# LIU-YUXI/SA-GNN

Hardware: AMD Instinct MI355X
Metric: spmm_edges_per_sec (higher is better)
Workload: dtype f32

## Files before the change

### include/sagnn.h

```cpp
#ifndef SAGNN_H
#define SAGNN_H

#include <stddef.h>
#include <stdint.h>

#ifdef __cplusplus
extern "C" {
#endif

#define SAGNN_VERSION 10302

enum {
  SAGNN_OK = 0,
  SAGNN_ERR_NULL = -1,
  SAGNN_ERR_DIM = -2,
  SAGNN_ERR_ALIGN = -3,
  SAGNN_ERR_CSR = -4,
  SAGNN_ERR_ARG = -5,
  SAGNN_ERR_WORKSPACE = -6,
  SAGNN_ERR_NOMEM = -7
};

int sagnn_version(void);

enum { SAGNN_ENGINE_F16X2 = 0, SAGNN_ENGINE_F32 = 1, SAGNN_ENGINE_VALU = 2 };
int sagnn_set_engine(int engine);
int sagnn_get_engine(void);
int sagnn_range_redo_count(int64_t* count, int reset);

size_t sagnn_last_error(char* buf, size_t cap);

int sagnn_profile_enable(int capacity);
int sagnn_profile_read(float* ms, int32_t* kind, int64_t* units_a, int64_t* units_b, int cap,
                       int* n_out);

int sagnn_csr_check_host(const int32_t* h_rowptr, const int32_t* h_colidx,
                         int64_t n_rows, int64_t n_src, int64_t nnz);

typedef struct sagnn_spmm_plan sagnn_spmm_plan;

typedef struct sagnn_spmm_tuning {
  int32_t short_thresh;
  int32_t long_thresh;
  int32_t chunk_edges;
  int32_t reserved;
} sagnn_spmm_tuning;

typedef struct sagnn_spmm_plan_info {
  int64_t n_rows, n_src, nnz;
  int64_t n_long_rows;
  int64_t n_chunks;
  int32_t short_thresh, long_thresh, chunk_edges;
  int32_t max_degree;
  int32_t on_device;
  int32_t reserved;
} sagnn_spmm_plan_info;

int sagnn_spmm_plan_create(const int32_t* h_rowptr, const int32_t* d_rowptr,
                           const int32_t* d_colidx, int64_t n_rows, int64_t n_src,
                           int64_t nnz, const sagnn_spmm_tuning* tuning ,
                           sagnn_spmm_plan** plan_out);
int sagnn_spmm_plan_destroy(sagnn_spmm_plan* plan);
int sagnn_spmm_plan_get_info(const sagnn_spmm_plan* plan, sagnn_spmm_plan_info* info);
int sagnn_spmm_plan_copy_chunks(const sagnn_spmm_plan* plan, int32_t* rows, int32_t* e_begin,
                                int32_t* e_end, int64_t cap);
size_t sagnn_spmm_workspace_bytes(const sagnn_spmm_plan* plan, int d);

int sagnn_spmm_f32(const sagnn_spmm_plan* plan, const float* X, int64_t ldx, int d,
                   const float* residual, int64_t ldr, float leaky, float* out, int64_t ldo,
                   const float* acc_in, int64_t ld_acc_in, float* acc_out, int64_t ld_acc_out,
                   void* workspace, size_t workspace_bytes, void* stream);

typedef struct sagnn_spmm_epilogue {
  float leaky;
  const float* residual; int64_t ldr;
  float* out; int64_t ldo;
  const float* acc_in; int64_t ld_acc_in;
  float* acc_out; int64_t ld_acc_out;
  uint8_t* mask_out;
  const uint8_t* mask_in;
  float* out2; int64_t ldo2; float slope2;
  const float* acc_in2; int64_t ld_acc_in2;
} sagnn_spmm_epilogue;

int sagnn_spmm_ex_f32(const sagnn_spmm_plan* plan, const float* X, int64_t ldx, int d,
                      const sagnn_spmm_epilogue* epilogue, void* workspace, size_t workspace_bytes,
                      void* stream);
int sagnn_mask_scale_f32(const float* g, int64_t ldg, const uint8_t* mask, float slope, float* out, int64_t ldo,
                         int64_t n_rows, int d, void* stream);

int sagnn_gnn_interval_f32(const sagnn_spmm_plan* plan_user, const sagnn_spmm_plan* plan_item,
                           const float* u0, int64_t ld_u0, const float* i0, int64_t ld_i0,
                           int d, int n_layers, float leaky, float* scratch_u, float* scratch_i,
                           float* user_out, int64_t ld_uo, float* item_out, int64_t ld_io,
                           void* workspace, size_t workspace_bytes, void* stream);

int sagnn_gnn_interval_ex_f32(const sagnn_spmm_plan* plan_user, const sagnn_spmm_plan* plan_item,
                              const float* u0, int64_t ld_u0, const float* i0, int64_t ld_i0, int d,
                              int n_layers, float leaky, float* scratch_u, float* scratch_i,
                              float* user_out, int64_t ld_uo, float* item_out, int64_t ld_io,
                              uint8_t* mask_u, uint8_t* mask_i, void* workspace,
                              size_t workspace_bytes, void* stream);

int sagnn_gnn_interval_bwd_f32(const sagnn_spmm_plan* plan_user, const sagnn_spmm_plan* plan_item,
                               const float* G_u, int64_t ld_gu, const float* G_i, int64_t ld_gi, int d,
                               int n_layers, float leaky, const uint8_t* mask_u, const uint8_t* mask_i,
                               float* scratch_u, float* scratch_i, float* grad_u0, int64_t ld_du,
                               float* grad_i0, int64_t ld_di, void* workspace, size_t workspace_bytes,
                               void* stream);

typedef struct sagnn_spmm_batch sagnn_spmm_batch;
int sagnn_spmm_batch_create(const sagnn_spmm_plan* const* plans_user, const sagnn_spmm_plan* const* plans_item,
                            int n_intervals, sagnn_spmm_batch** batch_out);
int sagnn_spmm_batch_destroy(sagnn_spmm_batch* batch);
size_t sagnn_spmm_batch_workspace_bytes(const sagnn_spmm_batch* batch, int d);
int sagnn_gnn_stack_f32(const sagnn_spmm_batch* batch, const float* u0, int64_t ld_u0, int64_t slab_u0,
                        const float* i0, int64_t ld_i0, int64_t slab_i0, int d, int n_layers, float leaky,
                        float* scratch_u, float* scratch_i, float* user_out, int64_t ld_uo, int64_t slab_uo,
                        float* item_out, int64_t ld_io, int64_t slab_io, uint8_t* mask_u, uint8_t* mask_i,
                        void* workspace, size_t workspace_bytes, void* stream);
int sagnn_gnn_stack_bwd_f32(const sagnn_spmm_batch* batch, const float* G_u, int64_t ld_gu, int64_t slab_gu,
                            const float* G_i, int64_t ld_gi, int64_t slab_gi, int d, int n_layers, float leaky,
                            const uint8_t* mask_u, const uint8_t* mask_i, float* scratch_u, float* scratch_i,
                            float* grad_u0, int64_t ld_du, int64_t slab_du, float* grad_i0, int64_t ld_di,
                            int64_t slab_di, void* workspace, size_t workspace_bytes, void* stream);

int sagnn_lstm_fwd_f32(const float* x, int64_t ld_n, int64_t ld_t, int64_t n, int t, int d, const float* W,
                       const float* b, float forget_bias, const float* drop_scale, float* h,
                       int64_t ld_h, void* stream);
int sagnn_lstm_fwd_state_f32(const float* x, int64_t ld_n, int64_t ld_t, int64_t n, int t, int d,
                             const float* W, const float* b, float forget_bias, const float* drop_scale,
                             const float* h_init, int64_t ld_hi, const float* c_init, float* h, int64_t ld_h,
                             float* c_final, void* stream);
int sagnn_layernorm_td_f32(const float* x, int64_t ld_n, int64_t ld_t, int64_t n, int t, int d,
                           const float* gamma, const float* beta, float eps, float* y,
                           int64_t ld_y, void* stream);
int sagnn_mhsa_mean_f32(const float* x, int64_t ld_n, int64_t ld_t, int64_t n, int t, int d, int heads,
                        const float* Wq, const float* bq, const float* Wk, const float* bk,
                        const float* Wv, const float* bv, float* out, int64_t ld_out,
                        void* stream);
size_t sagnn_mhsa_wide_workspace_bytes(int64_t n, int t, int d);
int sagnn_mhsa_mean_wide_f32(const float* x, int64_t ld_n, int64_t ld_t, int64_t n, int t, int d, int heads,
                             const float* Wq, const float* bq, const float* Wk, const float* bk, const float* Wv,
                             const float* bv, float* out, int64_t ld_out, void* workspace, size_t workspace_bytes,
                             void* stream);
size_t sagnn_ln_mhsa_mean_workspace_bytes(int64_t n, int t, int d, int heads);
int sagnn_ln_mhsa_mean_f32(const float* x, int64_t ld_n, int64_t ld_t, int64_t n, int t, int d, int heads,
                           const float* ln_gamma, const float* ln_beta, float ln_eps, const float* Wq,
                           const float* bq, const float* Wk, const float* bk, const float* Wv, const float* bv,
                           float* out, int64_t ld_out, void* workspace, size_t workspace_bytes, void* stream);
int sagnn_interval_fusion_f32(const float* x, int64_t ld_n, int64_t ld_t, int64_t n, int t, int d, int heads,
                              const float* lstm_W, const float* lstm_b, float forget_bias,
                              const float* ln_gamma, const float* ln_beta, float ln_eps,
                              const float* Wq, const float* bq, const float* Wk, const float* bk,
                              const float* Wv, const float* bv, float* out, int64_t ld_out,
                              void* workspace, size_t workspace_bytes, void* stream);
size_t sagnn_interval_fusion_workspace_bytes(int64_t n, int t, int d);

int sagnn_lstm_fwd_train_f32(const float* x, int64_t ld_n, int64_t ld_t, int64_t n, int t, int d,
                             const float* W, const float* b, float forget_bias, const float* drop_scale,
                             float* h, int64_t ld_h, float* gates, float* cell, void* stream);
int sagnn_attn_bwd_f32(float* qkv, const float* g_out, int64_t ld_g, int64_t n, int t, int d, int heads,
                       void* stream);
int sagnn_layernorm_td_bwd_f32(const float* h, int64_t ld_h, const float* dy, int64_t ld_dy, int64_t n, int t,
                               int d, const float* gamma, float eps, float* dh, int64_t ld_dh, float* dgamma,
                               float* dbeta, void* stream);
int sagnn_lstm_bwd_step_f32(const float* gates, const float* cell, const float* dh_ext, int64_t ld_dhe,
                            const float* drop_scale, const float* dh_rec, int64_t ld_dhr, const float* dc_in,
                            float* dgates, float* dc_out, int64_t n, int t, int d, int ts, void* stream);
int sagnn_attn_bwd_front_supported(int d, int t, int heads);
int sagnn_attn_bwd_front_f32(const float* x, int64_t ld_n, int64_t ld_t, int64_t n, int t, int d, int heads,
                             const float* ln_gamma, const float* ln_beta, float ln_eps, int apply_ln,
                             const float* Wq, const float* bq, const float* Wk, const float* bk, const float* Wv,
                             const float* bv, const float* g_out, int64_t ld_g, float* dqkv, float* y_out,
                             void* stream);
int sagnn_attn_bwd_tail_supported(int d);
int sagnn_attn_bwd_tail_f32(float* y, const float* dqkv, int64_t rows, int d, const float* Wqkv, float* dWqkv,
                            float* dbqkv, void* stream);
int sagnn_lstm_bwd_supported(int d);
int sagnn_lstm_bwd_f32(const float* x, int64_t ld_n, int64_t ld_t, const float* h, const float* gates,
                       const float* cell, const float* dh_ext, int64_t ld_dhe, const float* drop_scale,
                       const float* W, float* dx, float* dW, float* db, int64_t n, int t, int d, void* stream);
size_t sagnn_lstm_bwd_workspace_bytes(int64_t n, int t, int d);
int sagnn_lstm_bwd_ws_f32(const float* x, int64_t ld_n, int64_t ld_t, const float* h, const float* gates,
                          const float* cell, const float* dh_ext, int64_t ld_dhe, const float* drop_scale,
                          const float* W, float* dx, float* dW, float* db, int64_t n, int t, int d, void* workspace,
                          size_t workspace_bytes, void* stream);

int sagnn_leaky_add_f32(const float* a, const float* b, float* out, float leaky, int64_t count, void* stream);
int sagnn_pair_score_f32(const float* U, int64_t ldu, const float* I, int64_t ldi, const float* S, int64_t lds,
                         const float* A, int64_t lda, const int32_t* uids, const int32_t* iids,
                         const int32_t* locs, float leaky, float* out, int64_t n_pairs, int d, void* stream);

int sagnn_pair_score_bwd_f32(const float* U, int64_t ldu, const float* I, int64_t ldi, const float* S, int64_t lds,
                             const float* A, int64_t lda, const int32_t* uids, const int32_t* iids,
                             const int32_t* locs, float leaky, const float* g, float* dU, float* dI, float* dS,
                             float* dA, int64_t n_pairs, int d, void* stream);
int sagnn_prod_leaky_sum_f32(const float* X, int64_t ldx, const float* Y, int64_t ldy, const int32_t* uids,
                             const int32_t* iids, float leaky, float* out, int64_t n_pairs, int d, void* stream);
int sagnn_prod_leaky_sum_bwd_f32(const float* X, int64_t ldx, const float* Y, int64_t ldy, const int32_t* uids,
                                 const int32_t* iids, float leaky, const float* g, float* dX, float* dY,
                                 int64_t n_pairs, int d, void* stream);
int sagnn_meta_features_f32(const float* F, int64_t ldf, const float* V, int64_t ldv, const int32_t* uids,
                            float* out, int64_t n, int d, void* stream);
int sagnn_meta_features_bwd_f32(const float* F, int64_t ldf, const float* V, int64_t ldv, const int32_t* uids,
                                const float* dm, float* dF, float* dV, int64_t n, int d, void* stream);
int sagnn_leaky_f32(const float* a, const float* g, float* out, float leaky, int64_t count, int backward,
                    void* stream);
int sagnn_rowdot_sigmoid_f32(const float* A, int64_t lda, const float* w3, const float* b3, float* out, int64_t n,
                             int k, void* stream);
int sagnn_rowdot_sigmoid_bwd_f32(const float* A, int64_t lda, const float* w3, const float* w, const float* dw,
                                 float* dA, int64_t ldda, float* dw3, float* db3, int64_t n, int k, void* stream);
int sagnn_hinge_f32(const float* pos, const float* neg, const float* wp, const float* wn, const float* sp,
                    const float* sn, float scale, float* loss, float* dpos, float* dneg, float* dwp, float* dwn,
                    int64_t n, void* stream);

int sagnn_mul_f32(const float* a, const float* b, float* out, int64_t count, void* stream);

int sagnn_adam_step_f32(float* param, const float* grad, float* m, float* v, int64_t count, float lr,
                        float beta1, float beta2, float eps, float l2, int64_t step, void* stream);

int sagnn_adam_multi_f32(int n_tensors, float* const* params, const float* const* grads, float* const* m,
                         float* const* v, const int64_t* counts, const float* l2, float lr, float beta1,
                         float beta2, float eps, int64_t step, void* stream);

int sagnn_dense_nn_f32(const float* X, int64_t ldx, int64_t n, int din, int dout, const float* W,
                       const float* bias, float* Y, int64_t ldy, int accumulate, void* stream);
int sagnn_dense_tn_f32(const float* X, int64_t ldx, const float* G, int64_t ldg, int64_t n, int din,
                       int dout, float* dW, float* db, void* stream);
int sagnn_dense_tn_seg_f32(const float* X, int64_t ldx, int64_t x_seg, const float* G, int64_t ldg, int64_t g_seg,
                           int64_t seg_rows, int n_seg, int din, int dout, float* dW, float* db, void* stream);

size_t sagnn_score_topk_workspace_bytes(int64_t n_queries, int64_t n_items, int d, int k);
int sagnn_score_topk_f32(const float* Q, int64_t ldq, const float* I, int64_t ldi, int64_t n_queries, int64_t n_items,
                         int d, int k, const int32_t* excl_rowptr, const int32_t* excl_items, const int32_t* target,
                         int32_t* topk_items, float* topk_scores, int64_t* target_rank, void* workspace,
                         size_t workspace_bytes, void* stream);

int sagnn_candidate_rank_f32(const float* U, int64_t ldu, const float* I, int64_t ldi, const float* S, int64_t lds,
                             const float* A, int64_t lda, const int32_t* uids, const int32_t* cand, int64_t ldc,
                             const int32_t* target, float leaky, int64_t n_rows, int C, int d, int64_t* rank,
                             float* scores, int64_t ld_scores, void* stream);

int sagnn_sample_train_i32(const int32_t* bat_ids, int64_t n_batch, int64_t n_slots, const int64_t* seq_ptr,
                           const int32_t* seq_items, const int64_t* ban_ptr, const int32_t* ban_items, int64_t n_users,
                           int64_t n_items, int train_sample_num, int pred_num, int pos_length, const int64_t* pair_off,
                           int64_t n_pairs, uint64_t seed, int64_t step, int32_t* uids, int32_t* iids,
                           int32_t* uLocs_seq, int64_t* seg_begin, int32_t* seg_len, void* stream);
int sagnn_sample_ssl_i32(const int32_t* bat_ids, int64_t n_batch, int n_intervals, const int64_t* sub_ptr,
                         const int32_t* sub_items, int64_t n_users, int ssl_num, const int64_t* ssl_off, int64_t n_out,
                         uint64_t seed, int64_t step, int32_t* uids, int32_t* iids, int32_t* uLocs_seq, void* stream);
int sagnn_seq_sum_f32(const float* fi, int64_t ldf, int64_t n_items, const float* pos_embed, int64_t ldp,
                      int pos_length, const int32_t* seq_items, int64_t n_flat, const int64_t* seg_begin,
                      const int32_t* seg_len, int64_t n_slots, int d, float* seq_tok, float* pos_tok, int64_t ldo,
                      void* stream);
int sagnn_seq_sum_bwd_f32(const float* g_seq, const float* g_pos, int64_t ldg, const int32_t* seq_items, int64_t n_flat,
                          const int64_t* seg_begin, const int32_t* seg_len, int64_t n_slots, int pos_length, int d,
                          float* d_fi, int64_t ld_dfi, int64_t n_items, float* d_pos, int64_t ld_dpos, void* stream);

int sagnn_rows_mark_i32(const int32_t* ids, int64_t n_ids, int64_t n_rows, uint8_t* flags, void* stream);
int sagnn_rows_mark_seg_i32(const int32_t* seq_items, int64_t n_flat, const int64_t* seg_begin, const int32_t* seg_len,
                            int64_t n_slots, int max_len, int64_t n_rows, uint8_t* flags, void* stream);
size_t sagnn_rows_compact_workspace_bytes(int64_t n_rows);
int sagnn_rows_compact_i32(uint8_t* flags, int64_t n_rows, int32_t* rows, int64_t cap, int32_t* count, void* workspace,
                           size_t workspace_bytes, void* stream);
int sagnn_rows_gather_f32(const float* x, int64_t ld_n, int64_t ld_t, int64_t n_rows, int t, int d, const int32_t* rows,
                          int64_t cap, const int32_t* count, float* out, void* stream);
int sagnn_rows_scatter_f32(const float* src, const int32_t* rows, int64_t cap, const int32_t* count, int t, int d,
                           float* dst, int64_t ld_n, int64_t ld_t, int64_t n_rows, void* stream);

#ifdef __cplusplus
}
#endif
#endif
```

### sa-gnn_amd/_lib.py

```python
from __future__ import annotations

import ctypes
import os
from ctypes import POINTER, c_char_p, c_float, c_int, c_int32, c_int64, c_size_t, c_uint64, c_void_p

_HERE = os.path.dirname(os.path.abspath(__file__))
LIB_PATH = os.environ.get("SAGNN_LIB") or os.path.join(_HERE, "lib", "libsagnn.so")


class SagnnError(RuntimeError):
    def __init__(self, code: int, msg: str):
        super().__init__(f"libsagnn error {code}: {msg}")
        self.code = code


class Tuning(ctypes.Structure):
    _fields_ = [("short_thresh", c_int32), ("long_thresh", c_int32), ("chunk_edges", c_int32),
                ("reserved", c_int32)]


class SpmmEpilogue(ctypes.Structure):
    _fields_ = [("leaky", c_float), ("residual", c_void_p), ("ldr", c_int64), ("out", c_void_p),
                ("ldo", c_int64), ("acc_in", c_void_p), ("ld_acc_in", c_int64), ("acc_out", c_void_p),
                ("ld_acc_out", c_int64), ("mask_out", c_void_p), ("mask_in", c_void_p),
                ("out2", c_void_p), ("ldo2", c_int64), ("slope2", c_float), ("acc_in2", c_void_p),
                ("ld_acc_in2", c_int64)]


class PlanInfo(ctypes.Structure):
    _fields_ = [("n_rows", c_int64), ("n_src", c_int64), ("nnz", c_int64),
                ("n_long_rows", c_int64), ("n_chunks", c_int64), ("short_thresh", c_int32),
                ("long_thresh", c_int32), ("chunk_edges", c_int32), ("max_degree", c_int32),
                ("on_device", c_int32), ("reserved", c_int32)]


SIGNATURES = {
    "sagnn_version": (c_int, []),
    "sagnn_set_engine": (c_int, [c_int]),
    "sagnn_get_engine": (c_int, []),
    "sagnn_range_redo_count": (c_int, [POINTER(c_int64), c_int]),
    "sagnn_last_error": (c_size_t, [c_char_p, c_size_t]),
    "sagnn_profile_enable": (c_int, [c_int]),
    "sagnn_profile_read": (c_int, [c_void_p, c_void_p, c_void_p, c_void_p, c_int, POINTER(c_int)]),
    "sagnn_csr_check_host": (c_int, [c_void_p, c_void_p, c_int64, c_int64, c_int64]),
    "sagnn_spmm_plan_create": (c_int, [c_void_p, c_void_p, c_void_p, c_int64, c_int64, c_int64,
                                       POINTER(Tuning), POINTER(c_void_p)]),
    "sagnn_spmm_plan_destroy": (c_int, [c_void_p]),
    "sagnn_spmm_plan_get_info": (c_int, [c_void_p, POINTER(PlanInfo)]),
    "sagnn_spmm_plan_copy_chunks": (c_int, [c_void_p, c_void_p, c_void_p, c_void_p, c_int64]),
    "sagnn_spmm_workspace_bytes": (c_size_t, [c_void_p, c_int]),
    "sagnn_spmm_f32": (c_int, [c_void_p, c_void_p, c_int64, c_int, c_void_p, c_int64, c_float,
                               c_void_p, c_int64, c_void_p, c_int64, c_void_p, c_int64, c_void_p,
                               c_size_t, c_void_p]),
    "sagnn_spmm_ex_f32": (c_int, [c_void_p, c_void_p, c_int64, c_int, POINTER(SpmmEpilogue), c_void_p, c_size_t,
                                  c_void_p]),
    "sagnn_mask_scale_f32": (c_int, [c_void_p, c_int64, c_void_p, c_float, c_void_p, c_int64, c_int64, c_int, c_void_p]),
    "sagnn_gnn_interval_ex_f32": (c_int, [c_void_p, c_void_p, c_void_p, c_int64, c_void_p, c_int64, c_int, c_int,
                                          c_float, c_void_p, c_void_p, c_void_p, c_int64, c_void_p, c_int64,
                                          c_void_p, c_void_p, c_void_p, c_size_t, c_void_p]),
    "sagnn_gnn_interval_bwd_f32": (c_int, [c_void_p, c_void_p, c_void_p, c_int64, c_void_p, c_int64, c_int, c_int,
                                           c_float, c_void_p, c_void_p, c_void_p, c_void_p, c_void_p, c_int64,
                                           c_void_p, c_int64, c_void_p, c_size_t, c_void_p]),
    "sagnn_spmm_batch_create": (c_int, [c_void_p, c_void_p, c_int, POINTER(c_void_p)]),
    "sagnn_spmm_batch_destroy": (c_int, [c_void_p]),
    "sagnn_spmm_batch_workspace_bytes": (c_size_t, [c_void_p, c_int]),
    "sagnn_gnn_stack_f32": (c_int, [c_void_p, c_void_p, c_int64, c_int64, c_void_p, c_int64, c_int64, c_int, c_int, c_float,
                                    c_void_p, c_void_p, c_void_p, c_int64, c_int64, c_void_p, c_int64, c_int64, c_void_p,
                                    c_void_p, c_void_p, c_size_t, c_void_p]),
    "sagnn_gnn_stack_bwd_f32": (c_int, [c_void_p, c_void_p, c_int64, c_int64, c_void_p, c_int64, c_int64, c_int, c_int,
                                        c_float, c_void_p, c_void_p, c_void_p, c_void_p, c_void_p, c_int64, c_int64,
                                        c_void_p, c_int64, c_int64, c_void_p, c_size_t, c_void_p]),
    "sagnn_gnn_interval_f32": (c_int, [c_void_p, c_void_p, c_void_p, c_int64, c_void_p, c_int64,
                                       c_int, c_int, c_float, c_void_p, c_void_p, c_void_p, c_int64,
                                       c_void_p, c_int64, c_void_p, c_size_t, c_void_p]),
    "sagnn_lstm_fwd_train_f32": (c_int, [c_void_p, c_int64, c_int64, c_int64, c_int, c_int, c_void_p, c_void_p, c_float,
                                         c_void_p, c_void_p, c_int64, c_void_p, c_void_p, c_void_p]),
    "sagnn_mhsa_wide_workspace_bytes": (c_size_t, [c_int64, c_int, c_int]),
    "sagnn_ln_mhsa_mean_workspace_bytes": (c_size_t, [c_int64, c_int, c_int, c_int]),
    "sagnn_ln_mhsa_mean_f32": (c_int, [c_void_p, c_int64, c_int64, c_int64, c_int, c_int, c_int, c_void_p, c_void_p,
                                       c_float, c_void_p, c_void_p, c_void_p, c_void_p, c_void_p, c_void_p, c_void_p,
                                       c_int64, c_void_p, c_size_t, c_void_p]),
    "sagnn_mhsa_mean_wide_f32": (c_int, [c_void_p, c_int64, c_int64, c_int64, c_int, c_int, c_int, c_void_p, c_void_p,
                                         c_void_p, c_void_p, c_void_p, c_void_p, c_void_p, c_int64, c_void_p, c_size_t,
                                         c_void_p]),
    "sagnn_attn_bwd_f32": (c_int, [c_void_p, c_void_p, c_int64, c_int64, c_int, c_int, c_int, c_void_p]),
    "sagnn_layernorm_td_bwd_f32": (c_int, [c_void_p, c_int64, c_void_p, c_int64, c_int64, c_int, c_int, c_void_p,
                                           c_float, c_void_p, c_int64, c_void_p, c_void_p, c_void_p]),
    "sagnn_lstm_bwd_step_f32": (c_int, [c_void_p, c_void_p, c_void_p, c_int64, c_void_p, c_void_p, c_int64, c_void_p,
                                        c_void_p, c_void_p, c_int64, c_int, c_int, c_int, c_void_p]),
    "sagnn_attn_bwd_front_supported": (c_int, [c_int, c_int, c_int]),
    "sagnn_attn_bwd_front_f32": (c_int, [c_void_p, c_int64, c_int64, c_int64, c_int, c_int, c_int, c_void_p, c_void_p,
                                         c_float, c_int, c_void_p, c_void_p, c_void_p, c_void_p, c_void_p, c_void_p,
                                         c_void_p, c_int64, c_void_p, c_void_p, c_void_p]),
    "sagnn_attn_bwd_tail_supported": (c_int, [c_int]),
    "sagnn_attn_bwd_tail_f32": (c_int, [c_void_p, c_void_p, c_int64, c_int, c_void_p, c_void_p, c_void_p, c_void_p]),
    "sagnn_lstm_bwd_supported": (c_int, [c_int]),
    "sagnn_lstm_bwd_f32": (c_int, [c_void_p, c_int64, c_int64, c_void_p, c_void_p, c_void_p, c_void_p, c_int64, c_void_p,
                                   c_void_p, c_void_p, c_void_p, c_void_p, c_int64, c_int, c_int, c_void_p]),
    "sagnn_lstm_bwd_workspace_bytes": (c_size_t, [c_int64, c_int, c_int]),
    "sagnn_lstm_bwd_ws_f32": (c_int, [c_void_p, c_int64, c_int64, c_void_p, c_void_p, c_void_p, c_void_p, c_int64, c_void_p,
                                      c_void_p, c_void_p, c_void_p, c_void_p, c_int64, c_int, c_int, c_void_p, c_size_t, c_void_p]),
    "sagnn_leaky_add_f32": (c_int, [c_void_p, c_void_p, c_void_p, c_float, c_int64, c_void_p]),
    "sagnn_pair_score_f32": (c_int, [c_void_p, c_int64, c_void_p, c_int64, c_void_p, c_int64, c_void_p, c_int64,
                                     c_void_p, c_void_p, c_void_p, c_float, c_void_p, c_int64, c_int, c_void_p]),
    "sagnn_pair_score_bwd_f32": (c_int, [c_void_p, c_int64, c_void_p, c_int64, c_void_p, c_int64, c_void_p, c_int64,
                                         c_void_p, c_void_p, c_void_p, c_float, c_void_p, c_void_p, c_void_p, c_void_p,
                                         c_void_p, c_int64, c_int, c_void_p]),
    "sagnn_prod_leaky_sum_f32": (c_int, [c_void_p, c_int64, c_void_p, c_int64, c_void_p, c_void_p, c_float, c_void_p,
                                         c_int64, c_int, c_void_p]),
    "sagnn_prod_leaky_sum_bwd_f32": (c_int, [c_void_p, c_int64, c_void_p, c_int64, c_void_p, c_void_p, c_float,
                                             c_void_p, c_void_p, c_void_p, c_int64, c_int, c_void_p]),
    "sagnn_meta_features_f32": (c_int, [c_void_p, c_int64, c_void_p, c_int64, c_void_p, c_void_p, c_int64, c_int,
                                        c_void_p]),
    "sagnn_meta_features_bwd_f32": (c_int, [c_void_p, c_int64, c_void_p, c_int64, c_void_p, c_void_p, c_void_p,
                                            c_void_p, c_int64, c_int, c_void_p]),
    "sagnn_leaky_f32": (c_int, [c_void_p, c_void_p, c_void_p, c_float, c_int64, c_int, c_void_p]),
    "sagnn_rowdot_sigmoid_f32": (c_int, [c_void_p, c_int64, c_void_p, c_void_p, c_void_p, c_int64, c_int, c_void_p]),
    "sagnn_rowdot_sigmoid_bwd_f32": (c_int, [c_void_p, c_int64, c_void_p, c_void_p, c_void_p, c_void_p, c_int64,
                                             c_void_p, c_void_p, c_int64, c_int, c_void_p]),
    "sagnn_hinge_f32": (c_int, [c_void_p, c_void_p, c_void_p, c_void_p, c_void_p, c_void_p, c_float, c_void_p,
                                c_void_p, c_void_p, c_void_p, c_void_p, c_int64, c_void_p]),
    "sagnn_mul_f32": (c_int, [c_void_p, c_void_p, c_void_p, c_int64, c_void_p]),
    "sagnn_adam_step_f32": (c_int, [c_void_p, c_void_p, c_void_p, c_void_p, c_int64, c_float, c_float, c_float,
                                    c_float, c_float, c_int64, c_void_p]),
    "sagnn_adam_multi_f32": (c_int, [c_int, c_void_p, c_void_p, c_void_p, c_void_p, c_void_p, c_void_p, c_float, c_float,
                                     c_float, c_float, c_int64, c_void_p]),
    "sagnn_dense_nn_f32": (c_int, [c_void_p, c_int64, c_int64, c_int, c_int, c_void_p, c_void_p, c_void_p, c_int64,
                                   c_int, c_void_p]),
    "sagnn_dense_tn_f32": (c_int, [c_void_p, c_int64, c_void_p, c_int64, c_int64, c_int, c_int, c_void_p, c_void_p,
                                   c_void_p]),
    "sagnn_dense_tn_seg_f32": (c_int, [c_void_p, c_int64, c_int64, c_void_p, c_int64, c_int64, c_int64, c_int, c_int, c_int,
                                       c_void_p, c_void_p, c_void_p]),
    "sagnn_lstm_fwd_f32": (c_int, [c_void_p, c_int64, c_int64, c_int64, c_int, c_int, c_void_p, c_void_p,
                                   c_float, c_void_p, c_void_p, c_int64, c_void_p]),
    "sagnn_lstm_fwd_state_f32": (c_int, [c_void_p, c_int64, c_int64, c_int64, c_int, c_int, c_void_p, c_void_p, c_float,
                                         c_void_p, c_void_p, c_int64, c_void_p, c_void_p, c_int64, c_void_p, c_void_p]),
    "sagnn_layernorm_td_f32": (c_int, [c_void_p, c_int64, c_int64, c_int64, c_int, c_int, c_void_p, c_void_p,
                                       c_float, c_void_p, c_int64, c_void_p]),
    "sagnn_mhsa_mean_f32": (c_int, [c_void_p, c_int64, c_int64, c_int64, c_int, c_int, c_int, c_void_p,
                                    c_void_p, c_void_p, c_void_p, c_void_p, c_void_p, c_void_p,
                                    c_int64, c_void_p]),
    "sagnn_interval_fusion_f32": (c_int, [c_void_p, c_int64, c_int64, c_int64, c_int, c_int, c_int, c_void_p,
                                          c_void_p, c_float, c_void_p, c_void_p, c_float, c_void_p,
                                          c_void_p, c_void_p, c_void_p, c_void_p, c_void_p, c_void_p,
                                          c_int64, c_void_p, c_size_t, c_void_p]),
    "sagnn_interval_fusion_workspace_bytes": (c_size_t, [c_int64, c_int, c_int]),
    "sagnn_score_topk_workspace_bytes": (c_size_t, [c_int64, c_int64, c_int, c_int]),
    "sagnn_score_topk_f32": (c_int, [c_void_p, c_int64, c_void_p, c_int64, c_int64, c_int64, c_int, c_int, c_void_p,
                                     c_void_p, c_void_p, c_void_p, c_void_p, c_void_p, c_void_p, c_size_t, c_void_p]),
    "sagnn_candidate_rank_f32": (c_int, [c_void_p, c_int64, c_void_p, c_int64, c_void_p, c_int64, c_void_p, c_int64,
                                         c_void_p, c_void_p, c_int64, c_void_p, c_float, c_int64, c_int, c_int, c_void_p,
                                         c_void_p, c_int64, c_void_p]),
    "sagnn_sample_train_i32": (c_int, [c_void_p, c_int64, c_int64, c_void_p, c_void_p, c_void_p, c_void_p, c_int64, c_int64,
                                       c_int, c_int, c_int, c_void_p, c_int64, c_uint64, c_int64, c_void_p, c_void_p,
                                       c_void_p, c_void_p, c_void_p, c_void_p]),
    "sagnn_sample_ssl_i32": (c_int, [c_void_p, c_int64, c_int, c_void_p, c_void_p, c_int64, c_int, c_void_p, c_int64,
                                     c_uint64, c_int64, c_void_p, c_void_p, c_void_p, c_void_p]),
    "sagnn_seq_sum_f32": (c_int, [c_void_p, c_int64, c_int64, c_void_p, c_int64, c_int, c_void_p, c_int64, c_void_p,
                                  c_void_p, c_int64, c_int, c_void_p, c_void_p, c_int64, c_void_p]),
    "sagnn_seq_sum_bwd_f32": (c_int, [c_void_p, c_void_p, c_int64, c_void_p, c_int64, c_void_p, c_void_p, c_int64, c_int,
                                      c_int, c_void_p, c_int64, c_int64, c_void_p, c_int64, c_void_p]),
    "sagnn_rows_mark_i32": (c_int, [c_void_p, c_int64, c_int64, c_void_p, c_void_p]),
    "sagnn_rows_mark_seg_i32": (c_int, [c_void_p, c_int64, c_void_p, c_void_p, c_int64, c_int, c_int64, c_void_p, c_void_p]),
    "sagnn_rows_compact_workspace_bytes": (c_size_t, [c_int64]),
    "sagnn_rows_compact_i32": (c_int, [c_void_p, c_int64, c_void_p, c_int64, c_void_p, c_void_p, c_size_t, c_void_p]),
    "sagnn_rows_gather_f32": (c_int, [c_void_p, c_int64, c_int64, c_int64, c_int, c_int, c_void_p, c_int64, c_void_p,
                                      c_void_p, c_void_p]),
    "sagnn_rows_scatter_f32": (c_int, [c_void_p, c_void_p, c_int64, c_void_p, c_int, c_int, c_void_p, c_int64, c_int64,
                                       c_int64, c_void_p]),
}

_lib = None


def load() -> ctypes.CDLL:
    global _lib
    if _lib is not None:
        return _lib
    if not os.path.exists(LIB_PATH):
        raise ImportError(
            f"{LIB_PATH} not found: build it with `python -c 'import __graft_entry__ as g; "
            "g.build()'` (or `make -C sa-gnn_amd/csrc`). There is no fallback path.")
    lib = ctypes.CDLL(LIB_PATH)
    for name, (res, args) in SIGNATURES.items():
        fn = getattr(lib, name)
        fn.restype = res
        fn.argtypes = args
    _lib = lib
    return lib


def last_error() -> str:
    buf = ctypes.create_string_buffer(1024)
    load().sagnn_last_error(buf, 1024)
    return buf.value.decode("utf-8", "replace")


def check(rc: int) -> None:
    if rc != 0:
        raise SagnnError(rc, last_error())
```

### sa-gnn_amd/csrc/attn_split.hip

```cpp
#include "common.h"
#include "f16_split.h"

namespace {

typedef float f32x4 __attribute__((ext_vector_type(4)));
typedef int i32x4 __attribute__((ext_vector_type(4)));
typedef int i32x2 __attribute__((ext_vector_type(2)));

constexpr int kRows = 64;
constexpr int kBT = 4;
constexpr int kRec = 48;

template <int D>
__device__ __forceinline__ int swz(int row) {
  if (D == 128) return row & 15;
  if (D == 64) return (row >> 1) & 7;
  const int g = (row >> 2) & 3;
  return (0x78 >> (2 * g)) & 3;
}
__device__ __forceinline__ void lds_barrier() { asm volatile("s_waitcnt lgkmcnt(0)\n\ts_barrier" ::: "memory"); }

__host__ __device__ constexpr int pad_node(int t) { return t == 6 ? 16 : 0; }
__host__ __device__ constexpr int pad_group(int t) { return (t == 1 || t == 3 || t == 5) ? 64 : t == 6 ? 32 : 16; }
__host__ __device__ constexpr int lanes_per_pair(int t, int d) {
  if (d == 128) return (t % 4 == 0) ? 4 : (t % 2 == 0) ? 2 : 1;
  return t == 16 ? 4 : (t == 8 || t == 12) ? 2 : 1;
}

template <int DK>
struct HeadVec {
  typedef float type __attribute__((ext_vector_type(DK)));
  static __device__ __forceinline__ type load(const char* p, int gs) { return *reinterpret_cast<const type*>(p); }
  static __device__ __forceinline__ void store(char* p, int gs, type v) { *reinterpret_cast<type*>(p) = v; }
};
template <>
struct HeadVec<8> {
  typedef float type __attribute__((ext_vector_type(8)));
  typedef float f4 __attribute__((ext_vector_type(4)));
  static __device__ __forceinline__ type load(const char* p, int gs) {
    const f4 a = *reinterpret_cast<const f4*>(p), b = *reinterpret_cast<const f4*>(p + gs);
    return type{a[0], a[1], a[2], a[3], b[0], b[1], b[2], b[3]};
  }
  static __device__ __forceinline__ void store(char* p, int gs, type v) {
    *reinterpret_cast<f4*>(p) = f4{v[0], v[1], v[2], v[3]};
    *reinterpret_cast<f4*>(p + gs) = f4{v[4], v[5], v[6], v[7]};
  }
};

template <int CTRL>
__device__ __forceinline__ float dpp_add(float v) {
  return v + __builtin_bit_cast(float, __builtin_amdgcn_update_dpp(0, __builtin_bit_cast(int, v), CTRL, 0xf, 0xf, true));
}
template <int LPR>
__device__ __forceinline__ float row_sum(float v) {
  v = dpp_add<0xB1>(v);
  v = dpp_add<0x4E>(v);
  v = dpp_add<0x141>(v);
  if constexpr (LPR >= 16) v = dpp_add<0x140>(v);
  if constexpr (LPR == 32) v += __shfl_xor(v, 16);
  return v;
}

template <int D, int T, int LP, bool BWD>
__global__ __launch_bounds__(64 * (D >= 64 ? 4 : D / 16), (D == 128 || (BWD && T >= 8)) ? 1 : 2) void ln_mhsa_split_kernel(
    const float* __restrict__ x, int64_t ld_n, int64_t ld_t, int64_t n, const float* __restrict__ gamma,
    const float* __restrict__ beta, float eps, int apply_ln, const float* __restrict__ Wq,
    const float* __restrict__ bq, const float* __restrict__ Wk, const float* __restrict__ bk,
    const float* __restrict__ Wv, const float* __restrict__ bv, float* out, int64_t ld_out,
    int64_t n_tiles, float* __restrict__ dqkv_out, float* __restrict__ y_out, unsigned int* __restrict__ redo_ctr) {
  static_assert(!BWD || D <= 64 || LP == 1, "d = 128: the backward front keeps a pair in one lane");
  constexpr int NW = D >= 64 ? 4 : D / 16, NT = 64 * NW, KS = D / 32;
  constexpr int DK = D / 16;
  constexpr int HPW = 16 / DK;
  constexpr int NB = kRows / T;
  constexpr int ROWS = NB * T;
  constexpr int PLANE = kRows * D * 2;
  constexpr int LPR = D / 4, RPP = NT / LPR, NFILL = kRows / RPP;
  constexpr int PN = pad_node(T), PG = pad_group(T);
  constexpr int GS = kRows * kRec + NB * PN + PG;
  constexpr int QKVW = 4 * GS;
  typedef typename HeadVec<DK>::type vec;

  extern __shared__ __attribute__((aligned(16))) char lds[];
  char* const Yp = lds;
  char* const QKV = lds + 2 * PLANE;
  float2* const rstat = reinterpret_cast<float2*>(QKV + NW * QKVW);
  float2* const nstat = rstat + kRows;
  int* const flags = reinterpret_cast<int*>(nstat + NB);
  const int tid = threadIdx.x, lane = tid & 63;
  const int wave = __builtin_amdgcn_readfirstlane(tid >> 6);
  const int m = lane & 15, q = lane >> 4;
  const int cbase = 64 * (int)blockIdx.y + 16 * wave;
  const int col0 = cbase + 4 * q;
  const int fr = tid / LPR, fc4 = (tid % LPR) * 4;
  char* const tab = QKV + wave * QKVW;
  constexpr bool WL = D == 64 && (T & (T - 1)) == 0;
  constexpr int PP = T >= 4 ? T / 4 : 1;
  constexpr int GP = T >= 4 ? 4 : T;
  auto fill_row = [&](int p, int fr_now) { return WL ? 16 * wave + 4 * p + (lane >> 4) : p * RPP + fr_now; };

  float k4096 = 4096.f;
  asm volatile("" : "+v"(k4096));
  if (tid < 3) flags[tid] = 0;
  __syncthreads();
  const float qscale = 1.44269504088896340736f * (DK == 4 ? 0.5f : DK == 2 ? 0.70710678118654752440f : 0.35355339059327376220f);

  i32x4 wf[3][KS][2];
  {
    const float* const Ws[3] = {Wq, Wk, Wv};
    RangeTrack wr = range_init();
#pragma unroll
    for (int mat = 0; mat < 3; ++mat)
#pragma unroll
      for (int ks = 0; ks < KS; ++ks) {
        float wv[8];
#pragma unroll
        for (int j = 0; j < 8; ++j) wv[j] = Ws[mat][(size_t)(32 * ks + 8 * q + j) * D + cbase + m] * (mat == 0 ? qscale : 1.f);
        range_seg4(wr, wv[0], wv[1], wv[2], wv[3]);
        range_seg4(wr, wv[4], wv[5], wv[6], wv[7]);
#pragma unroll
        for (int e = 0; e < 4; ++e) {
          const int hd = head2(wv[2 * e], wv[2 * e + 1]);
          wf[mat][ks][0][e] = hd;
          wf[mat][ks][1][e] = tail2(hd, wv[2 * e], wv[2 * e + 1], k4096);
        }
      }
    if (range_bad(wr)) flags[2] = 1;
  }
  f32x4 bias3[3];
#pragma unroll
  for (int r = 0; r < 4; ++r) {
    bias3[0][r] = bq[col0 + r] * qscale;
    bias3[1][r] = bk[col0 + r];
    bias3[2][r] = bv[col0 + r];
  }
  float4 g4 = make_float4(1.f, 1.f, 1.f, 1.f), b4 = make_float4(0.f, 0.f, 0.f, 0.f);
  if (apply_ln) {
    g4 = *reinterpret_cast<const float4*>(gamma + fc4);
    b4 = *reinterpret_cast<const float4*>(beta + fc4);
  }
  const float inv_t = 1.f / (float)T;

  float4 xr[NFILL];
  auto fetch_tile = [&](int64_t tile) {
    const int64_t node0 = tile * NB;
#pragma unroll
    for (int p = 0; p < NFILL; ++p) {
      const int r = fill_row(p, fr);
      const int nb = r / T, ts = r - nb * T;
      xr[p] = make_float4(0.f, 0.f, 0.f, 0.f);
      if (tile < n_tiles && r < ROWS && node0 + nb < n)
        xr[p] = *reinterpret_cast<const float4*>(x + (node0 + nb) * ld_n + (int64_t)ts * ld_t + fc4);
    }
  };
  fetch_tile(blockIdx.x);

  int par = 0;
  for (int64_t tile = blockIdx.x; tile < n_tiles; tile += gridDim.x, par ^= 1) {
    const int64_t node0 = tile * NB;
    if (tid == 0) flags[par] = 0;
    int fr_ = fr, fc4_ = fc4, m_ = m, q_ = q;
    asm volatile("" : "+v"(fr_), "+v"(fc4_), "+v"(m_), "+v"(q_));

    float2 wst[NFILL];
    if constexpr (WL) {
      if (apply_ln) {
        float mr[NFILL], m2[NFILL];
#pragma unroll
        for (int p = 0; p < NFILL; ++p) {
          mr[p] = row_sum<LPR>((xr[p].x + xr[p].y) + (xr[p].z + xr[p].w)) * (1.f / (float)D);
          const float dx = xr[p].x - mr[p], dy = xr[p].y - mr[p], dz = xr[p].z - mr[p], dw = xr[p].w - mr[p];
          m2[p] = row_sum<LPR>((dx * dx + dy * dy) + (dz * dz + dw * dw));
        }
#pragma unroll
        for (int j = 0; j < NFILL / PP; ++j) {
          float sm = 0.f;
#pragma unroll
          for (int i = 0; i < PP; ++i) sm += mr[j * PP + i];
          if constexpr (GP >= 2) sm += __shfl_xor(sm, 16);
          if constexpr (GP == 4) sm += __shfl_xor(sm, 32);
          const float mean = sm * inv_t;
          float q2 = 0.f;
#pragma unroll
          for (int i = 0; i < PP; ++i) {
            const float dm = mr[j * PP + i] - mean;
            q2 += m2[j * PP + i] + (float)D * dm * dm;
          }
          if constexpr (GP >= 2) q2 += __shfl_xor(q2, 16);
          if constexpr (GP == 4) q2 += __shfl_xor(q2, 32);
          const float2 st = make_float2(mean, rsqrtf(q2 * (1.f / (float)(T * D)) + eps));
#pragma unroll
          for (int i = 0; i < PP; ++i) wst[j * PP + i] = st;
          const int r0 = fill_row(j * PP, fr_);
          if (fc4_ == 0 && r0 % T == 0) nstat[r0 / T] = st;
        }
      }
    } else if (apply_ln) {
#pragma unroll
      for (int p = 0; p < NFILL; ++p) {
        const float mr = row_sum<LPR>((xr[p].x + xr[p].y) + (xr[p].z + xr[p].w)) * (1.f / (float)D);
        const float dx = xr[p].x - mr, dy = xr[p].y - mr, dz = xr[p].z - mr, dw = xr[p].w - mr;
        const float m2 = row_sum<LPR>((dx * dx + dy * dy) + (dz * dz + dw * dw));
        if (fc4_ == 0) rstat[p * RPP + fr_] = make_float2(mr, m2);
      }
      lds_barrier();
      if (tid < NB) {
        float ms = 0.f;
#pragma unroll
        for (int ts = 0; ts < T; ++ts) ms += rstat[tid * T + ts].x;
        const float mean = ms * inv_t;
        float m2 = 0.f;
#pragma unroll
        for (int ts = 0; ts < T; ++ts) {
          const float2 st = rstat[tid * T + ts];
          const float dm = st.x - mean;
          m2 += st.y + (float)D * dm * dm;
        }
        nstat[tid] = make_float2(mean, rsqrtf(m2 * (1.f / (float)(T * D)) + eps));
      }
      lds_barrier();
    }
    RangeTrack yr = range_init();
#pragma unroll
    for (int p = 0; p < NFILL; ++p) {
      const int r = fill_row(p, fr_);
      float4 y = xr[p];
      if (apply_ln) {
        const float2 st = WL ? wst[p] : nstat[r < ROWS ? r / T : 0];
        const float ix = st.y * g4.x, iy = st.y * g4.y, iz = st.y * g4.z, iw = st.y * g4.w;
        y.x = xr[p].x * ix + (b4.x - st.x * ix);
        y.y = xr[p].y * iy + (b4.y - st.x * iy);
        y.z = xr[p].z * iz + (b4.z - st.x * iz);
        y.w = xr[p].w * iw + (b4.w - st.x * iw);
      }
      range_seg4(yr, y.x, y.y, y.z, y.w);
      if constexpr (BWD) {
        if (y_out && blockIdx.y == 0 && r < ROWS && node0 + r / T < n)
          *reinterpret_cast<float4*>(y_out + (node0 * T + r) * D + fc4_) = y;
      }
      const int p0 = head2(y.x, y.y), p1 = head2(y.z, y.w);
      const int off = r * (D * 2) + (((fc4_ >> 3) ^ swz<D>(r)) << 4) + ((fc4_ >> 2) & 1) * 8;
      *reinterpret_cast<i32x2*>(Yp + off) = i32x2{p0, p1};
      *reinterpret_cast<i32x2*>(Yp + PLANE + off) = i32x2{tail2(p0, y.x, y.y, k4096), tail2(p1, y.z, y.w, k4096)};
    }
    fetch_tile(tile + gridDim.x);
    lds_barrier();
    if (range_bad(yr)) flags[par] = 1;

#pragma unroll
    for (int bt = 0; bt < kBT; ++bt) {
      const int row = bt * 16 + m_;
      const int sw = swz<D>(row);
      f32x4 hi[3] = {bias3[0], bias3[1], bias3[2]};
      f32x4 lo[3];
#pragma unroll
      for (int ks = 0; ks < KS; ++ks) {
        const int off = row * (D * 2) + (((ks * 4 + q_) ^ sw) << 4);
        const f16x8 b1 = __builtin_bit_cast(f16x8, *reinterpret_cast<const i32x4*>(Yp + off));
        const f16x8 b2 = __builtin_bit_cast(f16x8, *reinterpret_cast<const i32x4*>(Yp + PLANE + off));
#pragma unroll
        for (int mat = 0; mat < 3; ++mat) {
          const f16x8 a1 = __builtin_bit_cast(f16x8, wf[mat][ks][0]);
          const f16x8 a2 = __builtin_bit_cast(f16x8, wf[mat][ks][1]);
          lo[mat] = __builtin_amdgcn_mfma_f32_16x16x32_f16(a2, b1, ks == 0 ? f32x4{0.f, 0.f, 0.f, 0.f} : lo[mat], 0, 0, 0);
          lo[mat] = __builtin_amdgcn_mfma_f32_16x16x32_f16(a1, b2, lo[mat], 0, 0, 0);
          hi[mat] = __builtin_amdgcn_mfma_f32_16x16x32_f16(a1, b1, hi[mat], 0, 0, 0);
        }
      }
      f32x4 acc[3];
#pragma unroll
      for (int mat = 0; mat < 3; ++mat)
#pragma unroll
        for (int r = 0; r < 4; ++r) acc[mat][r] = fmaf(lo[mat][r], kLoInv, hi[mat][r]);
      char* rec = tab + q_ * GS + row * kRec + (row / T) * PN;
      *reinterpret_cast<f32x4*>(rec) = acc[0];
      *reinterpret_cast<f32x4*>(rec + 16) = acc[1];
      *reinterpret_cast<f32x4*>(rec + 32) = acc[2];
    }
    lds_barrier();
    if (flags[par] | flags[2]) {
      if (tid == 0 && redo_ctr) atomicAdd(redo_ctr, 1u);
      constexpr int NCOL = 16 * NW;
      const float* const Ws[3] = {Wq, Wk, Wv};
      const float* const bs[3] = {bq, bk, bv};
      for (int idx = tid; idx < ROWS * 3 * NCOL; idx += NT) {
        const int r = idx / (3 * NCOL), rem = idx - r * (3 * NCOL), mat = rem / NCOL, cl = rem - mat * NCOL;
        const int nb = r / T, ts = r - nb * T;
        if (node0 + nb >= n) continue;
        const int col = 64 * (int)blockIdx.y + cl;
        const float sc = mat == 0 ? qscale : 1.f;
        const float2 st = apply_ln ? nstat[nb] : make_float2(0.f, 1.f);
        const float* const xrow = x + (node0 + nb) * ld_n + (int64_t)ts * ld_t;
        float acc = bs[mat][col] * sc;
        for (int k = 0; k < D; ++k) {
          float yv = xrow[k];
          if (apply_ln) {
            const float ik = st.y * gamma[k];
            yv = yv * ik + (beta[k] - st.x * ik);
          }
          acc = fmaf(yv, Ws[mat][(size_t)k * D + col] * sc, acc);
        }
        *reinterpret_cast<float*>(QKV + (cl >> 4) * QKVW + ((cl >> 2) & 3) * GS + r * kRec + nb * PN + mat * 16 + (cl & 3) * 4) = acc;
      }
      __syncthreads();
    }

    constexpr int PAIRS = NB * HPW;
    constexpr int LSTEP = 64 / LP;
    constexpr int TQ = T / LP;
    constexpr int KC = T <= 8 ? T : T / 2;
    static_assert(T % LP == 0 && T % KC == 0 && LP <= T, "query / key split");
    const int part = lane % LP;
    if constexpr (BWD) {
      const float scale = qscale * 0.69314718055994530942f;
      auto quad_sum = [&](float v) {
        if constexpr (LP > 1) v += __builtin_bit_cast(float, __builtin_amdgcn_update_dpp(0, __builtin_bit_cast(int, v), 0xB1, 0xf, 0xf, true));
        if constexpr (LP > 2) v += __builtin_bit_cast(float, __builtin_amdgcn_update_dpp(0, __builtin_bit_cast(int, v), 0x4E, 0xf, 0xf, true));
        return v;
      };
#pragma unroll 1
      for (int p = lane / LP; p < PAIRS; p += LSTEP) {
        const int hl = p % HPW, nb = p / HPW;
        const char* base = tab + ((hl * DK) >> 2) * GS + nb * (T * kRec + PN) + ((hl * DK) & 3) * 4;
        const int64_t node = node0 + nb;
        vec g = (vec)(0.f);
        if (node < n) g = *reinterpret_cast<const vec*>(out + node * ld_out + cbase + hl * DK);
        g *= inv_t;
        vec kv[T], vv[T], dk[T];
        float ps[T], asum[T];
#pragma unroll
        for (int ts = 0; ts < T; ++ts) {
          kv[ts] = HeadVec<DK>::load(base + ts * kRec + 16, GS);
          vv[ts] = HeadVec<DK>::load(base + ts * kRec + 32, GS);
          dk[ts] = (vec)(0.f);
          asum[ts] = 0.f;
          float pd = g[0] * vv[ts][0];
#pragma unroll
          for (int c = 1; c < DK; ++c) pd = fmaf(g[c], vv[ts][c], pd);
          ps[ts] = pd;
        }
        float* const drow = dqkv_out + (node * T) * (3 * D) + cbase + hl * DK;
#pragma unroll
        for (int i = 0; i < TQ; ++i) {
          const int tq = part * TQ + i;
          const vec qv = HeadVec<DK>::load(base + tq * kRec, GS);
          float a[T];
          float rs = 0.f;
#pragma unroll
          for (int s_ = 0; s_ < T; ++s_) {
            float z = qv[0] * kv[s_][0];
#pragma unroll
            for (int c = 1; c < DK; ++c) z = fmaf(qv[c], kv[s_][c], z);
            a[s_] = __builtin_amdgcn_exp2f(z);
            rs += a[s_];
          }
          const float inv = __builtin_amdgcn_rcpf(rs + 1e-8f);
          float dot = 0.f;
#pragma unroll
          for (int s_ = 0; s_ < T; ++s_) {
            a[s_] *= inv;
            dot = fmaf(a[s_], ps[s_], dot);
          }
          vec dq = (vec)(0.f);
#pragma unroll
          for (int s_ = 0; s_ < T; ++s_) {
            const float dz = a[s_] * (ps[s_] - dot);
            dq += dz * kv[s_];
            dk[s_] += dz * qv;
            asum[s_] += a[s_];
          }
          if (node < n) *reinterpret_cast<vec*>(drow + tq * (3 * D)) = dq * scale;
        }
        if constexpr (LP > 1) {
#pragma unroll
          for (int ts = 0; ts < T; ++ts) {
#pragma unroll
            for (int c = 0; c < DK; ++c) {
              float v = dk[ts][c];
              v = quad_sum(v);
              dk[ts][c] = v;
            }
            asum[ts] = quad_sum(asum[ts]);
          }
        }
        if (node < n) {
#pragma unroll
          for (int ts = 0; ts < T; ++ts) {
            if (LP > 1 && ts / TQ != part) continue;
            *reinterpret_cast<vec*>(drow + ts * (3 * D) + D) = dk[ts] * 0.69314718055994530942f;
            *reinterpret_cast<vec*>(drow + ts * (3 * D) + 2 * D) = g * asum[ts];
          }
        }
      }
      continue;
    }
#pragma unroll 1
    for (int p = lane / LP; p < PAIRS; p += LSTEP) {
      const int hl = p % HPW, nb = p / HPW;
      char* base = tab + ((hl * DK) >> 2) * GS + nb * (T * kRec + PN) + ((hl * DK) & 3) * 4;
      vec qv[TQ];
      float e[TQ][T], rs[TQ];
#pragma unroll
      for (int i = 0; i < TQ; ++i) qv[i] = HeadVec<DK>::load(base + (part * TQ + i) * kRec, GS);
#pragma unroll
      for (int ch = 0; ch < T / KC; ++ch) {
        vec k[KC];
#pragma unroll
        for (int s = 0; s < KC; ++s) k[s] = HeadVec<DK>::load(base + (ch * KC + s) * kRec + 16, GS);
#pragma unroll
        for (int i = 0; i < TQ; ++i)
#pragma unroll
          for (int s = 0; s < KC; ++s) {
            float pd = qv[i][0] * k[s][0];
#pragma unroll
            for (int c = 1; c < DK; ++c) pd = fmaf(qv[i][c], k[s][c], pd);
            const float ev = __builtin_amdgcn_exp2f(pd);
            e[i][ch * KC + s] = ev;
            rs[i] = (ch == 0 && s == 0) ? ev : rs[i] + ev;
          }
      }
      float w[T];
#pragma unroll
      for (int i = 0; i < TQ; ++i) {
        const float inv = __builtin_amdgcn_rcpf(rs[i] + 1e-8f);
#pragma unroll
        for (int s = 0; s < T; ++s) w[s] = i == 0 ? e[0][s] * inv : fmaf(e[i][s], inv, w[s]);
      }
      vec o = (vec)(0.f);
#pragma unroll
      for (int ch = 0; ch < T / KC; ++ch) {
        vec v[KC];
#pragma unroll
        for (int s = 0; s < KC; ++s) v[s] = HeadVec<DK>::load(base + (ch * KC + s) * kRec + 32, GS);
#pragma unroll
        for (int s = 0; s < KC; ++s) o += w[ch * KC + s] * v[s];
      }
      if (LP > 1) {
#pragma unroll
        for (int c = 0; c < DK; ++c) {
          float oc = o[c];
          oc += __builtin_bit_cast(float, __builtin_amdgcn_update_dpp(0, __builtin_bit_cast(int, oc), 0xB1, 0xf, 0xf, true));
          if (LP > 2) oc += __builtin_bit_cast(float, __builtin_amdgcn_update_dpp(0, __builtin_bit_cast(int, oc), 0x4E, 0xf, 0xf, true));
          o[c] = oc;
        }
      }
      const int64_t node = node0 + nb;
      if (part == 0 && node < n) {
        const vec ov = o * inv_t;
        float* dst = out + node * ld_out + cbase + hl * DK;
        if constexpr (DK == 8) {
          *reinterpret_cast<float4*>(dst) = make_float4(ov[0], ov[1], ov[2], ov[3]);
          *reinterpret_cast<float4*>(dst + 4) = make_float4(ov[4], ov[5], ov[6], ov[7]);
        } else {
          *reinterpret_cast<vec*>(dst) = ov;
        }
      }
    }
  }
}

}

namespace sagnn {

template <int D, int T, bool BWD = false>
static int launch_split(const float* x, int64_t ld_n, int64_t ld_t, int64_t n, const float* gamma, const float* beta,
                        float eps, int apply_ln, const float* Wq, const float* bq, const float* Wk, const float* bk,
                        const float* Wv, const float* bv, float* out, int64_t ld_out, hipStream_t s,
                        float* dqkv = nullptr, float* y = nullptr) {
  constexpr int NW = D >= 64 ? 4 : D / 16, NB = kRows / T;
  constexpr int LP = (BWD && D == 128) ? 1 : lanes_per_pair(T, D);
  constexpr int GS = kRows * kRec + NB * pad_node(T) + pad_group(T);
  const size_t lds = (size_t)2 * kRows * D * 2 + (size_t)NW * 4 * GS + (size_t)(kRows + NB) * sizeof(float2) + 16;
  if (int rc = ensure_dynamic_lds(reinterpret_cast<const void*>(&ln_mhsa_split_kernel<D, T, LP, BWD>), lds)) return rc;
  const int per_cu = (D == 128 || (BWD && T >= 8)) ? 1 : D == 64 ? 2 : 4;
  constexpr int CB = D == 128 ? 2 : 1;
  const int64_t n_tiles = (n + NB - 1) / NB;
  const int64_t want = (int64_t)cu_count_current() * per_cu / CB;
  const int64_t blocks = n_tiles < want ? n_tiles : (want > 0 ? want : 1);
  ProfileScope prof(kProfMhsa, s, n, T);
  hipLaunchKernelGGL((ln_mhsa_split_kernel<D, T, LP, BWD>), dim3((unsigned)blocks, CB), dim3(64 * NW), lds, s, x, ld_n, ld_t, n,
                     gamma, beta, eps, apply_ln, Wq, bq, Wk, bk, Wv, bv, out, ld_out, n_tiles, dqkv, y, redo_counter());
  SAGNN_HIP_TRY(hipGetLastError());
  return SAGNN_OK;
}

template <int D>
static int dispatch_t(const float* x, int64_t ld_n, int64_t ld_t, int64_t n, int t, const float* gamma,
                      const float* beta, float eps, int apply_ln, const float* Wq, const float* bq, const float* Wk,
                      const float* bk, const float* Wv, const float* bv, float* out, int64_t ld_out, hipStream_t s) {
#define SAGNN_T_CASE(TT) \
  case TT: return launch_split<D, TT>(x, ld_n, ld_t, n, gamma, beta, eps, apply_ln, Wq, bq, Wk, bk, Wv, bv, out, ld_out, s);
  switch (t) {
    SAGNN_T_CASE(1) SAGNN_T_CASE(2) SAGNN_T_CASE(3) SAGNN_T_CASE(4) SAGNN_T_CASE(5) SAGNN_T_CASE(6)
    SAGNN_T_CASE(8) SAGNN_T_CASE(12) SAGNN_T_CASE(16)
    default: return fail(SAGNN_ERR_DIM, "split attention: t = %d has no specialised kernel", t);
  }
#undef SAGNN_T_CASE
}

int ln_mhsa_mean_split(const float* x, int64_t ld_n, int64_t ld_t, int64_t n, int t, int d, int heads,
                       const float* gamma, const float* beta, float eps, int apply_ln, const float* Wq,
                       const float* bq, const float* Wk, const float* bk, const float* Wv, const float* bv,
                       float* out, int64_t ld_out, hipStream_t s) {
  if (!mhsa_split_supported(d, t, heads)) return fail(SAGNN_ERR_DIM, "split attention: unsupported d/t/heads");
  if (d == 128) return dispatch_t<128>(x, ld_n, ld_t, n, t, gamma, beta, eps, apply_ln, Wq, bq, Wk, bk, Wv, bv, out, ld_out, s);
  if (d == 64) return dispatch_t<64>(x, ld_n, ld_t, n, t, gamma, beta, eps, apply_ln, Wq, bq, Wk, bk, Wv, bv, out, ld_out, s);
  return dispatch_t<32>(x, ld_n, ld_t, n, t, gamma, beta, eps, apply_ln, Wq, bq, Wk, bk, Wv, bv, out, ld_out, s);
}

template <int D>
static int dispatch_bwd_t(const float* x, int64_t ld_n, int64_t ld_t, int64_t n, int t, const float* gamma, const float* beta,
                          float eps, int apply_ln, const float* Wq, const float* bq, const float* Wk, const float* bk,
                          const float* Wv, const float* bv, const float* g_out, int64_t ld_g, float* dqkv, float* y,
                          hipStream_t s) {
#define SAGNN_T_CASE(TT)                                                                                              \
  case TT:                                                                                                            \
    return launch_split<D, TT, true>(x, ld_n, ld_t, n, gamma, beta, eps, apply_ln, Wq, bq, Wk, bk, Wv, bv,            \
                                     const_cast<float*>(g_out), ld_g, s, dqkv, y);
  switch (t) {
    SAGNN_T_CASE(1) SAGNN_T_CASE(2) SAGNN_T_CASE(3) SAGNN_T_CASE(4) SAGNN_T_CASE(5) SAGNN_T_CASE(6)
    case 8: case 12: case 16:
      if constexpr (D <= 64) {
        if (t == 8) return launch_split<D, 8, true>(x, ld_n, ld_t, n, gamma, beta, eps, apply_ln, Wq, bq, Wk, bk, Wv, bv, const_cast<float*>(g_out), ld_g, s, dqkv, y);
        if (t == 12) return launch_split<D, 12, true>(x, ld_n, ld_t, n, gamma, beta, eps, apply_ln, Wq, bq, Wk, bk, Wv, bv, const_cast<float*>(g_out), ld_g, s, dqkv, y);
        return launch_split<D, 16, true>(x, ld_n, ld_t, n, gamma, beta, eps, apply_ln, Wq, bq, Wk, bk, Wv, bv, const_cast<float*>(g_out), ld_g, s, dqkv, y);
      }
      [[fallthrough]];
    default: return fail(SAGNN_ERR_DIM, "split attention backward front: t = %d has no specialised kernel", t);
  }
#undef SAGNN_T_CASE
}

int attn_bwd_front_split(const float* x, int64_t ld_n, int64_t ld_t, int64_t n, int t, int d, int heads, const float* gamma,
                         const float* beta, float eps, int apply_ln, const float* Wq, const float* bq, const float* Wk,
                         const float* bk, const float* Wv, const float* bv, const float* g_out, int64_t ld_g, float* dqkv,
                         float* y, hipStream_t s) {
  if (!attn_bwd_front_split_supported(d, t, heads)) return fail(SAGNN_ERR_DIM, "split attention backward front: unsupported d/t/heads");
  if (d == 128)
    return dispatch_bwd_t<128>(x, ld_n, ld_t, n, t, gamma, beta, eps, apply_ln, Wq, bq, Wk, bk, Wv, bv, g_out, ld_g, dqkv, y, s);
  if (d == 64)
    return dispatch_bwd_t<64>(x, ld_n, ld_t, n, t, gamma, beta, eps, apply_ln, Wq, bq, Wk, bk, Wv, bv, g_out, ld_g, dqkv, y, s);
  return dispatch_bwd_t<32>(x, ld_n, ld_t, n, t, gamma, beta, eps, apply_ln, Wq, bq, Wk, bk, Wv, bv, g_out, ld_g, dqkv, y, s);
}

}
```

### sa-gnn_amd/csrc/common.h

```cpp
#pragma once
#include <hip/hip_runtime.h>
#include <stdint.h>
#include <stdio.h>
#include <string>

#include "engine.h"
#include "sagnn.h"

namespace sagnn {

std::string& last_error_slot();
int fail(int code, const char* fmt, ...) __attribute__((format(printf, 2, 3)));
int hip_fail(hipError_t e, const char* what);

inline bool aligned16(const void* p) { return (reinterpret_cast<uintptr_t>(p) & 15u) == 0; }

#define SAGNN_HIP_TRY(expr)                                   \
  do {                                                        \
    hipError_t _e = (expr);                                   \
    if (_e != hipSuccess) return ::sagnn::hip_fail(_e, #expr); \
  } while (0)

inline int lanes_per_row(int d) {
  int need = (d + 3) / 4;
  int lpr = 8;
  while (lpr < need) lpr <<= 1;
  return lpr;
}

int ensure_dynamic_lds(const void* kernel, size_t bytes);
int cu_count_current();
unsigned int* redo_counter();

int lstm_fwd_mfma(const float* x, int64_t ld_n, int64_t ld_t, int64_t n, int t, int d, const float* W,
                  const float* b, float forget_bias, const float* drop, float* h, int64_t ld_h,
                  float* gates_out, float* c_out, const float* h_init, int64_t ld_hi, const float* c_init,
                  float* c_final, hipStream_t s);
int ln_mhsa_mean_mfma(const float* x, int64_t ld_n, int64_t ld_t, int64_t n, int t, int d, int heads,
                      const float* gamma, const float* beta, float eps, int apply_ln, const float* Wq,
                      const float* bq, const float* Wk, const float* bk, const float* Wv,
                      const float* bv, float* out, int64_t ld_out, hipStream_t s);
int attn_bwd_front_mfma(const float* x, int64_t ld_n, int64_t ld_t, int64_t n, int t, int d, int heads,
                        const float* gamma, const float* beta, float eps, int apply_ln, const float* Wq,
                        const float* bq, const float* Wk, const float* bk, const float* Wv, const float* bv,
                        const float* g_out, int64_t ld_g, float* dqkv, float* y, hipStream_t s);
int lstm_fwd_f16(const float* x, int64_t ld_n, int64_t ld_t, int64_t n, int t, int d, const float* W, const float* b,
                 float forget_bias, const float* drop, float* h, int64_t ld_h, float* gates_out, float* c_out,
                 const float* h_init, int64_t ld_hi, const float* c_init, float* c_final, hipStream_t s);
int ln_mhsa_mean_split(const float* x, int64_t ld_n, int64_t ld_t, int64_t n, int t, int d, int heads,
                       const float* gamma, const float* beta, float eps, int apply_ln, const float* Wq,
                       const float* bq, const float* Wk, const float* bk, const float* Wv, const float* bv,
                       float* out, int64_t ld_out, hipStream_t s);
int lstm_fwd_split128(const float* x, int64_t ld_n, int64_t ld_t, int64_t n, int t, const float* W, const float* b,
                      float forget_bias, const float* drop, float* h, int64_t ld_h, float* gates_out, float* c_out,
                      const float* h_init, int64_t ld_hi, const float* c_init, float* c_final, hipStream_t s);
int attn_bwd_tail_f16(float* y, const float* dqkv, int64_t rows, int d, const float* Wqkv, float* dWqkv, float* dbqkv,
                      hipStream_t s);
int lstm_dw_f16(const float* x, int64_t ld_n, int64_t ld_t, const float* h, const float* dg, int64_t n, int t, int d, float* dW,
                hipStream_t s);
int attn_bwd_front_split(const float* x, int64_t ld_n, int64_t ld_t, int64_t n, int t, int d, int heads, const float* gamma,
                         const float* beta, float eps, int apply_ln, const float* Wq, const float* bq, const float* Wk,
                         const float* bk, const float* Wv, const float* bv, const float* g_out, int64_t ld_g, float* dqkv,
                         float* y, hipStream_t s);
int dense_nn_any(const float* X, int64_t ldx, int64_t n, int din, int dout, const float* W, int64_t ldw,
                 const float* bias, float* Y, int64_t ldy, int accumulate, hipStream_t s);
int dense_tn_any(const float* X, int64_t ldx, const float* G, int64_t ldg, int64_t n, int din, int dout, float* dW,
                 int64_t lddw, float* db, hipStream_t s);
int gemm_nn(const float* X, int64_t ldx, int64_t n, int din, int dout, const float* W, int64_t ldw, const float* bias, float* Y,
            int64_t ldy, int accumulate, hipStream_t s);
int gemm_tn(const float* X, int64_t ldx, int64_t xseg, const float* G, int64_t ldg, int64_t gseg, int64_t seg_rows, int64_t n_seg,
            int din, int dout, float* dW, int64_t lddw, float* db, hipStream_t s);

enum ProfileKind { kProfSpmmRows = 0, kProfSpmmFixup = 1, kProfLstm = 2, kProfLayerNorm = 3, kProfMhsa = 4 };

class ProfileScope {
 public:
  ProfileScope(int kind, hipStream_t stream, int64_t units_a, int64_t units_b);
  ~ProfileScope();
  ProfileScope(const ProfileScope&) = delete;
  ProfileScope& operator=(const ProfileScope&) = delete;

 private:
  int slot_;
  hipStream_t stream_;
};

}
```

### sa-gnn_amd/csrc/engine.cpp

```cpp
#include "engine.h"

#include "common.h"

namespace sagnn {

static thread_local Engine tl_engine = Engine::F16x2;
Engine calling_engine() { return tl_engine; }

static bool d32_or_64(int d) { return d == 32 || d == 64; }

LstmFwd select_lstm_fwd(Engine e, int d, int t, bool vec, int64_t ld_h, bool h_vec, bool train, bool drop, bool drop_vec) {
  if (e == Engine::Valu || !vec) return LstmFwd::Valu;
  if (d32_or_64(d)) {
    if (e == Engine::F16x2 && !(train && drop) && ld_h < (1 << 22) && (int64_t)t * d < (1 << 18)) return LstmFwd::F16x2;
    return LstmFwd::F32Mfma;
  }
  if (d == 128 && e == Engine::F16x2 && h_vec && (train ? drop_vec : !drop)) return LstmFwd::Split128;
  return LstmFwd::Valu;
}

AttnFwd select_attn_fwd(Engine e, int d, int t, int heads, bool vec) {
  if (e == Engine::Valu) return AttnFwd::Valu;
  if (vec && e == Engine::F16x2 && mhsa_split_supported(d, t, heads)) return AttnFwd::Split;
  if (vec && mhsa_mfma_supported(d, t, heads)) return AttnFwd::F32Mfma;
  if (!d32_or_64(d) && wide_supported(d)) return AttnFwd::Wide;
  return AttnFwd::Valu;
}

AttnBwdFront select_attn_bwd_front(Engine e, int d, int t, int heads) {
  if (e != Engine::F32 && attn_bwd_front_split_supported(d, t, heads)) return AttnBwdFront::Split;
  if (mhsa_mfma_supported(d, t, heads) && (d / heads == 2 || d / heads == 4) && (t <= 6 || t == 8))
    return AttnBwdFront::F32Mfma;
  return AttnBwdFront::None;
}

AttnBwdTail select_attn_bwd_tail(Engine e, int d) {
  return !d32_or_64(d) ? AttnBwdTail::None : e == Engine::F32 ? AttnBwdTail::F32Mfma : AttnBwdTail::F16x2;
}

LstmBwd select_lstm_bwd(Engine e, int d, bool workspace) {
  return !d32_or_64(d) ? LstmBwd::None : e == Engine::F16x2 && workspace ? LstmBwd::SplitDw : LstmBwd::OneLaunch;
}

bool mhsa_split_supported(int d, int t, int heads) {
  if (heads != 16 || !(d == 32 || d == 64 || d == 128)) return false;
  return (t >= 1 && t <= 6) || t == 8 || t == 12 || t == 16;
}

bool attn_bwd_front_split_supported(int d, int t, int heads) {
  if (heads != 16) return false;
  if (d == 128) return t >= 1 && t <= 6;
  return d32_or_64(d) && ((t >= 1 && t <= 6) || t == 8 || t == 12 || t == 16);
}

bool mhsa_mfma_supported(int d, int t, int heads) {
  if (!d32_or_64(d) || t < 1 || t > 32 || heads < 1 || d % heads) return false;
  const int dk = d / heads;
  return (dk & (dk - 1)) == 0;
}

bool wide_supported(int d) { return d % 32 == 0 && d >= 32 && d <= 256; }

}

extern "C" int sagnn_set_engine(int engine) {
  if (engine != SAGNN_ENGINE_F16X2 && engine != SAGNN_ENGINE_F32 && engine != SAGNN_ENGINE_VALU)
    return sagnn::fail(SAGNN_ERR_ARG, "sagnn_set_engine: unknown engine %d", engine);
  sagnn::tl_engine = static_cast<sagnn::Engine>(engine);
  return SAGNN_OK;
}
extern "C" int sagnn_get_engine(void) { return static_cast<int>(sagnn::calling_engine()); }
```

### sa-gnn_amd/csrc/engine.h

```cpp
#pragma once
#include <stdint.h>

#include "sagnn.h"

namespace sagnn {

enum class Engine { F16x2 = SAGNN_ENGINE_F16X2, F32 = SAGNN_ENGINE_F32, Valu = SAGNN_ENGINE_VALU };
Engine calling_engine();

enum class LstmFwd { F16x2, F32Mfma, Split128, Valu };
enum class AttnFwd { Split, F32Mfma, Wide, Valu };
enum class AttnBwdFront { Split, F32Mfma, None };
enum class AttnBwdTail { F16x2, F32Mfma, None };
enum class LstmBwd { OneLaunch, SplitDw, None };

LstmFwd select_lstm_fwd(Engine e, int d, int t, bool vec, int64_t ld_h, bool h_vec, bool train, bool drop, bool drop_vec);
AttnFwd select_attn_fwd(Engine e, int d, int t, int heads, bool vec);
AttnBwdFront select_attn_bwd_front(Engine e, int d, int t, int heads);
AttnBwdTail select_attn_bwd_tail(Engine e, int d);
LstmBwd select_lstm_bwd(Engine e, int d, bool workspace);

bool mhsa_split_supported(int d, int t, int heads);
bool attn_bwd_front_split_supported(int d, int t, int heads);
bool mhsa_mfma_supported(int d, int t, int heads);
bool wide_supported(int d);

}
```

### sa-gnn_amd/csrc/fusion.hip

```cpp
#include "common.h"

namespace {

constexpr int kBlock = 256;
constexpr int kLstmRowsPerThread = 4;

__device__ __forceinline__ float sigmoidf_(float x) { return 1.f / (1.f + expf(-x)); }

__global__ void lstm_fwd_valu_kernel(const float* __restrict__ x, int64_t ld_n, int64_t ld_t,
                                     int64_t n, int t, int d, const float* __restrict__ W,
                                     const float* __restrict__ b, float forget_bias,
                                     const float* __restrict__ drop, float* __restrict__ h_out,
                                     int64_t ld_h, float* __restrict__ gates_out,
                                     float* __restrict__ c_out, const float* __restrict__ h_init, int64_t ld_hi,
                                     const float* __restrict__ c_init, float* __restrict__ c_final) {
  extern __shared__ float sm[];
  constexpr int RPT = kLstmRowsPerThread;
  const int j = threadIdx.x % d;
  const int rs = threadIdx.x / d;
  const int slots = blockDim.x / d;
  const int rows_pb = slots * RPT;
  const int64_t row_base = (int64_t)blockIdx.x * rows_pb;
  const int d2 = 2 * d, d4 = 4 * d;

  float c[RPT];
#pragma unroll
  for (int r = 0; r < RPT; ++r) {
    const int64_t row = row_base + rs * RPT + r;
    c[r] = (c_init && row < n) ? c_init[row * d + j] : 0.f;
  }
  for (int i = threadIdx.x; i < rows_pb * d; i += blockDim.x) {
    const int64_t row = row_base + i / d;
    sm[(i / d) * d2 + d + (i % d)] = (h_init && row < n) ? h_init[row * ld_hi + (i % d)] : 0.f;
  }

  const float b_i = b[j], b_j = b[d + j], b_f = b[2 * d + j], b_o = b[3 * d + j];
  for (int ts = 0; ts < t; ++ts) {
    for (int i = threadIdx.x; i < rows_pb * d; i += blockDim.x) {
      const int r = i / d, k = i % d;
      const int64_t row = row_base + r;
      sm[r * d2 + k] = row < n ? x[row * ld_n + (int64_t)ts * ld_t + k] : 0.f;
    }
    __syncthreads();
    float gi[RPT], gj[RPT], gf[RPT], go[RPT];
#pragma unroll
    for (int r = 0; r < RPT; ++r) {
      gi[r] = 0.f;
      gj[r] = 0.f;
      gf[r] = 0.f;
      go[r] = 0.f;
    }
    for (int k = 0; k < d2; ++k) {
      const float* wr = W + (int64_t)k * d4 + j;
      const float wi = wr[0], wj = wr[d], wf = wr[2 * d], wo = wr[3 * d];
#pragma unroll
      for (int r = 0; r < RPT; ++r) {
        const float a = sm[(rs * RPT + r) * d2 + k];
        gi[r] = fmaf(a, wi, gi[r]);
        gj[r] = fmaf(a, wj, gj[r]);
        gf[r] = fmaf(a, wf, gf[r]);
        go[r] = fmaf(a, wo, go[r]);
      }
    }
    __syncthreads();
#pragma unroll
    for (int r = 0; r < RPT; ++r) {
      const int lr = rs * RPT + r;
      const int64_t row = row_base + lr;
      const float si = sigmoidf_(gi[r] + b_i), tj = tanhf(gj[r] + b_j);
      const float sf = sigmoidf_(gf[r] + b_f + forget_bias), so = sigmoidf_(go[r] + b_o);
      const float cn = c[r] * sf + si * tj;
      const float hn = tanhf(cn) * so;
      c[r] = cn;
      sm[lr * d2 + d + j] = hn;
      if (gates_out && row < n) {
        float* gp = gates_out + (row * t + ts) * (int64_t)d4 + j;
        gp[0] = si;
        gp[d] = tj;
        gp[2 * d] = sf;
        gp[3 * d] = so;
        c_out[(row * t + ts) * (int64_t)d + j] = cn;
      }
      if (row < n) {
        const int64_t o = row * ld_h + (int64_t)ts * d + j;
        h_out[o] = drop ? hn * drop[row * (int64_t)t * d + (int64_t)ts * d + j] : hn;
      }
    }
  }
  if (c_final) {
#pragma unroll
    for (int r = 0; r < RPT; ++r) {
      const int64_t row = row_base + rs * RPT + r;
      if (row < n) c_final[row * d + j] = c[r];
    }
  }
}

__global__ void layernorm_td_kernel(const float* x, int64_t ld_n, int64_t ld_t, int64_t n, int t, int d,
                                    const float* __restrict__ gamma,
                                    const float* __restrict__ beta, float eps, float* y,
                                    int64_t ld_y) {
  const int lane = threadIdx.x & 63;
  const int64_t node = (int64_t)blockIdx.x * (blockDim.x >> 6) + (threadIdx.x >> 6);
  if (node >= n) return;
  const int td = t * d;
  const float* xr = x + node * ld_n;
  float s = 0.f;
  for (int i = lane; i < td; i += 64) s += xr[(int64_t)(i / d) * ld_t + (i % d)];
#pragma unroll
  for (int off = 32; off > 0; off >>= 1) s += __shfl_xor(s, off);
  const float mean = s / (float)td;
  float v = 0.f;
  for (int i = lane; i < td; i += 64) {
    const float dlt = xr[(int64_t)(i / d) * ld_t + (i % d)] - mean;
    v = fmaf(dlt, dlt, v);
  }
#pragma unroll
  for (int off = 32; off > 0; off >>= 1) v += __shfl_xor(v, off);
  const float rstd = rsqrtf(v / (float)td + eps);
  float* yr = y + node * ld_y;
  for (int i = lane; i < td; i += 64) {
    const int k = i % d;
    const float inv = rstd * gamma[k];
    yr[i] = xr[(int64_t)(i / d) * ld_t + k] * inv + (beta[k] - mean * inv);
  }
}

__global__ void mhsa_mean_valu_kernel(const float* __restrict__ x, int64_t ld_n, int64_t ld_t,
                                      int64_t n, int t, int d, int heads,
                                      const float* __restrict__ Wq,
                                      const float* __restrict__ bq, const float* __restrict__ Wk,
                                      const float* __restrict__ bk, const float* __restrict__ Wv,
                                      const float* __restrict__ bv, float* __restrict__ out,
                                      int64_t ld_out) {
  extern __shared__ float sm[];
  const int j = threadIdx.x % d;
  const int slot = threadIdx.x / d;
  const int slots = blockDim.x / d;
  const int td = t * d;
  float* ys = sm + (size_t)slot * 4 * td;
  float* qs = ys + td;
  float* ks = qs + td;
  float* vs = ks + td;
  const int dk = d / heads;
  const int hoff = (j / dk) * dk;
  const float scale = 1.f / sqrtf((float)dk);

  for (int64_t node0 = (int64_t)blockIdx.x * slots; node0 < n; node0 += (int64_t)gridDim.x * slots) {
    const int64_t node = node0 + slot;
    const bool valid = node < n;
    for (int ts = 0; ts < t; ++ts) ys[ts * d + j] = valid ? x[node * ld_n + (int64_t)ts * ld_t + j] : 0.f;
    __syncthreads();
    for (int ts = 0; ts < t; ++ts) {
      float q = 0.f, k = 0.f, v = 0.f;
      for (int kk = 0; kk < d; ++kk) {
        const float a = ys[ts * d + kk];
        q = fmaf(a, Wq[kk * d + j], q);
        k = fmaf(a, Wk[kk * d + j], k);
        v = fmaf(a, Wv[kk * d + j], v);
      }
      qs[ts * d + j] = q + bq[j];
      ks[ts * d + j] = k + bk[j];
      vs[ts * d + j] = v + bv[j];
    }
    __syncthreads();
    float o = 0.f;
    for (int tq = 0; tq < t; ++tq) {
      float rowsum = 0.f, ctx = 0.f;
      for (int s = 0; s < t; ++s) {
        float dot = 0.f;
        for (int c = 0; c < dk; ++c) dot = fmaf(qs[tq * d + hoff + c], ks[s * d + hoff + c], dot);
        const float e = expf(dot * scale);
        rowsum += e;
        ctx = fmaf(e, vs[s * d + j], ctx);
      }
      o += ctx / (rowsum + 1e-8f);
    }
    if (valid) out[node * ld_out + j] = o / (float)t;
    __syncthreads();
  }
}



__global__ void attn_mean_from_qkv_kernel(const float* __restrict__ qkv, int64_t n, int t, int d, int heads,
                                          float* __restrict__ out, int64_t ld_out) {
  extern __shared__ float sm[];
  const int j = threadIdx.x % d;
  const int slot = threadIdx.x / d;
  const int slots = blockDim.x / d;
  const int td = t * d;
  float* qs = sm + (size_t)slot * 3 * td;
  float* ks = qs + td;
  float* vs = ks + td;
  const int dk = d / heads;
  const int hoff = (j / dk) * dk;
  const float scale = 1.f / sqrtf((float)dk);
  for (int64_t node0 = (int64_t)blockIdx.x * slots; node0 < n; node0 += (int64_t)gridDim.x * slots) {
    const int64_t node = node0 + slot;
    const bool valid = node < n;
    const float* row = qkv + (valid ? node : 0) * (int64_t)(3 * td);
    for (int ts = 0; ts < t; ++ts) {
      qs[ts * d + j] = row[ts * 3 * d + j];
      ks[ts * d + j] = row[ts * 3 * d + d + j];
      vs[ts * d + j] = row[ts * 3 * d + 2 * d + j];
    }
    __syncthreads();
    float o = 0.f;
    for (int tq = 0; tq < t; ++tq) {
      float rowsum = 0.f, ctx = 0.f;
      for (int s2 = 0; s2 < t; ++s2) {
        float dot = 0.f;
        for (int c = 0; c < dk; ++c) dot = fmaf(qs[tq * d + hoff + c], ks[s2 * d + hoff + c], dot);
        const float e = expf(dot * scale);
        rowsum += e;
        ctx = fmaf(e, vs[s2 * d + j], ctx);
      }
      o += ctx / (rowsum + 1e-8f);
    }
    if (valid) out[node * ld_out + j] = o / (float)t;
    __syncthreads();
  }
}

int check_dims(int64_t n, int t, int d) {
  if (n < 0) return sagnn::fail(SAGNN_ERR_ARG, "n = %lld < 0", (long long)n);
  if (t < 1 || t > 64) return sagnn::fail(SAGNN_ERR_DIM, "t = %d: need 1..64", t);
  if (d < 4 || d > 256 || (d & 3)) return sagnn::fail(SAGNN_ERR_DIM, "d = %d: need a multiple of 4 in [4, 256]", d);
  return SAGNN_OK;
}

int check_strides(int64_t ld_n, int64_t ld_t, int64_t n, int t, int d) {
  if (ld_n < d || ld_t < d) return sagnn::fail(SAGNN_ERR_ARG, "ld_n / ld_t smaller than d");
  const bool node_major = ld_n >= (int64_t)(t - 1) * ld_t + d;
  const bool time_major = ld_t >= (n - 1) * ld_n + d;
  if (!node_major && !time_major && n > 1 && t > 1)
    return sagnn::fail(SAGNN_ERR_ARG, "ld_n = %lld, ld_t = %lld overlap for n = %lld, t = %d",
                       (long long)ld_n, (long long)ld_t, (long long)n, t);
  return SAGNN_OK;
}

}

namespace sagnn {

int lstm_fwd_valu(const float* x, int64_t ld_n, int64_t ld_t, int64_t n, int t, int d, const float* W,
                  const float* b, float forget_bias, const float* drop, float* h, int64_t ld_h,
                  float* gates_out, float* c_out, const float* h_init, int64_t ld_hi, const float* c_init,
                  float* c_final, hipStream_t s) {
  const int slots = kBlock / d > 0 ? kBlock / d : 1;
  const int threads = slots * d;
  const int rows_pb = slots * kLstmRowsPerThread;
  const int64_t blocks = (n + rows_pb - 1) / rows_pb;
  if (blocks > INT32_MAX) return fail(SAGNN_ERR_ARG, "grid too large");
  const size_t lds = (size_t)rows_pb * 2 * d * sizeof(float);
  ProfileScope prof(kProfLstm, s, n, t);
  hipLaunchKernelGGL(lstm_fwd_valu_kernel, dim3((unsigned)blocks), dim3(threads), lds, s, x, ld_n, ld_t,
                     n, t, d, W, b, forget_bias, drop, h, ld_h, gates_out, c_out, h_init, ld_hi, c_init, c_final);
  SAGNN_HIP_TRY(hipGetLastError());
  return SAGNN_OK;
}

int mhsa_mean_valu(const float* x, int64_t ld_n, int64_t ld_t, int64_t n, int t, int d, int heads,
                   const float* Wq, const float* bq, const float* Wk, const float* bk,
                   const float* Wv, const float* bv, float* out, int64_t ld_out, hipStream_t s) {
  int slots = kBlock / d > 0 ? kBlock / d : 1;
  while (slots > 1 && (size_t)slots * 4 * t * d * sizeof(float) > 64 * 1024) slots >>= 1;
  const size_t lds = (size_t)slots * 4 * t * d * sizeof(float);
  if (lds > 160 * 1024) return fail(SAGNN_ERR_DIM, "t*d = %d too large for LDS", t * d);
  int64_t blocks = (n + slots - 1) / slots;
  if (blocks > 8192) blocks = 8192;
  ProfileScope prof(kProfMhsa, s, n, t);
  hipLaunchKernelGGL(mhsa_mean_valu_kernel, dim3((unsigned)blocks), dim3(slots * d), lds, s, x, ld_n,
                     ld_t, n, t, d, heads, Wq, bq, Wk, bk, Wv, bv, out, ld_out);
  SAGNN_HIP_TRY(hipGetLastError());
  return SAGNN_OK;
}

}


namespace sagnn {

int mhsa_mean_wide(const float* x, int64_t ld_n, int64_t ld_t, int64_t n, int t, int d, int heads, const float* Wq,
                   const float* bq, const float* Wk, const float* bk, const float* Wv, const float* bv, float* out,
                   int64_t ld_out, float* ws, hipStream_t s) {
  ProfileScope prof(kProfMhsa, s, n, t);
  const int64_t ldq = (int64_t)t * 3 * d;
  for (int ts = 0; ts < t; ++ts) {
    const float* xt = x + (int64_t)ts * ld_t;
    float* qt = ws + (int64_t)ts * 3 * d;
    if (int rc = dense_nn_any(xt, ld_n, n, d, d, Wq, d, bq, qt, ldq, 0, s)) return rc;
    if (int rc = dense_nn_any(xt, ld_n, n, d, d, Wk, d, bk, qt + d, ldq, 0, s)) return rc;
    if (int rc = dense_nn_any(xt, ld_n, n, d, d, Wv, d, bv, qt + 2 * d, ldq, 0, s)) return rc;
  }
  int slots = kBlock / d > 0 ? kBlock / d : 1;
  while (slots > 1 && (size_t)slots * 3 * t * d * sizeof(float) > 64 * 1024) slots >>= 1;
  const size_t lds = (size_t)slots * 3 * t * d * sizeof(float);
  if (lds > 160 * 1024) return fail(SAGNN_ERR_DIM, "t*d = %d too large for LDS", t * d);
  if (int rc = sagnn::ensure_dynamic_lds(reinterpret_cast<const void*>(&attn_mean_from_qkv_kernel), lds)) return rc;
  int64_t blocks = (n + slots - 1) / slots;
  if (blocks > 16384) blocks = 16384;
  hipLaunchKernelGGL(attn_mean_from_qkv_kernel, dim3((unsigned)blocks), dim3(slots * d), lds, s, ws, n, t, d, heads,
                     out, ld_out);
  SAGNN_HIP_TRY(hipGetLastError());
  return SAGNN_OK;
}

}

extern "C" size_t sagnn_mhsa_wide_workspace_bytes(int64_t n, int t, int d) {
  return (n <= 0 || d <= 0 || t <= 0) ? 0 : (size_t)n * (size_t)t * 3 * (size_t)d * sizeof(float);
}

extern "C" int sagnn_mhsa_mean_wide_f32(const float* x, int64_t ld_n, int64_t ld_t, int64_t n, int t, int d,
                                        int heads, const float* Wq, const float* bq, const float* Wk,
                                        const float* bk, const float* Wv, const float* bv, float* out,
                                        int64_t ld_out, void* workspace, size_t workspace_bytes, void* stream) {
  if (int rc = check_dims(n, t, d)) return rc;
  if (!sagnn::wide_supported(d)) return sagnn::fail(SAGNN_ERR_DIM, "d = %d: the wide path needs a multiple of 32", d);
  if (heads < 1 || d % heads) return sagnn::fail(SAGNN_ERR_DIM, "heads = %d does not divide d = %d", heads, d);
  if (!x || !Wq || !bq || !Wk || !bk || !Wv || !bv || !out) return sagnn::fail(SAGNN_ERR_NULL, "null tensor pointer");
  if (int rc = check_strides(ld_n, ld_t, n, t, d)) return rc;
  if ((ld_n & 3) || (ld_t & 3) || !sagnn::aligned16(x)) return sagnn::fail(SAGNN_ERR_ALIGN, "x rows must be 16-byte aligned");
  if (n == 0) return SAGNN_OK;
  if (!workspace || workspace_bytes < sagnn_mhsa_wide_workspace_bytes(n, t, d))
    return sagnn::fail(SAGNN_ERR_WORKSPACE, "mhsa wide workspace needs %zu bytes", sagnn_mhsa_wide_workspace_bytes(n, t, d));
  return sagnn::mhsa_mean_wide(x, ld_n, ld_t, n, t, d, heads, Wq, bq, Wk, bk, Wv, bv, out, ld_out,
                               static_cast<float*>(workspace), static_cast<hipStream_t>(stream));
}

static int lstm_fwd(const float* x, int64_t ld_n, int64_t ld_t, int64_t n, int t, int d, const float* W, const float* b,
                    float forget_bias, const float* drop, float* h, int64_t ld_h, bool train, float* gates, float* cell,
                    const float* h_init, int64_t ld_hi, const float* c_init, float* c_final, void* stream) {
  if (int rc = check_dims(n, t, d)) return rc;
  if (!x || !W || !b || !h || (train && (!gates || !cell))) return sagnn::fail(SAGNN_ERR_NULL, "null tensor pointer");
  if ((h_init == nullptr) != (c_init == nullptr)) return sagnn::fail(SAGNN_ERR_NULL, "give both h_init and c_init or neither");
  if (int rc = check_strides(ld_n, ld_t, n, t, d)) return rc;
  if (ld_h < (int64_t)t * d) return sagnn::fail(SAGNN_ERR_ARG, "ld_h smaller than t*d");
  if (h_init && ld_hi < d) return sagnn::fail(SAGNN_ERR_ARG, "ld_hi smaller than d");
  if (n == 0) return SAGNN_OK;
  const bool vec = sagnn::aligned16(x) && (ld_n & 3) == 0 && (ld_t & 3) == 0 &&
                   (!h_init || (sagnn::aligned16(h_init) && (ld_hi & 3) == 0));
  const bool h_vec = (ld_h & 3) == 0 && sagnn::aligned16(h);
  hipStream_t s = static_cast<hipStream_t>(stream);
  switch (sagnn::select_lstm_fwd(sagnn::calling_engine(), d, t, vec, ld_h, h_vec, train, drop != nullptr,
                                 !drop || sagnn::aligned16(drop))) {
    case sagnn::LstmFwd::F16x2:
      return sagnn::lstm_fwd_f16(x, ld_n, ld_t, n, t, d, W, b, forget_bias, drop, h, ld_h, gates, cell, h_init, ld_hi, c_init,
                                 c_final, s);
    case sagnn::LstmFwd::F32Mfma:
      return sagnn::lstm_fwd_mfma(x, ld_n, ld_t, n, t, d, W, b, forget_bias, drop, h, ld_h, gates, cell, h_init, ld_hi, c_init,
                                  c_final, s);
    case sagnn::LstmFwd::Split128:
      return sagnn::lstm_fwd_split128(x, ld_n, ld_t, n, t, W, b, forget_bias, drop, h, ld_h, gates, cell, h_init, ld_hi, c_init,
                                      c_final, s);
    default:
      return sagnn::lstm_fwd_valu(x, ld_n, ld_t, n, t, d, W, b, forget_bias, drop, h, ld_h, gates, cell, h_init, ld_hi, c_init,
                                  c_final, s);
  }
}

extern "C" int sagnn_lstm_fwd_state_f32(const float* x, int64_t ld_n, int64_t ld_t, int64_t n, int t, int d,
                                        const float* W, const float* b, float forget_bias,
                                        const float* drop_scale, const float* h_init, int64_t ld_hi,
                                        const float* c_init, float* h, int64_t ld_h, float* c_final, void* stream) {
  return lstm_fwd(x, ld_n, ld_t, n, t, d, W, b, forget_bias, drop_scale, h, ld_h, false, nullptr, nullptr, h_init, ld_hi,
                  c_init, c_final, stream);
}

extern "C" int sagnn_lstm_fwd_f32(const float* x, int64_t ld_n, int64_t ld_t, int64_t n, int t, int d,
                                  const float* W, const float* b, float forget_bias,
                                  const float* drop_scale, float* h, int64_t ld_h, void* stream) {
  return lstm_fwd(x, ld_n, ld_t, n, t, d, W, b, forget_bias, drop_scale, h, ld_h, false, nullptr, nullptr, nullptr, 0, nullptr,
                  nullptr, stream);
}

extern "C" int sagnn_lstm_fwd_train_f32(const float* x, int64_t ld_n, int64_t ld_t, int64_t n, int t, int d,
                                        const float* W, const float* b, float forget_bias,
                                        const float* drop_scale, float* h, int64_t ld_h, float* gates,
                                        float* cell, void* stream) {
  return lstm_fwd(x, ld_n, ld_t, n, t, d, W, b, forget_bias, drop_scale, h, ld_h, true, gates, cell, nullptr, 0, nullptr,
                  nullptr, stream);
}

extern "C" int sagnn_layernorm_td_f32(const float* x, int64_t ld_n, int64_t ld_t, int64_t n, int t, int d,
                                      const float* gamma, const float* beta, float eps, float* y,
                                      int64_t ld_y, void* stream) {
  if (int rc = check_dims(n, t, d)) return rc;
  if (!x || !gamma || !beta || !y) return sagnn::fail(SAGNN_ERR_NULL, "null tensor pointer");
  if (int rc = check_strides(ld_n, ld_t, n, t, d)) return rc;
  if (ld_y < (int64_t)t * d) return sagnn::fail(SAGNN_ERR_ARG, "ld_y smaller than t*d");
  if (n == 0) return SAGNN_OK;
  const int64_t blocks = (n + 3) / 4;
  if (blocks > INT32_MAX) return sagnn::fail(SAGNN_ERR_ARG, "grid too large");
  sagnn::ProfileScope prof(sagnn::kProfLayerNorm, static_cast<hipStream_t>(stream), n, t);
  hipLaunchKernelGGL(layernorm_td_kernel, dim3((unsigned)blocks), dim3(kBlock), 0,
                     static_cast<hipStream_t>(stream), x, ld_n, ld_t, n, t, d, gamma, beta, eps, y, ld_y);
  SAGNN_HIP_TRY(hipGetLastError());
  return SAGNN_OK;
}

static bool fused(sagnn::AttnFwd k) { return k == sagnn::AttnFwd::Split || k == sagnn::AttnFwd::F32Mfma; }

static int fused_attention(sagnn::AttnFwd k, const float* x, int64_t ld_n, int64_t ld_t, int64_t n, int t, int d, int heads,
                           const float* gamma, const float* beta, float eps, int apply_ln, const float* Wq, const float* bq,
                           const float* Wk, const float* bk, const float* Wv, const float* bv, float* out, int64_t ld_out,
                           void* stream) {
  const auto launch = k == sagnn::AttnFwd::Split ? sagnn::ln_mhsa_mean_split : sagnn::ln_mhsa_mean_mfma;
  return launch(x, ld_n, ld_t, n, t, d, heads, gamma, beta, eps, apply_ln, Wq, bq, Wk, bk, Wv, bv, out, ld_out,
                static_cast<hipStream_t>(stream));
}

extern "C" int sagnn_mhsa_mean_f32(const float* x, int64_t ld_n, int64_t ld_t, int64_t n, int t, int d, int heads,
                                   const float* Wq, const float* bq, const float* Wk,
                                   const float* bk, const float* Wv, const float* bv, float* out,
                                   int64_t ld_out, void* stream) {
  if (int rc = check_dims(n, t, d)) return rc;
  if (heads < 1 || d % heads) return sagnn::fail(SAGNN_ERR_DIM, "heads = %d does not divide d = %d", heads, d);
  if (!x || !Wq || !bq || !Wk || !bk || !Wv || !bv || !out)
    return sagnn::fail(SAGNN_ERR_NULL, "null tensor pointer");
  if (int rc = check_strides(ld_n, ld_t, n, t, d)) return rc;
  if (ld_out < d) return sagnn::fail(SAGNN_ERR_ARG, "ld_out smaller than d");
  if (n == 0) return SAGNN_OK;
  const bool vec = sagnn::aligned16(x) && (ld_n & 3) == 0 && (ld_t & 3) == 0;
  const sagnn::AttnFwd k = sagnn::select_attn_fwd(sagnn::calling_engine(), d, t, heads, vec);
  if (fused(k))
    return fused_attention(k, x, ld_n, ld_t, n, t, d, heads, nullptr, nullptr, 0.f, 0, Wq, bq, Wk, bk, Wv, bv, out, ld_out,
                           stream);
  return sagnn::mhsa_mean_valu(x, ld_n, ld_t, n, t, d, heads, Wq, bq, Wk, bk, Wv, bv, out, ld_out,
                               static_cast<hipStream_t>(stream));
}

extern "C" size_t sagnn_interval_fusion_workspace_bytes(int64_t n, int t, int d) {
  if (n <= 0 || t <= 0 || d <= 0) return 0;
  size_t bytes = (size_t)n * (size_t)t * (size_t)d * sizeof(float);
  if (sagnn::select_attn_fwd(sagnn::calling_engine(), d, t, 1, false) == sagnn::AttnFwd::Wide)
    bytes += sagnn_mhsa_wide_workspace_bytes(n, t, d);
  return bytes;
}

extern "C" int sagnn_interval_fusion_f32(const float* x, int64_t ld_n, int64_t ld_t, int64_t n, int t,
                                         int d, int heads, const float* lstm_W, const float* lstm_b,
                                         float forget_bias, const float* ln_gamma,
                                         const float* ln_beta, float ln_eps, const float* Wq,
                                         const float* bq, const float* Wk, const float* bk,
                                         const float* Wv, const float* bv, float* out,
                                         int64_t ld_out, void* workspace, size_t workspace_bytes,
                                         void* stream) {
  if (int rc = check_dims(n, t, d)) return rc;
  const size_t need = sagnn_interval_fusion_workspace_bytes(n, t, d);
  if (n > 0 && (!workspace || workspace_bytes < need))
    return sagnn::fail(SAGNN_ERR_WORKSPACE, "fusion workspace needs %zu bytes", need);
  float* h = static_cast<float*>(workspace);
  const int64_t ldw = (int64_t)t * d;
  if (heads < 1 || d % heads) return sagnn::fail(SAGNN_ERR_DIM, "heads = %d does not divide d = %d", heads, d);
  if (!ln_gamma || !ln_beta || !Wq || !bq || !Wk || !bk || !Wv || !bv || !out)
    return sagnn::fail(SAGNN_ERR_NULL, "null tensor pointer");
  if (n == 0) return SAGNN_OK;
  const sagnn::AttnFwd k = sagnn::select_attn_fwd(sagnn::calling_engine(), d, t, heads, true);
  if (int rc = sagnn_lstm_fwd_f32(x, ld_n, ld_t, n, t, d, lstm_W, lstm_b, forget_bias, nullptr, h, ldw, stream)) return rc;
  if (fused(k))
    return fused_attention(k, h, ldw, d, n, t, d, heads, ln_gamma, ln_beta, ln_eps, 1, Wq, bq, Wk, bk, Wv, bv, out, ld_out,
                           stream);
  if (int rc = sagnn_layernorm_td_f32(h, ldw, d, n, t, d, ln_gamma, ln_beta, ln_eps, h, ldw, stream)) return rc;
  if (k == sagnn::AttnFwd::Wide)
    return sagnn_mhsa_mean_wide_f32(h, ldw, d, n, t, d, heads, Wq, bq, Wk, bk, Wv, bv, out, ld_out, h + n * ldw,
                                    workspace_bytes - (size_t)n * ldw * sizeof(float), stream);
  return sagnn_mhsa_mean_f32(h, ldw, d, n, t, d, heads, Wq, bq, Wk, bk, Wv, bv, out, ld_out, stream);
}


extern "C" size_t sagnn_ln_mhsa_mean_workspace_bytes(int64_t n, int t, int d, int heads) {
  if (n <= 0 || t <= 0 || d <= 0) return 0;
  const sagnn::AttnFwd k = sagnn::select_attn_fwd(sagnn::calling_engine(), d, t, heads, true);
  if (fused(k)) return 0;
  size_t bytes = (size_t)n * (size_t)t * (size_t)d * sizeof(float);
  if (k == sagnn::AttnFwd::Wide) bytes += sagnn_mhsa_wide_workspace_bytes(n, t, d);
  return bytes;
}

extern "C" int sagnn_ln_mhsa_mean_f32(const float* x, int64_t ld_n, int64_t ld_t, int64_t n, int t, int d, int heads,
                                      const float* ln_gamma, const float* ln_beta, float ln_eps, const float* Wq,
                                      const float* bq, const float* Wk, const float* bk, const float* Wv,
                                      const float* bv, float* out, int64_t ld_out, void* workspace,
                                      size_t workspace_bytes, void* stream) {
  if (int rc = check_dims(n, t, d)) return rc;
  if (heads < 1 || d % heads) return sagnn::fail(SAGNN_ERR_DIM, "heads = %d does not divide d = %d", heads, d);
  if (!x || !ln_gamma || !ln_beta || !Wq || !bq || !Wk || !bk || !Wv || !bv || !out)
    return sagnn::fail(SAGNN_ERR_NULL, "null tensor pointer");
  if (int rc = check_strides(ld_n, ld_t, n, t, d)) return rc;
  if (ld_out < d) return sagnn::fail(SAGNN_ERR_ARG, "ld_out smaller than d");
  if (n == 0) return SAGNN_OK;
  const bool vec = sagnn::aligned16(x) && (ld_n & 3) == 0 && (ld_t & 3) == 0;
  const sagnn::AttnFwd k = sagnn::select_attn_fwd(sagnn::calling_engine(), d, t, heads, vec);
  if (fused(k))
    return fused_attention(k, x, ld_n, ld_t, n, t, d, heads, ln_gamma, ln_beta, ln_eps, 1, Wq, bq, Wk, bk, Wv, bv, out, ld_out,
                           stream);
  const size_t ybytes = (size_t)n * t * d * sizeof(float);
  size_t need = ybytes + (k == sagnn::AttnFwd::Wide ? sagnn_mhsa_wide_workspace_bytes(n, t, d) : 0);
  if (!workspace || workspace_bytes < need)
    return sagnn::fail(SAGNN_ERR_WORKSPACE, "ln_mhsa_mean workspace needs %zu bytes", need);
  float* y = static_cast<float*>(workspace);
  const int64_t ldw = (int64_t)t * d;
  if (int rc = sagnn_layernorm_td_f32(x, ld_n, ld_t, n, t, d, ln_gamma, ln_beta, ln_eps, y, ldw, stream)) return rc;
  if (k == sagnn::AttnFwd::Wide)
    return sagnn_mhsa_mean_wide_f32(y, ldw, d, n, t, d, heads, Wq, bq, Wk, bk, Wv, bv, out, ld_out, y + n * ldw,
                                    workspace_bytes - ybytes, stream);
  return sagnn_mhsa_mean_f32(y, ldw, d, n, t, d, heads, Wq, bq, Wk, bk, Wv, bv, out, ld_out, stream);
}

extern "C" int sagnn_attn_bwd_front_supported(int d, int t, int heads) {
  const sagnn::Engine e = sagnn::calling_engine();
  return e != sagnn::Engine::Valu && sagnn::select_attn_bwd_front(e, d, t, heads) != sagnn::AttnBwdFront::None;
}

extern "C" int sagnn_attn_bwd_front_f32(const float* x, int64_t ld_n, int64_t ld_t, int64_t n, int t, int d, int heads,
                                        const float* ln_gamma, const float* ln_beta, float ln_eps, int apply_ln,
                                        const float* Wq, const float* bq, const float* Wk, const float* bk,
                                        const float* Wv, const float* bv, const float* g_out, int64_t ld_g,
                                        float* dqkv, float* y_out, void* stream) {
  if (int rc = check_dims(n, t, d)) return rc;
  const sagnn::AttnBwdFront k = sagnn::select_attn_bwd_front(sagnn::calling_engine(), d, t, heads);
  if (k == sagnn::AttnBwdFront::None)
    return sagnn::fail(SAGNN_ERR_DIM, "attn_bwd_front: unsupported d = %d, t = %d, heads = %d", d, t, heads);
  if (!x || !Wq || !bq || !Wk || !bk || !Wv || !bv || !g_out || !dqkv || (apply_ln && (!ln_gamma || !ln_beta)))
    return sagnn::fail(SAGNN_ERR_NULL, "null tensor pointer");
  if (int rc = check_strides(ld_n, ld_t, n, t, d)) return rc;
  if (ld_g < d) return sagnn::fail(SAGNN_ERR_ARG, "ld_g smaller than d");
  if (!sagnn::aligned16(x) || (ld_n & 3) || (ld_t & 3) || !sagnn::aligned16(g_out) || (ld_g & 3) ||
      !sagnn::aligned16(dqkv) || (y_out && !sagnn::aligned16(y_out)))
    return sagnn::fail(SAGNN_ERR_ALIGN, "attn_bwd_front: need 16-byte aligned rows");
  if (n == 0) return SAGNN_OK;
  const auto launch = k == sagnn::AttnBwdFront::Split ? sagnn::attn_bwd_front_split : sagnn::attn_bwd_front_mfma;
  return launch(x, ld_n, ld_t, n, t, d, heads, ln_gamma, ln_beta, ln_eps, apply_ln, Wq, bq, Wk, bk, Wv, bv, g_out, ld_g, dqkv,
                y_out, static_cast<hipStream_t>(stream));
}
```

### sa-gnn_amd/csrc/lstm_f16.hip

```cpp
#include "lstm_f16_kernel.h"

namespace sagnn {

int lstm_fwd_f16(const float* x, int64_t ld_n, int64_t ld_t, int64_t n, int t, int d, const float* W, const float* b,
                 float forget_bias, const float* drop, float* h, int64_t ld_h, float* gates_out, float* c_out,
                 const float* h_init, int64_t ld_hi, const float* c_init, float* c_final, hipStream_t s) {
  const bool save = gates_out != nullptr;
  if (ld_h >= (1 << 22) || (int64_t)t * d >= (1 << 18))
    return fail(SAGNN_ERR_ARG, "f16 LSTM: output row stride must stay below 2^22 floats and t*d below 2^18");
  if (ld_h < (int64_t)t * d) return fail(SAGNN_ERR_ARG, "f16 LSTM: ld_h = %lld < t*d", (long long)ld_h);
  if (save && drop) return fail(SAGNN_ERR_ARG, "f16 LSTM: the training forward takes no dropout mask");
  if (d == 64) return save ? lstm_f16_d64_save(SAGNN_LSTM_F16_PASS) : lstm_f16_d64(SAGNN_LSTM_F16_PASS);
  if (d == 32) return save ? lstm_f16_d32_save(SAGNN_LSTM_F16_PASS) : lstm_f16_d32(SAGNN_LSTM_F16_PASS);
  return fail(SAGNN_ERR_DIM, "f16 LSTM supports d = 32 or 64, got %d", d);
}

}
```

### sa-gnn_amd/csrc/lstm_f16_kernel.h

```cpp
#include <type_traits>
#include <utility>

#pragma once
#include "common.h"
#include "f16_split.h"

namespace {

typedef float f32x4 __attribute__((ext_vector_type(4)));
typedef int i32x4 __attribute__((ext_vector_type(4)));
typedef int i32x2 __attribute__((ext_vector_type(2)));

#ifndef SAGNN_LSTM_F16_BT
#define SAGNN_LSTM_F16_BT 6
#endif
constexpr int kBT = SAGNN_LSTM_F16_BT;
static_assert(kBT % 2 == 0 && kBT >= 4, "x passes ride two per tile on the last kBT / 2 tiles");
constexpr int kRows = 16 * kBT;

template <int D>
__device__ __forceinline__ int swz(int row) {
  if (D == 64) return (row >> 1) & 7;
  const int g = (row >> 2) & 3;
  return (0x78 >> (2 * g)) & 3;
}

template <int LO, class F, int... I>
__device__ __forceinline__ void static_for_impl(F&& f, std::integer_sequence<int, I...>) {
  (f(std::integral_constant<int, LO + I>{}), ...);
}
template <int LO, int HI, class F>
__device__ __forceinline__ void static_for(F&& f) {
  if constexpr (HI > LO) static_for_impl<LO>(static_cast<F&&>(f), std::make_integer_sequence<int, HI - LO>{});
}

constexpr int kGateOps = 118, kXOps = 16;
#include "lstm_f16_schedule.inc"
template <int NM, bool XO>
__host__ __device__ constexpr int sched_start(int i) {
  if (NM == 48) return XO ? kStart48X[i] : kStart48[i];
  if (NM == 24) return XO ? kStart24X[i] : kStart24[i];
  return XO ? kStart12X[i] : kStart12[i];
}
template <int NM, bool XO>
__host__ __device__ constexpr int sched_op(int pos) {
  if (NM == 48) return XO ? kOrder48X[pos] : kOrder48[pos];
  if (NM == 24) return XO ? kOrder24X[pos] : kOrder24[pos];
  return XO ? kOrder12X[pos] : kOrder12[pos];
}

__device__ __forceinline__ void lds_barrier() {
  asm volatile("s_waitcnt lgkmcnt(0)\n\ts_barrier" ::: "memory");
}

__device__ __forceinline__ float sigmoid_e2(float z) {
  return __builtin_amdgcn_rcpf(1.f + __builtin_amdgcn_exp2f(-1.44269504088896340736f * z));
}

template <int D, bool SAVE, bool DROP>
__global__ __launch_bounds__(64 * (D / 16), 1) void lstm_fwd_f16_kernel(
    const float* __restrict__ x, int64_t ld_n, int64_t ld_t, int64_t n, int t, const float* __restrict__ W,
    const float* __restrict__ bias, float forget_bias, const float* __restrict__ drop, float* __restrict__ h_out,
    int64_t ld_h, float* __restrict__ gates_out, float* __restrict__ c_out, int64_t n_tiles,
    const float* __restrict__ h_init, int64_t ld_hi, const float* __restrict__ c_init, float* __restrict__ c_final,
    unsigned int* __restrict__ redo_ctr) {
  constexpr int NW = D / 16;
  constexpr int NT = 64 * NW;
  constexpr int KSH = D / 32;
  constexpr int KS = 2 * KSH;
  constexpr int NC = 4 * D;
  constexpr int PLANE = kRows * D * 2;
  constexpr int LPR = D / 4;
  constexpr int RPP = NT / LPR;
  constexpr int NFILL = kRows / RPP;
  constexpr float kL2E = 1.44269504088896340736f;

  extern __shared__ __attribute__((aligned(16))) char lds[];
  char* const Xp = lds;
  char* const Hp = lds + 4 * PLANE;
  int* const flags = reinterpret_cast<int*>(lds + 8 * PLANE);
  const int tid = threadIdx.x;
  const int lane = tid & 63;
  const int wave = __builtin_amdgcn_readfirstlane(tid >> 6);
  const int m = lane & 15, q = lane >> 4;
  const int hid0 = 16 * wave + 4 * q;
  const int fr = tid / LPR, fc4 = (tid % LPR) * 4;
  float k4096 = 4096.f;
  asm volatile("" : "+v"(k4096));

  if (tid < 3) flags[tid] = 0;
  __syncthreads();

  i32x4 wf[4][KS][2];
  {
    RangeTrack wr = range_init();
#pragma unroll
    for (int g = 0; g < 4; ++g)
#pragma unroll
      for (int ks = 0; ks < KS; ++ks) {
        float wv[8];
#pragma unroll
        for (int j = 0; j < 8; ++j)
          wv[j] = W[(size_t)(32 * ks + 8 * q + j) * NC + g * D + 16 * wave + m] * (g == 1 ? 2.f * kL2E : -kL2E);
        range_seg4(wr, wv[0], wv[1], wv[2], wv[3]);
        range_seg4(wr, wv[4], wv[5], wv[6], wv[7]);
#pragma unroll
        for (int e = 0; e < 4; ++e) {
          const int hd = head2(wv[2 * e], wv[2 * e + 1]);
          wf[g][ks][0][e] = hd;
          wf[g][ks][1][e] = tail_hi(tail_lo(resid<0>(hd, wv[2 * e]), k4096), resid<1>(hd, wv[2 * e + 1]), k4096);
        }
      }
    if (range_bad(wr)) flags[2] = 1;
  }
  f32x4 bc[4];
#pragma unroll
  for (int g = 0; g < 4; ++g)
#pragma unroll
    for (int r = 0; r < 4; ++r) {
      const float b = bias[g * D + hid0 + r] + (g == 2 ? forget_bias : 0.f);
      bc[g][r] = (g == 1 ? 2.f * kL2E : -kL2E) * b;
    }

  auto write_pieces = [&](char* img, int row, int col4, float4 v) {
    const int p0 = head2(v.x, v.y), p1 = head2(v.z, v.w);
    const int s0 = tail_hi(tail_lo(resid<0>(p0, v.x), k4096), resid<1>(p0, v.y), k4096);
    const int s1 = tail_hi(tail_lo(resid<0>(p1, v.z), k4096), resid<1>(p1, v.w), k4096);
    const int off = row * (D * 2) + ((((col4 >> 3)) ^ swz<D>(row)) << 4) + ((col4 >> 2) & 1) * 8;
    *reinterpret_cast<i32x2*>(img + off) = i32x2{p0, p1};
    *reinterpret_cast<i32x2*>(img + PLANE + off) = i32x2{s0, s1};
  };

  int par = 0;
  for (int64_t tile = blockIdx.x; tile < n_tiles; tile += gridDim.x, par ^= 1) {
    const int64_t row0 = tile * kRows;
    const int rows_valid = (int)(n - row0 < kRows ? n - row0 : kRows);
    if (tid == 0) flags[par] = 0;
    RangeTrack xrng = range_init();
    float4 xr[NFILL];
    auto fetch_x = [&](int ts) {
#pragma unroll
      for (int p = 0; p < NFILL; ++p) {
        const int r = p * RPP + fr;
        xr[p] = make_float4(0.f, 0.f, 0.f, 0.f);
        if (r < rows_valid) xr[p] = *reinterpret_cast<const float4*>(x + (row0 + r) * ld_n + (int64_t)ts * ld_t + fc4);
      }
    };
    fetch_x(0);

    const auto rs_h = __builtin_amdgcn_make_buffer_rsrc(h_out + row0 * ld_h, 0, rows_valid * (int)ld_h * 4, 0x00020000);
    const auto rs_g = __builtin_amdgcn_make_buffer_rsrc(SAVE ? gates_out + row0 * t * NC : h_out, 0,
                                                        SAVE ? rows_valid * t * NC * 4 : 0, 0x00020000);
    const auto rs_c = __builtin_amdgcn_make_buffer_rsrc(SAVE ? c_out + row0 * t * D : h_out, 0,
                                                        SAVE ? rows_valid * t * D * 4 : 0, 0x00020000);
    const auto rs_d = __builtin_amdgcn_make_buffer_rsrc(const_cast<float*>(drop ? drop + row0 * t * D : x), 0,
                                                        drop ? rows_valid * t * D * 4 : 0, 0x00020000);
    const auto rs_ci = __builtin_amdgcn_make_buffer_rsrc(const_cast<float*>(c_init ? c_init + row0 * D : x), 0,
                                                         c_init ? rows_valid * D * 4 : 0, 0x00020000);
    const auto rs_cf = __builtin_amdgcn_make_buffer_rsrc(c_final ? c_final + row0 * D : h_out, 0,
                                                         c_final ? rows_valid * D * 4 : 0, 0x00020000);

    f32x4 c[kBT];
#pragma unroll
    for (int bt = 0; bt < kBT; ++bt) {
      c[bt] = f32x4{0.f, 0.f, 0.f, 0.f};
      if (h_init) c[bt] = __builtin_bit_cast(f32x4, __builtin_amdgcn_raw_buffer_load_b128(rs_ci, ((bt * 16 + m) * D + hid0) * 4, 0, 0));
    }
    if (h_init) {
#pragma unroll
      for (int p = 0; p < NFILL; ++p) {
        const int r = p * RPP + fr;
        float4 v = make_float4(0.f, 0.f, 0.f, 0.f);
        if (r < rows_valid) v = *reinterpret_cast<const float4*>(h_init + (row0 + r) * ld_hi + fc4);
        range_seg4_hi(xrng, v.x, v.y, v.z, v.w);
        write_pieces(Hp, r, fc4, v);
      }
    }
#pragma unroll
    for (int p = 0; p < NFILL; ++p) {
      range_seg4(xrng, xr[p].x, xr[p].y, xr[p].z, xr[p].w);
      write_pieces(Xp, p * RPP + fr, fc4, xr[p]);
    }
    lds_barrier();

    auto step = [&](auto recur_c, int ts) {
      constexpr bool RECUR = decltype(recur_c)::value;
      constexpr int KSN = RECUR ? KS : KSH;
      constexpr int NM = 12 * KSN;
      const char* const Xcur = Xp + (ts & 1) * 2 * PLANE;
      const char* const Hcur = Hp + (ts & 1) * 2 * PLANE;
      char* const Hnxt = Hp + ((ts & 1) ^ 1) * 2 * PLANE;
      char* const Xnxt = Xp + ((ts & 1) ^ 1) * 2 * PLANE;
      int m_ = m, q_ = q, fr_ = fr, fc4_ = fc4;
      asm volatile("" : "+v"(m_), "+v"(q_), "+v"(fr_), "+v"(fc4_));
      const int hid = 16 * wave + 4 * q_;

      f32x4 ahi[4], alo[4];
      int xw0[2][2], xw1[2][2], xoff[2];
      float xq[2][4], xs[2];
      uint32_t xsb[2];
      f32x4 ga[4], gl[4];
      f32x4 dv;
      float tt[4][4], pr[4], cn[4], u[4], hn[4], hv[4], r1[4];
      int w0[2], w1[2], hoff;
      i32x4 bf[2][2];

      auto read_b = [&](int bt, int ks, i32x4 (&dst)[2]) {
        const int row = bt * 16 + m_;
        const char* img = ks < KSH ? Xcur : Hcur;
        const int off = row * (D * 2) + ((((ks % KSH) * 4 + q_) ^ swz<D>(row)) << 4);
        dst[0] = *reinterpret_cast<const i32x4*>(img + off);
        dst[1] = *reinterpret_cast<const i32x4*>(img + PLANE + off);
      };
      auto gate_op = [&](auto pb_c, auto k_c) {
        constexpr int PB = decltype(pb_c)::value, K = decltype(k_c)::value;
        const int row = PB * 16 + m_;
        if constexpr (K == 0) {
          const int e_td = (row * t + ts) * D + hid;
          if constexpr (DROP) dv = __builtin_bit_cast(f32x4, __builtin_amdgcn_raw_buffer_load_b128(rs_d, e_td * 4, 0, 0));
        } else if constexpr (K < 17) {
          constexpr int k = K - 1, g = k >> 2, r = k & 3;
          ga[g][r] = fmaf(gl[g][r], kLoInv, ga[g][r]);
        } else if constexpr (K < 33) {
          constexpr int k = K - 17, g = k >> 2, r = k & 3;
          tt[g][r] = __builtin_amdgcn_exp2f(ga[g][r]);
        } else if constexpr (K < 49) {
          constexpr int k = K - 33, g = k >> 2, r = k & 3;
          tt[g][r] = 1.f + tt[g][r];
        } else if constexpr (K < 65) {
          constexpr int k = K - 49, g = k >> 2, r = k & 3;
          tt[g][r] = __builtin_amdgcn_rcpf(tt[g][r]);
        } else if constexpr (K < 69) {
          tt[1][K - 65] = fmaf(-2.f, tt[1][K - 65], 1.f);
        } else if constexpr (K < 73) {
          pr[K - 69] = tt[0][K - 69] * tt[1][K - 69];
        } else if constexpr (K < 77) {
          cn[K - 73] = fmaf(c[PB][K - 73], tt[2][K - 73], pr[K - 73]);
        } else if constexpr (K < 81) {
          u[K - 77] = cn[K - 77] * (2.f * kL2E);
        } else if constexpr (K < 85) {
          u[K - 81] = __builtin_amdgcn_exp2f(u[K - 81]);
        } else if constexpr (K < 89) {
          u[K - 85] = 1.f + u[K - 85];
        } else if constexpr (K < 93) {
          u[K - 89] = __builtin_amdgcn_rcpf(u[K - 89]);
        } else if constexpr (K < 97) {
          u[K - 93] = fmaf(-2.f, u[K - 93], 1.f);
        } else if constexpr (K < 101) {
          hn[K - 97] = u[K - 97] * tt[3][K - 97];
        } else if constexpr (K < 105) {
          if constexpr (DROP) hv[K - 101] = hn[K - 101] * dv[K - 101];
          else hv[K - 101] = hn[K - 101];
        } else if constexpr (K == 105) {
          w0[0] = head2(hn[0], hn[1]);
        } else if constexpr (K == 106) {
          w0[1] = head2(hn[2], hn[3]);
        } else if constexpr (K < 111) {
          constexpr int i = K - 107;
          r1[i] = resid<(i & 1)>(w0[i >> 1], hn[i]);
        } else if constexpr (K == 111) {
          w1[0] = tail_lo(r1[0], k4096);
        } else if constexpr (K == 112) {
          w1[0] = tail_hi(w1[0], r1[1], k4096);
        } else if constexpr (K == 113) {
          w1[1] = tail_lo(r1[2], k4096);
        } else if constexpr (K == 114) {
          w1[1] = tail_hi(w1[1], r1[3], k4096);
          hoff = row * (D * 2) + (((hid >> 3) ^ swz<D>(row)) << 4) + ((hid >> 2) & 1) * 8;
        } else if constexpr (K == 115) {
          *reinterpret_cast<i32x2*>(Hnxt + hoff) = i32x2{w0[0], w0[1]};
          *reinterpret_cast<i32x2*>(Hnxt + PLANE + hoff) = i32x2{w1[0], w1[1]};
        } else if constexpr (K == 116) {
          const i32x4 hvv = {__builtin_bit_cast(int, hv[0]), __builtin_bit_cast(int, hv[1]), __builtin_bit_cast(int, hv[2]),
                             __builtin_bit_cast(int, hv[3])};
          __builtin_amdgcn_raw_buffer_store_b128(hvv, rs_h, (row * (int)ld_h + ts * D + hid) * 4, 0, 0);
          c[PB] = f32x4{cn[0], cn[1], cn[2], cn[3]};
        } else if constexpr (K == 117) {
          if constexpr (SAVE) {
            const int e_td = (row * t + ts) * D + hid;
            const int go_ = (row * t + ts) * NC + hid;
#pragma unroll
            for (int g = 0; g < 4; ++g) {
              const i32x4 gv = {__builtin_bit_cast(int, tt[g][0]), __builtin_bit_cast(int, tt[g][1]),
                                __builtin_bit_cast(int, tt[g][2]), __builtin_bit_cast(int, tt[g][3])};
              __builtin_amdgcn_raw_buffer_store_b128(gv, rs_g, (go_ + g * D) * 4, 0, 0);
            }
            const i32x4 cv = {__builtin_bit_cast(int, cn[0]), __builtin_bit_cast(int, cn[1]), __builtin_bit_cast(int, cn[2]),
                              __builtin_bit_cast(int, cn[3])};
            __builtin_amdgcn_raw_buffer_store_b128(cv, rs_c, e_td * 4, 0, 0);
          }
        } else {
          constexpr int PS = (K - kGateOps) / kXOps;
          constexpr int XP = 2 * (PB - (kBT - 1 - kBT / 2)) + PS;
          constexpr int X = (K - kGateOps) % kXOps;
          const float xv[4] = {xr[XP].x, xr[XP].y, xr[XP].z, xr[XP].w};
          const int xrow = XP * RPP + fr_;
          if constexpr (X == 0) {
            xw0[PS][0] = head2(xv[0], xv[1]);
          } else if constexpr (X == 1) {
            xw0[PS][1] = head2(xv[2], xv[3]);
          } else if constexpr (X < 6) {
            constexpr int i = X - 2;
            xq[PS][i] = resid<(i & 1)>(xw0[PS][i >> 1], xv[i]);
          } else if constexpr (X == 6) {
            xw1[PS][0] = tail_lo(xq[PS][0], k4096);
          } else if constexpr (X == 7) {
            xw1[PS][0] = tail_hi(xw1[PS][0], xq[PS][1], k4096);
          } else if constexpr (X == 8) {
            xw1[PS][1] = tail_lo(xq[PS][2], k4096);
          } else if constexpr (X == 9) {
            xw1[PS][1] = tail_hi(xw1[PS][1], xq[PS][3], k4096);
          } else if constexpr (X == 10) {
            xs[PS] = maxabs3(xv[0], xv[1], xv[2]);
          } else if constexpr (X == 11) {
            xs[PS] = maxabs_acc(xs[PS], xv[3]);
            xoff[PS] = xrow * (D * 2) + (((fc4_ >> 3) ^ swz<D>(xrow)) << 4) + ((fc4_ >> 2) & 1) * 8;
          } else if constexpr (X == 12) {
            xrng.hi = maxabs_acc(xrng.hi, xs[PS]);
          } else if constexpr (X == 13) {
            xsb[PS] = __builtin_bit_cast(uint32_t, xs[PS]) - 1u;
          } else if constexpr (X == 14) {
            xrng.lo = xsb[PS] < xrng.lo ? xsb[PS] : xrng.lo;
          } else {
            *reinterpret_cast<i32x2*>(Xnxt + xoff[PS]) = i32x2{xw0[PS][0], xw0[PS][1]};
            *reinterpret_cast<i32x2*>(Xnxt + PLANE + xoff[PS]) = i32x2{xw1[PS][0], xw1[PS][1]};
          }
        }
      };
      auto slot = [&](auto bt_c, auto i_c) {
        constexpr int BT = decltype(bt_c)::value, I = decltype(i_c)::value;
        constexpr int ks = I / 12, term = (I % 12) / 4, g = I % 4;
        constexpr int cur = (BT * KSN + ks) & 1;
        if constexpr (I % 12 == 0) {
          if constexpr (ks + 1 < KSN) read_b(BT, ks + 1, bf[cur ^ 1]);
          else if constexpr (BT + 1 < kBT) read_b(BT + 1, 0, bf[cur ^ 1]);
        }
        if constexpr (term == 0) {
          const f32x4 cin = ks == 0 ? f32x4{0.f, 0.f, 0.f, 0.f} : alo[g];
          alo[g] = __builtin_amdgcn_mfma_f32_16x16x32_f16(__builtin_bit_cast(f16x8, wf[g][ks][1]),
                                                          __builtin_bit_cast(f16x8, bf[cur][0]), cin, 0, 0, 0);
        } else if constexpr (term == 1) {
          alo[g] = __builtin_amdgcn_mfma_f32_16x16x32_f16(__builtin_bit_cast(f16x8, wf[g][ks][0]),
                                                          __builtin_bit_cast(f16x8, bf[cur][1]), alo[g], 0, 0, 0);
        } else {
          const f32x4 cin = ks == 0 ? bc[g] : ahi[g];
          ahi[g] = __builtin_amdgcn_mfma_f32_16x16x32_f16(__builtin_bit_cast(f16x8, wf[g][ks][0]),
                                                          __builtin_bit_cast(f16x8, bf[cur][0]), cin, 0, 0, 0);
        }
        if constexpr (BT > 0) {
          constexpr bool XO = BT >= kBT - kBT / 2;
          constexpr int lo = sched_start<NM, XO>(I), hi = sched_start<NM, XO>(I + 1);
          static_for<lo, hi>([&](auto pos_c) {
            gate_op(std::integral_constant<int, BT - 1>{}, std::integral_constant<int, sched_op<NM, XO>(decltype(pos_c)::value)>{});
          });
        }
        __builtin_amdgcn_sched_barrier(0);
      };
      auto tile_fn = [&](auto bt_c) {
        static_for<0, NM>([&](auto i_c) { slot(bt_c, i_c); });
#pragma unroll
        for (int g = 0; g < 4; ++g) ga[g] = ahi[g], gl[g] = alo[g];
      };
      read_b(0, 0, bf[0]);
      static_for<0, kBT>(tile_fn);
      static_for<0, kGateOps>([&](auto pos_c) {
        gate_op(std::integral_constant<int, kBT - 1>{}, std::integral_constant<int, kOrder48[decltype(pos_c)::value]>{});
      });
    };

    for (int ts = 0; ts < t; ++ts) {
      if (ts + 1 < t) fetch_x(ts + 1);
      if (ts > 0 || h_init != nullptr) step(std::true_type{}, ts);
      else step(std::false_type{}, ts);
      if (ts + 1 < t) lds_barrier();
    }
    if (range_bad(xrng)) flags[par] = 1;
    lds_barrier();
    const bool redo = (flags[par] | flags[2]) != 0;
    if (c_final && !redo) {
#pragma unroll
      for (int bt = 0; bt < kBT; ++bt)
        __builtin_amdgcn_raw_buffer_store_b128(__builtin_bit_cast(i32x4, c[bt]), rs_cf, ((bt * 16 + m) * D + hid0) * 4, 0, 0);
    }
    if (redo) {
      if (tid == 0 && redo_ctr) atomicAdd(redo_ctr, 1u);
      __syncthreads();
      float* const hs = reinterpret_cast<float*>(lds);
      float* const cs = hs + 2 * kRows * D;
      float* const xs = cs + kRows * D;
      for (int idx = tid; idx < kRows * D; idx += NT) {
        const int r = idx / D, uu = idx - r * D;
        const bool live = r < rows_valid;
        hs[idx] = (h_init && live) ? h_init[(row0 + r) * ld_hi + uu] : 0.f;
        cs[idx] = (c_init && live) ? c_init[(row0 + r) * D + uu] : 0.f;
      }
      constexpr int RSTEP = NT / D, RPT = kRows / RSTEP;
      static_assert(NT % D == 0 && kRows % RSTEP == 0, "one hidden unit per thread");
      const int uu = tid % D, r0 = tid / D;
      for (int ts = 0; ts < t; ++ts) {
        const float* const hc = hs + (ts & 1) * kRows * D;
        float* const hnx = hs + ((ts & 1) ^ 1) * kRows * D;
        __syncthreads();
        for (int idx = tid; idx < kRows * D; idx += NT) {
          const int r = idx / D, c_ = idx - r * D;
          xs[idx] = r < rows_valid ? x[(row0 + r) * ld_n + (int64_t)ts * ld_t + c_] : 0.f;
        }
        __syncthreads();
        float a[RPT][4];
#pragma unroll
        for (int j = 0; j < RPT; ++j)
#pragma unroll
          for (int g = 0; g < 4; ++g) a[j][g] = bias[g * D + uu] + (g == 2 ? forget_bias : 0.f);
        for (int half = 0; half < 2; ++half) {
          const float* const src = half ? hc : xs;
          for (int k = 0; k < D; k += 4) {
            float w[4][4];
#pragma unroll
            for (int kk = 0; kk < 4; ++kk)
#pragma unroll
              for (int g = 0; g < 4; ++g) w[kk][g] = W[(size_t)(half * D + k + kk) * NC + g * D + uu];
#pragma unroll
            for (int j = 0; j < RPT; ++j) {
              const float4 v = *reinterpret_cast<const float4*>(src + (r0 + j * RSTEP) * D + k);
              const float vv[4] = {v.x, v.y, v.z, v.w};
#pragma unroll
              for (int kk = 0; kk < 4; ++kk)
#pragma unroll
                for (int g = 0; g < 4; ++g) a[j][g] = fmaf(vv[kk], w[kk][g], a[j][g]);
            }
          }
        }
#pragma unroll
        for (int j = 0; j < RPT; ++j) {
          const int r = r0 + j * RSTEP, idx = r * D + uu;
          const float gi = sigmoid_e2(a[j][0]), gj = tanhf(a[j][1]), gf = sigmoid_e2(a[j][2]), go = sigmoid_e2(a[j][3]);
          const float cnew = fmaf(cs[idx], gf, gi * gj);
          const float hnew = tanhf(cnew) * go;
          cs[idx] = cnew;
          hnx[idx] = hnew;
          if (r < rows_valid) {
            const int64_t e_td = ((row0 + r) * t + ts) * D + uu;
            h_out[(row0 + r) * ld_h + (int64_t)ts * D + uu] = DROP ? hnew * drop[e_td] : hnew;
            if constexpr (SAVE) {
              float* const gp = gates_out + ((row0 + r) * t + ts) * NC + uu;
              gp[0] = gi, gp[D] = gj, gp[2 * D] = gf, gp[3 * D] = go;
              c_out[e_td] = cnew;
            }
          }
        }
      }
      __syncthreads();
      if (c_final)
        for (int idx = tid; idx < rows_valid * D; idx += NT) c_final[row0 * D + idx] = cs[idx];
      __syncthreads();
    }
  }
}

}

namespace sagnn {

template <int D, bool SAVE, bool DROP>
int launch_lstm_f16(const float* x, int64_t ld_n, int64_t ld_t, int64_t n, int t, const float* W, const float* b,
                    float forget_bias, const float* drop, float* h, int64_t ld_h, float* gates_out, float* c_out,
                    const float* h_init, int64_t ld_hi, const float* c_init, float* c_final, hipStream_t s) {
  const size_t lds = (size_t)8 * kRows * D * 2 + 16;
  if (int rc = ensure_dynamic_lds(reinterpret_cast<const void*>(&lstm_fwd_f16_kernel<D, SAVE, DROP>), lds)) return rc;
  const int per_cu = D == 64 ? 1 : 2;
  const int64_t n_tiles = (n + kRows - 1) / kRows;
  const int64_t want = (int64_t)cu_count_current() * per_cu;
  const int64_t blocks = n_tiles < want ? n_tiles : want;
  ProfileScope prof(kProfLstm, s, n, t);
  hipLaunchKernelGGL((lstm_fwd_f16_kernel<D, SAVE, DROP>), dim3((unsigned)blocks), dim3(64 * (D / 16)), lds, s, x, ld_n, ld_t,
                     n, t, W, b, forget_bias, drop, h, ld_h, gates_out, c_out, n_tiles, h_init, ld_hi, c_init, c_final, redo_counter());
  SAGNN_HIP_TRY(hipGetLastError());
  return SAGNN_OK;
}

#define SAGNN_LSTM_F16_ARGS                                                                                       \
  const float *x, int64_t ld_n, int64_t ld_t, int64_t n, int t, const float *W, const float *b, float forget_bias, \
      const float *drop, float *h, int64_t ld_h, float *gates_out, float *c_out, const float *h_init, int64_t ld_hi, \
      const float *c_init, float *c_final, hipStream_t s
#define SAGNN_LSTM_F16_PASS x, ld_n, ld_t, n, t, W, b, forget_bias, drop, h, ld_h, gates_out, c_out, h_init, ld_hi, c_init, c_final, s
int lstm_f16_d64(SAGNN_LSTM_F16_ARGS);
int lstm_f16_d64_save(SAGNN_LSTM_F16_ARGS);
int lstm_f16_d32(SAGNN_LSTM_F16_ARGS);
int lstm_f16_d32_save(SAGNN_LSTM_F16_ARGS);

}
```

### sa-gnn_amd/ops.py

```python
from __future__ import annotations

import ctypes

import numpy as np
import torch

from . import _lib
from ._lib import PlanInfo, Tuning, check

SUPPORTED_D = tuple(range(4, 257, 4))

ENGINES = {"f16x2": 0, "f32": 1, "valu": 2}


def set_engine(name: str) -> None:
    check(_lib.load().sagnn_set_engine(ENGINES[name]))


def get_engine() -> str:
    code = _lib.load().sagnn_get_engine()
    return next(k for k, v in ENGINES.items() if v == code)


def range_redo_count(reset: bool = False) -> int:
    n = ctypes.c_int64(0)
    check(_lib.load().sagnn_range_redo_count(ctypes.byref(n), 1 if reset else 0))
    return int(n.value)


class engine:

    def __init__(self, name: str):
        self.name = name

    def __enter__(self):
        self.prev = get_engine()
        set_engine(self.name)
        return self

    def __exit__(self, *exc):
        set_engine(self.prev)
        return False


def _stream() -> int:
    return torch._C._cuda_getCurrentRawStream(torch.cuda.current_device())


def _ptr(t: torch.Tensor | None) -> int | None:
    return None if t is None else t.data_ptr()


def _f32_rows(name: str, t: torch.Tensor | None, d: int, rows: int | None = None):
    if t is None:
        return 0
    if t.dtype != torch.float32 or not t.is_cuda:
        raise TypeError(f"{name}: expected a float32 device tensor, got {t.dtype} on {t.device}")
    if t.dim() != 2 or t.shape[1] != d or t.stride(1) != 1:
        raise ValueError(f"{name}: expected shape [rows, {d}] with unit inner stride, got "
                         f"{tuple(t.shape)} strides {t.stride()}")
    if rows is not None and t.shape[0] != rows:
        raise ValueError(f"{name}: expected {rows} rows, got {t.shape[0]}")
    return t.stride(0) if t.shape[0] > 1 else max(t.stride(0), d)


class SpmmPlan:

    def __init__(self, rowptr, colidx, n_rows: int, n_src: int, device=None,
                 tuning: tuple[int, int, int] | None = None, validate: bool = True):
        lib = _lib.load()
        self._lib = lib
        self._h = ctypes.c_void_p()
        self.n_rows, self.n_src = int(n_rows), int(n_src)
        rp_t = torch.as_tensor(rowptr)
        ci_t = torch.as_tensor(colidx)
        if rp_t.dtype != torch.int32 or ci_t.dtype != torch.int32:
            raise TypeError("rowptr/colidx must be int32")
        if rp_t.numel() != self.n_rows + 1:
            raise ValueError(f"rowptr has {rp_t.numel()} entries, expected n_rows+1 = {self.n_rows + 1}")
        self.nnz = int(ci_t.numel())
        rp_h = rp_t.cpu().contiguous()
        self._rowptr_host = rp_h.numpy()
        if validate:
            ci_h = ci_t.cpu().contiguous()
            check(lib.sagnn_csr_check_host(rp_h.data_ptr(), ci_h.data_ptr(), self.n_rows, self.n_src,
                                           self.nnz))
        tun = None
        if tuning is not None:
            tun = Tuning(int(tuning[0]), int(tuning[1]), int(tuning[2]), 0)
        if device is None:
            self.rowptr = self.colidx = None
            d_rp = d_ci = None
        else:
            self.rowptr = rp_t.to(device).contiguous()
            self.colidx = ci_t.to(device).contiguous()
            if self.colidx.numel() == 0:
                self.colidx = torch.zeros(1, dtype=torch.int32, device=device)
            d_rp, d_ci = self.rowptr.data_ptr(), self.colidx.data_ptr()
        check(lib.sagnn_spmm_plan_create(rp_h.data_ptr(), d_rp, d_ci, self.n_rows, self.n_src,
                                         self.nnz, ctypes.byref(tun) if tun else None,
                                         ctypes.byref(self._h)))
        info = PlanInfo()
        check(lib.sagnn_spmm_plan_get_info(self._h, ctypes.byref(info)))
        self.info = info
        self.device = device
        self._ws: dict[int, torch.Tensor] = {}
        self.partner_adjoint: SpmmPlan | None = None

    def __del__(self):
        h = getattr(self, "_h", None)
        if h is not None and h.value:
            self._lib.sagnn_spmm_plan_destroy(h)
            self._h = None

    @property
    def handle(self):
        return self._h

    def chunks(self):
        n = int(self.info.n_chunks)
        rows = np.empty(n, np.int32)
        e0 = np.empty(n, np.int32)
        e1 = np.empty(n, np.int32)
        check(self._lib.sagnn_spmm_plan_copy_chunks(self._h, rows.ctypes.data, e0.ctypes.data,
                                                    e1.ctypes.data, n))
        return rows, e0, e1

    def workspace_bytes(self, d: int) -> int:
        return int(self._lib.sagnn_spmm_workspace_bytes(self._h, int(d)))

    def workspace(self, d: int) -> torch.Tensor | None:
        need = self.workspace_bytes(d)
        if need == 0:
            return None
        ws = self._ws.get(d)
        if ws is None:
            ws = torch.empty(need // 4, dtype=torch.float32, device=self.device)
            self._ws[d] = ws
        return ws


def spmm(plan: SpmmPlan, x: torch.Tensor, leaky: float, residual: torch.Tensor | None = None,
         out: torch.Tensor | None = None, acc_in: torch.Tensor | None = None,
         acc_out: torch.Tensor | None = None, want_out: bool = True) -> torch.Tensor | None:
    d = int(x.shape[1])
    ldx = _f32_rows("x", x, d, plan.n_src)
    if out is None and want_out:
        out = torch.empty((plan.n_rows, d), dtype=torch.float32, device=x.device)
    ldr = _f32_rows("residual", residual, d, plan.n_rows)
    ldo = _f32_rows("out", out, d, plan.n_rows)
    ldai = _f32_rows("acc_in", acc_in, d, plan.n_rows)
    ldao = _f32_rows("acc_out", acc_out, d, plan.n_rows)
    ws = plan.workspace(d)
    check(plan._lib.sagnn_spmm_f32(plan.handle, _ptr(x), ldx, d, _ptr(residual), ldr, float(leaky),
                                   _ptr(out), ldo, _ptr(acc_in), ldai, _ptr(acc_out), ldao,
                                   _ptr(ws), 0 if ws is None else ws.numel() * 4, _stream()))
    return out


def spmm_ex(plan: SpmmPlan, x: torch.Tensor | None, leaky: float, residual=None, out=None, acc_in=None, acc_out=None,
            acc_in2=None, mask_out=None, mask_in=None, out2=None, slope2: float = 1.0, want_out: bool = False):
    ref = next(t_ for t_ in (x, residual, out, acc_out, out2) if t_ is not None)
    d = int(ref.shape[1])
    if out is None and want_out:
        out = torch.empty((plan.n_rows, d), dtype=torch.float32, device=ref.device)
    e = _lib.SpmmEpilogue()
    e.leaky, e.slope2 = float(leaky), float(slope2)
    e.residual, e.ldr = _ptr(residual), _f32_rows("residual", residual, d, plan.n_rows)
    e.out, e.ldo = _ptr(out), _f32_rows("out", out, d, plan.n_rows)
    e.acc_in, e.ld_acc_in = _ptr(acc_in), _f32_rows("acc_in", acc_in, d, plan.n_rows)
    e.acc_out, e.ld_acc_out = _ptr(acc_out), _f32_rows("acc_out", acc_out, d, plan.n_rows)
    e.acc_in2, e.ld_acc_in2 = _ptr(acc_in2), _f32_rows("acc_in2", acc_in2, d, plan.n_rows)
    e.out2, e.ldo2 = _ptr(out2), _f32_rows("out2", out2, d, plan.n_rows)
    for name, m in (("mask_out", mask_out), ("mask_in", mask_in)):
        if m is not None:
            _masks(name, m, (plan.n_rows, d // 4))
    e.mask_out, e.mask_in = _ptr(mask_out), _ptr(mask_in)
    ldx = _f32_rows("x", x, d, plan.n_src) if x is not None else d
    ws = plan.workspace(d)
    check(plan._lib.sagnn_spmm_ex_f32(plan.handle, _ptr(x), ldx, d, ctypes.byref(e), _ptr(ws), 0 if ws is None else ws.numel() * 4,
                                      _stream()))
    return out


def mask_scale(g: torch.Tensor, mask: torch.Tensor, slope: float, out: torch.Tensor):
    rows, d = int(g.shape[0]), int(g.shape[1])
    _masks("mask", mask, (rows, d // 4))
    check(_lib.load().sagnn_mask_scale_f32(_ptr(g), _f32_rows("g", g, d, rows), _ptr(mask), float(slope), _ptr(out),
                                           _f32_rows("out", out, d, rows), rows, d, _stream()))
    return out


def _interval_ws(plan_user: SpmmPlan, plan_item: SpmmPlan, d: int):
    wu, wi = plan_user.workspace(d), plan_item.workspace(d)
    return wu if (wi is None or (wu is not None and wu.numel() >= wi.numel())) else wi


def _scratch(name: str, s: torch.Tensor | None, k: int, rows: int, d: int, device):
    if s is None:
        return torch.empty(k * rows * d, dtype=torch.float32, device=device)
    if s.dtype != torch.float32 or not s.is_contiguous() or s.numel() < k * rows * d:
        raise ValueError(f"{name}: need a contiguous float32 buffer of {k}*{rows}*{d} elements")
    return s


def _masks(name: str, m: torch.Tensor, shape: tuple):
    if m.dtype != torch.uint8 or not m.is_contiguous() or m.numel() != int(np.prod(shape)):
        raise ValueError(f"{name}: need a contiguous uint8 tensor {list(shape)}")
    return m


def _adjoint_pair(plan_user: SpmmPlan, plan_item: SpmmPlan):
    adj_u, adj_i = plan_user.partner_adjoint, plan_item.partner_adjoint
    if (adj_u is None) != (adj_i is None):
        raise ValueError("give the exact adjoint of both plans or of neither")
    if adj_u is not None:
        return adj_u, adj_i
    if plan_user.nnz != plan_item.nnz:
        raise ValueError(f"plans are not a transposed pair (nnz {plan_user.nnz} vs {plan_item.nnz}: duplicated stored "
                         "entries?) — build them with graph.interval_pair, which adds the exact adjoints")
    return plan_user, plan_item


def gnn_interval(plan_user: SpmmPlan, plan_item: SpmmPlan, u0: torch.Tensor, i0: torch.Tensor,
                 n_layers: int, leaky: float, user_out: torch.Tensor, item_out: torch.Tensor,
                 scratch_u: torch.Tensor | None = None, scratch_i: torch.Tensor | None = None,
                 mask_u: torch.Tensor | None = None, mask_i: torch.Tensor | None = None):
    d = int(u0.shape[1])
    U, I = plan_user.n_rows, plan_item.n_rows
    ld_u0 = _f32_rows("u0", u0, d, U)
    ld_i0 = _f32_rows("i0", i0, d, I)
    ld_uo = _f32_rows("user_out", user_out, d, U)
    ld_io = _f32_rows("item_out", item_out, d, I)
    if n_layers > 1:
        scratch_u = _scratch("scratch_u", scratch_u, 2, U, d, u0.device)
        scratch_i = _scratch("scratch_i", scratch_i, 2, I, d, u0.device)
    if mask_u is not None:
        _masks("mask_u", mask_u, (n_layers, U, d // 4))
    if mask_i is not None:
        _masks("mask_i", mask_i, (n_layers, I, d // 4))
    ws = _interval_ws(plan_user, plan_item, d)
    check(plan_user._lib.sagnn_gnn_interval_ex_f32(
        plan_user.handle, plan_item.handle, _ptr(u0), ld_u0, _ptr(i0), ld_i0, d, int(n_layers),
        float(leaky), _ptr(scratch_u), _ptr(scratch_i), _ptr(user_out), ld_uo, _ptr(item_out), ld_io,
        _ptr(mask_u), _ptr(mask_i), _ptr(ws), 0 if ws is None else ws.numel() * 4, _stream()))
    return user_out, item_out


def gnn_interval_bwd(plan_user: SpmmPlan, plan_item: SpmmPlan, grad_user_out: torch.Tensor,
                     grad_item_out: torch.Tensor, n_layers: int, leaky: float, mask_u: torch.Tensor,
                     mask_i: torch.Tensor, grad_u0: torch.Tensor | None = None,
                     grad_i0: torch.Tensor | None = None, scratch_u: torch.Tensor | None = None,
                     scratch_i: torch.Tensor | None = None):
    d = int(grad_user_out.shape[1])
    U, I = plan_user.n_rows, plan_item.n_rows
    plan_user, plan_item = _adjoint_pair(plan_user, plan_item)
    ld_gu = _f32_rows("grad_user_out", grad_user_out, d, U)
    ld_gi = _f32_rows("grad_item_out", grad_item_out, d, I)
    dev = grad_user_out.device
    if grad_u0 is None:
        grad_u0 = torch.empty((U, d), dtype=torch.float32, device=dev)
    if grad_i0 is None:
        grad_i0 = torch.empty((I, d), dtype=torch.float32, device=dev)
    ld_du = _f32_rows("grad_u0", grad_u0, d, U)
    ld_di = _f32_rows("grad_i0", grad_i0, d, I)
    scratch_u = _scratch("scratch_u", scratch_u, 4, U, d, dev)
    scratch_i = _scratch("scratch_i", scratch_i, 4, I, d, dev)
    _masks("mask_u", mask_u, (n_layers, U, d // 4))
    _masks("mask_i", mask_i, (n_layers, I, d // 4))
    ws = _interval_ws(plan_user, plan_item, d)
    check(plan_user._lib.sagnn_gnn_interval_bwd_f32(
        plan_user.handle, plan_item.handle, _ptr(grad_user_out), ld_gu, _ptr(grad_item_out), ld_gi, d,
        int(n_layers), float(leaky), _ptr(mask_u), _ptr(mask_i), _ptr(scratch_u), _ptr(scratch_i),
        _ptr(grad_u0), ld_du, _ptr(grad_i0), ld_di, _ptr(ws), 0 if ws is None else ws.numel() * 4, _stream()))
    return grad_u0, grad_i0


class SpmmBatch:

    def __init__(self, plans_user, plans_item):
        if len(plans_user) != len(plans_item) or not plans_user:
            raise ValueError("one user-side and one item-side plan per interval")
        self.plans_user, self.plans_item = list(plans_user), list(plans_item)
        self.T, self.U, self.I = len(plans_user), plans_user[0].n_rows, plans_item[0].n_rows
        self.device = plans_user[0].device
        self._lib = _lib.load()
        self._h = ctypes.c_void_p()
        PU = (ctypes.c_void_p * self.T)(*[p.handle for p in self.plans_user])
        PI = (ctypes.c_void_p * self.T)(*[p.handle for p in self.plans_item])
        check(self._lib.sagnn_spmm_batch_create(PU, PI, self.T, ctypes.byref(self._h)))
        self.nnz = sum(p.nnz for p in self.plans_user) + sum(p.nnz for p in self.plans_item)
        self._ws: dict[int, torch.Tensor] = {}
        self._adjoint: SpmmBatch | None = None

    def __del__(self):
        h = getattr(self, "_h", None)
        if h is not None and h.value:
            self._lib.sagnn_spmm_batch_destroy(h)
            self._h = None

    @property
    def handle(self):
        return self._h

    def workspace(self, d: int):
        need = int(self._lib.sagnn_spmm_batch_workspace_bytes(self._h, int(d)))
        if need == 0:
            return None
        ws = self._ws.get(d)
        if ws is None:
            ws = torch.empty(need // 4, dtype=torch.float32, device=self.device)
            self._ws[d] = ws
        return ws

    def adjoint(self) -> "SpmmBatch":
        pairs = [_adjoint_pair(pu, pi) for pu, pi in zip(self.plans_user, self.plans_item)]
        if all(adj_u is pu for (adj_u, _), pu in zip(pairs, self.plans_user)):
            return self
        if self._adjoint is None:
            self._adjoint = SpmmBatch([a for a, _ in pairs], [a for _, a in pairs])
        return self._adjoint


def _slab(name: str, x: torch.Tensor, T: int, rows: int, d: int):
    if x.dtype != torch.float32 or not x.is_cuda or x.dim() != 3 or tuple(x.shape) != (T, rows, d) or x.stride(2) != 1:
        raise ValueError(f"{name}: expected a float32 device tensor indexed [{T}, {rows}, {d}] with unit feature stride, "
                         f"got {tuple(x.shape)} strides {x.stride()}")
    ld = int(x.stride(1)) if rows > 1 else max(int(x.stride(1)), d)
    slab = int(x.stride(0)) if T > 1 else 0
    return ld, slab


def gnn_stack(batch: SpmmBatch, u0: torch.Tensor, i0: torch.Tensor, n_layers: int, leaky: float,
              user_out: torch.Tensor, item_out: torch.Tensor, scratch_u: torch.Tensor | None = None,
              scratch_i: torch.Tensor | None = None, mask_u: torch.Tensor | None = None, mask_i: torch.Tensor | None = None):
    T, U, I = batch.T, batch.U, batch.I
    d = int(u0.shape[2])
    ld_u0, sl_u0 = _slab("u0", u0, T, U, d)
    ld_i0, sl_i0 = _slab("i0", i0, T, I, d)
    ld_uo, sl_uo = _slab("user_out", user_out, T, U, d)
    ld_io, sl_io = _slab("item_out", item_out, T, I, d)
    if n_layers > 1:
        scratch_u = _scratch("scratch_u", scratch_u, 2 * T, U, d, u0.device)
        scratch_i = _scratch("scratch_i", scratch_i, 2 * T, I, d, u0.device)
    if mask_u is not None:
        _masks("mask_u", mask_u, (T, n_layers, U, d // 4))
    if mask_i is not None:
        _masks("mask_i", mask_i, (T, n_layers, I, d // 4))
    ws = batch.workspace(d)
    check(batch._lib.sagnn_gnn_stack_f32(batch.handle, _ptr(u0), ld_u0, sl_u0, _ptr(i0), ld_i0, sl_i0, d, int(n_layers),
                                         float(leaky), _ptr(scratch_u), _ptr(scratch_i), _ptr(user_out), ld_uo, sl_uo,
                                         _ptr(item_out), ld_io, sl_io, _ptr(mask_u), _ptr(mask_i), _ptr(ws),
                                         0 if ws is None else ws.numel() * 4, _stream()))
    return user_out, item_out


def gnn_stack_bwd(batch: SpmmBatch, grad_user_out: torch.Tensor, grad_item_out: torch.Tensor, n_layers: int, leaky: float,
                  mask_u: torch.Tensor, mask_i: torch.Tensor, grad_u0: torch.Tensor, grad_i0: torch.Tensor,
                  scratch_u: torch.Tensor | None = None, scratch_i: torch.Tensor | None = None):
    adj = batch.adjoint()
    T, U, I = batch.T, batch.U, batch.I
    d = int(grad_user_out.shape[2])
    ld_gu, sl_gu = _slab("grad_user_out", grad_user_out, T, U, d)
    ld_gi, sl_gi = _slab("grad_item_out", grad_item_out, T, I, d)
    ld_du, sl_du = _slab("grad_u0", grad_u0, T, U, d)
    ld_di, sl_di = _slab("grad_i0", grad_i0, T, I, d)
    dev = grad_user_out.device
    scratch_u = _scratch("scratch_u", scratch_u, 4 * T, U, d, dev)
    scratch_i = _scratch("scratch_i", scratch_i, 4 * T, I, d, dev)
    _masks("mask_u", mask_u, (T, n_layers, U, d // 4))
    _masks("mask_i", mask_i, (T, n_layers, I, d // 4))
    ws = adj.workspace(d)
    check(adj._lib.sagnn_gnn_stack_bwd_f32(adj.handle, _ptr(grad_user_out), ld_gu, sl_gu, _ptr(grad_item_out), ld_gi, sl_gi, d,
                                           int(n_layers), float(leaky), _ptr(mask_u), _ptr(mask_i), _ptr(scratch_u),
                                           _ptr(scratch_i), _ptr(grad_u0), ld_du, sl_du, _ptr(grad_i0), ld_di, sl_di, _ptr(ws),
                                           0 if ws is None else ws.numel() * 4, _stream()))
    return grad_u0, grad_i0


def _ntd(name: str, x: torch.Tensor, dense_td: bool = False):
    if x.dtype != torch.float32 or not x.is_cuda or x.dim() != 3:
        raise TypeError(f"{name}: expected a float32 device tensor indexed [n, t, d]")
    n, t, d = (int(v) for v in x.shape)
    if x.stride(2) != 1:
        raise ValueError(f"{name}: the feature axis must have unit stride")
    ld_n = int(x.stride(0)) if n > 1 else max(int(x.stride(0)), d)
    ld_t = int(x.stride(1)) if t > 1 else max(int(x.stride(1)), d)
    if dense_td and ld_t != d:
        raise ValueError(f"{name}: the (t, d) block of each node must be contiguous")
    return n, t, d, ld_n, ld_t


def _vec(name: str, v: torch.Tensor, numel: int):
    if v.dtype != torch.float32 or not v.is_cuda or not v.is_contiguous() or v.numel() != numel:
        raise ValueError(f"{name}: expected a contiguous float32 device tensor of {numel} elements")
    return v.data_ptr()


def _wide(d: int) -> bool:
    return d % 32 == 0 and d not in (32, 64) and _lib.load().sagnn_get_engine() != ENGINES["valu"]


def lstm_fwd(x: torch.Tensor, W: torch.Tensor, b: torch.Tensor, forget_bias: float = 1.0,
             drop_scale: torch.Tensor | None = None, out: torch.Tensor | None = None,
             h0: torch.Tensor | None = None, c0: torch.Tensor | None = None, c_out: torch.Tensor | None = None):
    n, t, d, ld, ldt = _ntd("x", x)
    if out is None:
        out = torch.empty((n, t, d), dtype=torch.float32, device=x.device)
    _, _, _, ldh, _ = _ntd("out", out, dense_td=True)
    if drop_scale is not None and (not drop_scale.is_contiguous() or drop_scale.shape != x.shape):
        raise ValueError("drop_scale must be contiguous [n, t, d]")
    if (h0 is None) != (c0 is None):
        raise ValueError("give both h0 and c0 or neither")
    ld_hi = 0
    if h0 is not None:
        ld_hi = _f32_rows("h0", h0, d, n)
        if _f32_rows("c0", c0, d, n) != d:
            raise ValueError("c0 must be contiguous [n, d]")
    if c_out is not None and _f32_rows("c_out", c_out, d, n) != d:
        raise ValueError("c_out must be contiguous [n, d]")
    lib = _lib.load()
    check(lib.sagnn_lstm_fwd_state_f32(x.data_ptr(), ld, ldt, n, t, d, _vec("W", W, 8 * d * d),
                                       _vec("b", b, 4 * d), float(forget_bias), _ptr(drop_scale), _ptr(h0), ld_hi,
                                       _ptr(c0), out.data_ptr(), ldh, _ptr(c_out), _stream()))
    return out


def layernorm_td(x: torch.Tensor, gamma: torch.Tensor, beta: torch.Tensor, eps: float = 1e-12,
                 out: torch.Tensor | None = None):
    n, t, d, ld, ldt = _ntd("x", x)
    if out is None:
        out = torch.empty((n, t, d), dtype=torch.float32, device=x.device)
    _, _, _, ldy, _ = _ntd("out", out, dense_td=True)
    check(_lib.load().sagnn_layernorm_td_f32(x.data_ptr(), ld, ldt, n, t, d, _vec("gamma", gamma, d),
                                             _vec("beta", beta, d), float(eps), out.data_ptr(), ldy,
                                             _stream()))
    return out


def mhsa_mean(x: torch.Tensor, Wq, bq, Wk, bk, Wv, bv, heads: int, out: torch.Tensor | None = None):
    n, t, d, ld, ldt = _ntd("x", x)
    if out is None:
        out = torch.empty((n, d), dtype=torch.float32, device=x.device)
    ldo = _f32_rows("out", out, d, n)
    lib = _lib.load()
    if _wide(d):
        ws = torch.empty(int(lib.sagnn_mhsa_wide_workspace_bytes(n, t, d)) // 4, dtype=torch.float32, device=x.device)
        check(lib.sagnn_mhsa_mean_wide_f32(
            x.data_ptr(), ld, ldt, n, t, d, int(heads), _vec("Wq", Wq, d * d), _vec("bq", bq, d),
            _vec("Wk", Wk, d * d), _vec("bk", bk, d), _vec("Wv", Wv, d * d), _vec("bv", bv, d),
            out.data_ptr(), ldo, ws.data_ptr(), ws.numel() * 4, _stream()))
        return out
    check(lib.sagnn_mhsa_mean_f32(
        x.data_ptr(), ld, ldt, n, t, d, int(heads), _vec("Wq", Wq, d * d), _vec("bq", bq, d),
        _vec("Wk", Wk, d * d), _vec("bk", bk, d), _vec("Wv", Wv, d * d), _vec("bv", bv, d),
        out.data_ptr(), ldo, _stream()))
    return out


def ln_mhsa_mean(x: torch.Tensor, gamma, beta, Wq, bq, Wk, bk, Wv, bv, heads: int, eps: float = 1e-12):
    n, t, d, ld, ldt = _ntd("x", x)
    out = torch.empty((n, d), dtype=torch.float32, device=x.device)
    lib = _lib.load()
    need = int(lib.sagnn_ln_mhsa_mean_workspace_bytes(n, t, d, int(heads)))
    ws = torch.empty(need // 4, dtype=torch.float32, device=x.device) if need else None
    check(lib.sagnn_ln_mhsa_mean_f32(
        x.data_ptr(), ld, ldt, n, t, d, int(heads), _vec("gamma", gamma, d), _vec("beta", beta, d), float(eps),
        _vec("Wq", Wq, d * d), _vec("bq", bq, d), _vec("Wk", Wk, d * d), _vec("bk", bk, d), _vec("Wv", Wv, d * d),
        _vec("bv", bv, d), out.data_ptr(), d, _ptr(ws), need, _stream()))
    return out


def interval_fusion(x: torch.Tensor, p: dict, heads: int, out: torch.Tensor | None = None,
                    workspace: torch.Tensor | None = None):
    lib = _lib.load()
    n, t, d, ld, ldt = _ntd("x", x)
    if out is None:
        out = torch.empty((n, d), dtype=torch.float32, device=x.device)
    ldo = _f32_rows("out", out, d, n)
    need = int(lib.sagnn_interval_fusion_workspace_bytes(n, t, d))
    if workspace is None or workspace.numel() * workspace.element_size() < need:
        workspace = torch.empty(max(need // 4, 1), dtype=torch.float32, device=x.device)
    check(lib.sagnn_interval_fusion_f32(
        x.data_ptr(), ld, ldt, n, t, d, int(heads), _vec("lstm_W", p["lstm_W"], 8 * d * d),
        _vec("lstm_b", p["lstm_b"], 4 * d), 1.0, _vec("ln_gamma", p["ln_gamma"], d),
        _vec("ln_beta", p["ln_beta"], d), 1e-12, _vec("Wq", p["Wq"], d * d), _vec("bq", p["bq"], d),
        _vec("Wk", p["Wk"], d * d), _vec("bk", p["bk"], d), _vec("Wv", p["Wv"], d * d),
        _vec("bv", p["bv"], d), out.data_ptr(), ldo, workspace.data_ptr(),
        workspace.numel() * workspace.element_size(), _stream()))
    return out


def dense_nn(x: torch.Tensor, W: torch.Tensor, bias: torch.Tensor | None = None, out: torch.Tensor | None = None,
             accumulate: bool = False):
    n, din = int(x.shape[0]), int(x.shape[1])
    dout = int(W.shape[1])
    ldx = _f32_rows("x", x, din)
    if out is None:
        out = torch.empty((n, dout), dtype=torch.float32, device=x.device)
    ldy = _f32_rows("out", out, dout, n)
    check(_lib.load().sagnn_dense_nn_f32(x.data_ptr(), ldx, n, din, dout, _vec("W", W, din * dout),
                                         None if bias is None else _vec("bias", bias, dout), out.data_ptr(), ldy,
                                         int(accumulate), _stream()))
    return out


def dense_tn(x: torch.Tensor, g: torch.Tensor, dW: torch.Tensor, db: torch.Tensor | None = None):
    n, din = int(x.shape[0]), int(x.shape[1])
    dout = int(g.shape[1])
    ldx = _f32_rows("x", x, din)
    ldg = _f32_rows("g", g, dout, n)
    check(_lib.load().sagnn_dense_tn_f32(x.data_ptr(), ldx, g.data_ptr(), ldg, n, din, dout,
                                         _vec("dW", dW, din * dout), None if db is None else _vec("db", db, dout),
                                         _stream()))
    return dW


def dense_tn_seg(x: torch.Tensor, g: torch.Tensor, dW: torch.Tensor, db: torch.Tensor | None = None):
    if x.dim() != 3 or g.dim() != 3 or x.shape[:2] != g.shape[:2]:
        raise ValueError(f"dense_tn_seg: need x [s, n, din] and g [s, n, dout], got {tuple(x.shape)} / {tuple(g.shape)}")
    for name, v in (("x", x), ("g", g)):
        if v.dtype != torch.float32 or not v.is_cuda or v.stride(2) != 1:
            raise ValueError(f"dense_tn_seg: {name} must be float32 on the GPU with unit column stride")
    s_, n, din = (int(v) for v in x.shape)
    dout = int(g.shape[2])
    if s_ == 0 or n == 0:
        return dW
    check(_lib.load().sagnn_dense_tn_seg_f32(x.data_ptr(), int(x.stride(1)), int(x.stride(0)), g.data_ptr(), int(g.stride(1)),
                                             int(g.stride(0)), n, s_, din, dout, _vec("dW", dW, din * dout),
                                             None if db is None else _vec("db", db, dout), _stream()))
    return dW


def mul(a: torch.Tensor, b: torch.Tensor, out: torch.Tensor | None = None):
    if out is None:
        out = torch.empty_like(a)
    for name, x in (("a", a), ("b", b), ("out", out)):
        if x.dtype != torch.float32 or not x.is_contiguous() or x.numel() != a.numel():
            raise ValueError(f"{name}: need contiguous float32 tensors of equal size")
    check(_lib.load().sagnn_mul_f32(a.data_ptr(), b.data_ptr(), out.data_ptr(), a.numel(), _stream()))
    return out


class Adam:

    def __init__(self, params: dict, lr: float, decay: float = 1.0, decay_step: int = 1, reg: float = 0.0,
                 reg_names=(), beta1: float = 0.9, beta2: float = 0.999, eps: float = 1e-8):
        self.params = params
        self.lr0, self.decay, self.decay_step, self.reg = lr, decay, max(int(decay_step), 1), reg
        self.reg_names = set(reg_names)
        self.b1, self.b2, self.eps = beta1, beta2, eps
        self.m = {k: torch.zeros_like(v) for k, v in params.items()}
        self.v = {k: torch.zeros_like(v) for k, v in params.items()}
        self.global_step = 0

    def learning_rate(self) -> float:
        return self.lr0 * self.decay ** (self.global_step // self.decay_step)

    def step(self, grads: dict):
        lr = self.learning_rate()
        self.global_step += 1
        names, keep = [], []
        for k, g in grads.items():
            if g is None and not (k in self.reg_names and self.reg != 0.0):
                continue
            p = self.params[k]
            if not p.is_contiguous():
                raise ValueError(f"parameter {k!r} must be contiguous")
            if g is not None:
                g = g.contiguous()
                if g.numel() != p.numel() or g.dtype != torch.float32:
                    raise ValueError(f"gradient of {k!r}: expected {p.numel()} float32 elements")
                keep.append(g)
            names.append((k, g))
        n = len(names)
        if n == 0:
            return
        P, G, M, V = ((ctypes.c_void_p * n)() for _ in range(4))
        C, L2 = (ctypes.c_int64 * n)(), (ctypes.c_float * n)()
        for i, (k, g) in enumerate(names):
            p = self.params[k]
            P[i], G[i], M[i], V[i] = p.data_ptr(), (None if g is None else g.data_ptr()), self.m[k].data_ptr(), self.v[k].data_ptr()
            C[i], L2[i] = p.numel(), (self.reg if k in self.reg_names else 0.0)
        check(_lib.load().sagnn_adam_multi_f32(n, P, G, M, V, C, L2, lr, self.b1, self.b2, self.eps, self.global_step,
                                               _stream()))

    def state_dict(self) -> dict:
        out = {"global_step": torch.tensor(self.global_step, dtype=torch.int64)}
        for k in self.params:
            out["m/" + k] = self.m[k].detach().cpu()
            out["v/" + k] = self.v[k].detach().cpu()
        return out

    def load_state_dict(self, state: dict):
        want = {"global_step"} | {"m/" + k for k in self.params} | {"v/" + k for k in self.params}
        if set(state) != want:
            raise KeyError(f"optimizer state keys differ: missing {sorted(want - set(state))[:4]}, "
                           f"unexpected {sorted(set(state) - want)[:4]}")
        for k in self.params:
            for slot, name in ((self.m, "m/"), (self.v, "v/")):
                if tuple(state[name + k].shape) != tuple(slot[k].shape):
                    raise ValueError(f"optimizer slot {name + k}: shape {tuple(state[name + k].shape)} != {tuple(slot[k].shape)}")
                slot[k].copy_(state[name + k])
        self.global_step = int(state["global_step"])


def leaky_add(a: torch.Tensor, b: torch.Tensor | None, leaky: float, out: torch.Tensor | None = None):
    if out is None:
        out = torch.empty_like(a)
    for name, x in (("a", a), ("b", b), ("out", out)):
        if x is not None and (x.dtype != torch.float32 or not x.is_contiguous() or x.numel() != a.numel()):
            raise ValueError(f"{name}: need contiguous float32 tensors of equal size")
    check(_lib.load().sagnn_leaky_add_f32(a.data_ptr(), _ptr(b), out.data_ptr(), float(leaky), a.numel(), _stream()))
    return out


def pair_score(U: torch.Tensor, I: torch.Tensor, uids: torch.Tensor, iids: torch.Tensor, S: torch.Tensor | None = None,
               A: torch.Tensor | None = None, locs: torch.Tensor | None = None, leaky: float = 1.0):
    d = int(U.shape[1])
    n = int(uids.numel())
    out = torch.empty(n, dtype=torch.float32, device=U.device)
    for name, x in (("uids", uids), ("iids", iids), ("locs", locs)):
        if x is not None and (x.dtype != torch.int32 or not x.is_contiguous() or x.numel() != n):
            raise ValueError(f"{name}: need a contiguous int32 tensor of {n} elements")
    check(_lib.load().sagnn_pair_score_f32(
        U.data_ptr(), _f32_rows("U", U, d), I.data_ptr(), _f32_rows("I", I, d), _ptr(S),
        0 if S is None else _f32_rows("S", S, d), _ptr(A), 0 if A is None else _f32_rows("A", A, d),
        uids.data_ptr(), iids.data_ptr(), _ptr(locs), float(leaky), out.data_ptr(), n, d, _stream()))
    return out


_topk_ws: dict = {}


def _topk_workspace(device: torch.device, nbytes: int) -> torch.Tensor:
    ws = _topk_ws.get(device)
    if ws is None or ws.numel() < nbytes:
        ws = _topk_ws[device] = torch.empty(max(nbytes, 256), dtype=torch.uint8, device=device)
    return ws


def check_exclusions(rowptr, items, n_rows: int, n_items: int):
    as_np = lambda v: v.detach().cpu().numpy() if isinstance(v, torch.Tensor) else np.asarray(v)
    rp, it = as_np(rowptr).astype(np.int64).reshape(-1), as_np(items).astype(np.int64).reshape(-1)
    if rp.size != n_rows + 1 or rp[0] != 0 or rp[-1] != it.size:
        raise ValueError(f"excl rowptr: need {n_rows + 1} entries from 0 to len(items) = {it.size}")
    if (np.diff(rp) < 0).any():
        raise ValueError("excl rowptr: not monotone")
    if it.size and (it.min() < 0 or it.max() >= n_items):
        raise ValueError(f"excl items: ids outside [0, {n_items})")
    row = np.repeat(np.arange(n_rows), np.diff(rp))
    if ((np.diff(it) < 0) & (row[1:] == row[:-1])).any():
        raise ValueError("excl items: ids must be ascending within a row")
    return rp.astype(np.int32), it.astype(np.int32)


class ExclusionCSR:

    def __init__(self, rowptr, items, n_rows: int, n_items: int, device):
        rp, it = check_exclusions(rowptr, items, n_rows, n_items)
        self.n_rows, self.n_items = int(n_rows), int(n_items)
        self.rowptr = torch.from_numpy(rp).to(device)
        self.items = torch.from_numpy(it).to(device) if it.size else torch.zeros(1, dtype=torch.int32, device=device)

    def rows(self, lo: int, hi: int) -> "ExclusionCSR":
        lo, hi = int(lo), int(hi)
        if not 0 <= lo <= hi <= self.n_rows:
            raise ValueError(f"rows [{lo}, {hi}) outside [0, {self.n_rows})")
        view = ExclusionCSR.__new__(ExclusionCSR)
        view.n_rows, view.n_items = hi - lo, self.n_items
        view.rowptr, view.items = self.rowptr[lo:hi + 1], self.items
        return view


def score_topk(Q: torch.Tensor, I: torch.Tensor, k: int, excl=None, target=None):
    lib = _lib.load()
    if Q.dim() != 2:
        raise ValueError(f"Q: expected [B, d], got {tuple(Q.shape)}")
    B, d = int(Q.shape[0]), int(Q.shape[1])
    n_items = int(I.shape[0]) if I.dim() == 2 else 0
    pre = isinstance(excl, ExclusionCSR)
    if pre and (excl.n_rows != B or excl.n_items != n_items):
        raise ValueError(f"excl: an ExclusionCSR of {excl.n_rows} rows over {excl.n_items} items, "
                         f"Q has {B} rows and I {n_items} items")
    ex = None if (excl is None or pre) else check_exclusions(excl[0], excl[1], B, n_items)
    ldq, ldi = _f32_rows("Q", Q, d), _f32_rows("I", I, d)
    dev = Q.device
    if I.device != dev:
        raise ValueError(f"I on {I.device}, Q on {dev}")
    rp_d = it_d = tg_d = rank = None
    if pre:
        if excl.rowptr.device != dev:
            raise ValueError(f"excl on {excl.rowptr.device}, Q on {dev}")
        rp_d, it_d = excl.rowptr, excl.items
    elif ex is not None:
        rp, it = ex
        rp_d = torch.from_numpy(rp).to(dev)
        it_d = torch.from_numpy(it).to(dev) if it.size else torch.zeros(1, dtype=torch.int32, device=dev)
    if target is not None:
        tg_d = torch.as_tensor(target, device=dev)
        if tg_d.dtype != torch.int32 or tg_d.dim() != 1 or tg_d.numel() != B or not tg_d.is_contiguous():
            raise ValueError(f"target: need a contiguous int32 vector of {B} elements")
        rank = torch.empty(B, dtype=torch.int64, device=dev)
    items = torch.empty((B, int(k)), dtype=torch.int32, device=dev)
    scores = torch.empty((B, int(k)), dtype=torch.float32, device=dev)
    need = int(lib.sagnn_score_topk_workspace_bytes(B, n_items, d, int(k)))
    ws = _topk_workspace(dev, need) if need else None
    check(lib.sagnn_score_topk_f32(Q.data_ptr(), ldq, I.data_ptr(), ldi, B, n_items, d, int(k), _ptr(rp_d), _ptr(it_d),
                                   _ptr(tg_d), items.data_ptr(), scores.data_ptr(), _ptr(rank), _ptr(ws), need, _stream()))
    return items, scores, rank


def candidate_rank(U: torch.Tensor, I: torch.Tensor, uids: torch.Tensor, cand: torch.Tensor, target: torch.Tensor,
                   S: torch.Tensor | None = None, A: torch.Tensor | None = None, leaky: float = 1.0,
                   want_scores: bool = False):
    d = int(U.shape[1])
    if cand.dim() != 2 or cand.dtype != torch.int32 or not cand.is_cuda or cand.stride(1) != 1:
        raise ValueError("cand: need an int32 device matrix [B, C] with unit inner stride")
    B, C = int(cand.shape[0]), int(cand.shape[1])
    ldc = cand.stride(0) if B > 1 else C
    cand_ptr = cand.data_ptr() if cand.numel() else _idx_ptr("cand", cand.new_zeros(0), torch.int32)
    dev = U.device
    rank = torch.empty(B, dtype=torch.int64, device=dev)
    scores = torch.empty((B, C), dtype=torch.float32, device=dev) if want_scores else None
    check(_lib.load().sagnn_candidate_rank_f32(
        U.data_ptr(), _f32_rows("U", U, d), I.data_ptr(), _f32_rows("I", I, d), _ptr(S),
        0 if S is None else _f32_rows("S", S, d, B), _ptr(A), 0 if A is None else _f32_rows("A", A, d),
        _idx_ptr("uids", uids, torch.int32, B), cand_ptr, ldc,
        _idx_ptr("target", target, torch.int32, B), float(leaky), B, C, d, _idx_ptr("rank", rank, torch.int64),
        _ptr(scores), C, _stream()))
    return rank, scores


_empty_ptrs: dict = {}


def _idx_ptr(name: str, t: torch.Tensor, dtype, numel: int | None = None) -> int:
    if not isinstance(t, torch.Tensor) or t.dtype != dtype or not t.is_cuda or not t.is_contiguous():
        raise TypeError(f"{name}: expected a contiguous {dtype} device tensor")
    if numel is not None and t.numel() != numel:
        raise ValueError(f"{name}: expected {numel} elements, got {t.numel()}")
    if t.numel():
        return t.data_ptr()
    buf = _empty_ptrs.get(t.device)
    if buf is None:
        buf = _empty_ptrs[t.device] = torch.zeros(4, dtype=torch.int32, device=t.device)
    return buf.data_ptr()


def _out(n: int, dtype, device) -> torch.Tensor:
    return torch.empty(max(int(n), 1), dtype=dtype, device=device)[:int(n)]


def sample_train(bat_ids: torch.Tensor, n_slots: int, seq_ptr: torch.Tensor, seq_items: torch.Tensor,
                 ban_ptr: torch.Tensor, ban_items: torch.Tensor, n_items: int, train_sample_num: int, pred_num: int,
                 pos_length: int, pair_off: torch.Tensor, n_pairs: int, seed: int, step: int):
    B, U = int(bat_ids.numel()), int(seq_ptr.numel()) - 1
    dev = bat_ids.device
    uids, iids, locs = (_out(2 * n_pairs, torch.int32, dev) for _ in range(3))
    seg_begin, seg_len = _out(n_slots, torch.int64, dev), _out(n_slots, torch.int32, dev)
    check(_lib.load().sagnn_sample_train_i32(
        _idx_ptr("bat_ids", bat_ids, torch.int32), B, int(n_slots), _idx_ptr("seq_ptr", seq_ptr, torch.int64),
        _idx_ptr("seq_items", seq_items, torch.int32), _idx_ptr("ban_ptr", ban_ptr, torch.int64, U + 1),
        _idx_ptr("ban_items", ban_items, torch.int32), U, int(n_items), int(train_sample_num), int(pred_num),
        int(pos_length), _idx_ptr("pair_off", pair_off, torch.int64, B), int(n_pairs), int(seed), int(step),
        _idx_ptr("uids", uids, torch.int32), _idx_ptr("iids", iids, torch.int32), _idx_ptr("uLocs_seq", locs, torch.int32),
        _idx_ptr("seg_begin", seg_begin, torch.int64), _idx_ptr("seg_len", seg_len, torch.int32), _stream()))
    return uids, iids, locs, seg_begin, seg_len


def sample_ssl(bat_ids: torch.Tensor, sub_ptr: torch.Tensor, sub_items: torch.Tensor, ssl_num: int,
               ssl_off: torch.Tensor, n_out: int, seed: int, step: int):
    T, B = int(sub_ptr.shape[0]), int(bat_ids.numel())
    U = int(sub_ptr.shape[1]) - 1
    dev = bat_ids.device
    uids, iids, locs = (_out(n_out, torch.int32, dev) for _ in range(3))
    check(_lib.load().sagnn_sample_ssl_i32(
        _idx_ptr("bat_ids", bat_ids, torch.int32), B, T, _idx_ptr("sub_ptr", sub_ptr, torch.int64),
        _idx_ptr("sub_items", sub_items, torch.int32), U, int(ssl_num), _idx_ptr("ssl_off", ssl_off, torch.int64, T * B),
        int(n_out), int(seed), int(step), _idx_ptr("uids", uids, torch.int32), _idx_ptr("iids", iids, torch.int32),
        _idx_ptr("uLocs_seq", locs, torch.int32), _stream()))
    return uids, iids, locs


def seq_sum(fi: torch.Tensor, pos_embed: torch.Tensor, seq_items: torch.Tensor, seg_begin: torch.Tensor,
            seg_len: torch.Tensor):
    d, P, n = int(fi.shape[1]), int(pos_embed.shape[0]), int(seg_len.numel())
    seq_tok = torch.empty((n, d), dtype=torch.float32, device=fi.device)
    pos_tok = torch.empty((n, d), dtype=torch.float32, device=fi.device)
    check(_lib.load().sagnn_seq_sum_f32(
        fi.data_ptr(), _f32_rows("fi", fi, d), int(fi.shape[0]), pos_embed.data_ptr(), _f32_rows("pos_embed", pos_embed, d),
        P, _idx_ptr("seq_items", seq_items, torch.int32), int(seq_items.numel()),
        _idx_ptr("seg_begin", seg_begin, torch.int64, n), _idx_ptr("seg_len", seg_len, torch.int32), n, d,
        seq_tok.data_ptr(), pos_tok.data_ptr(), d, _stream()))
    return seq_tok, pos_tok


def seq_sum_bwd(g_seq: torch.Tensor, g_pos: torch.Tensor, seq_items: torch.Tensor, seg_begin: torch.Tensor,
                seg_len: torch.Tensor, n_items: int, pos_length: int):
    n, d = int(seg_len.numel()), int(g_seq.shape[1])
    ld = _f32_rows("g_seq", g_seq, d, n)
    if _f32_rows("g_pos", g_pos, d, n) != ld:
        raise ValueError("g_seq and g_pos need the same row stride")
    d_fi = torch.zeros((int(n_items), d), dtype=torch.float32, device=g_seq.device)
    d_pos = torch.empty((int(pos_length), d), dtype=torch.float32, device=g_seq.device)
    check(_lib.load().sagnn_seq_sum_bwd_f32(
        g_seq.data_ptr(), g_pos.data_ptr(), ld, _idx_ptr("seq_items", seq_items, torch.int32), int(seq_items.numel()),
        _idx_ptr("seg_begin", seg_begin, torch.int64, n), _idx_ptr("seg_len", seg_len, torch.int32), n, int(pos_length), d,
        d_fi.data_ptr(), d, int(n_items), d_pos.data_ptr(), d, _stream()))
    return d_fi, d_pos


def _flags(name: str, flags: torch.Tensor) -> int:
    if flags.dtype != torch.uint8 or not flags.is_cuda or not flags.is_contiguous() or flags.dim() != 1:
        raise TypeError(f"{name}: expected a contiguous uint8 device vector")
    return flags.data_ptr() if flags.numel() else _idx_ptr(name, flags.new_zeros(0, dtype=torch.int32), torch.int32)


def rows_mark(ids: torch.Tensor, flags: torch.Tensor):
    check(_lib.load().sagnn_rows_mark_i32(_idx_ptr("ids", ids, torch.int32), int(ids.numel()), int(flags.numel()),
                                          _flags("flags", flags), _stream()))


def rows_mark_segments(seq_items: torch.Tensor, seg_begin: torch.Tensor, seg_len: torch.Tensor, max_len: int,
                       flags: torch.Tensor):
    n = int(seg_len.numel())
    check(_lib.load().sagnn_rows_mark_seg_i32(
        _idx_ptr("seq_items", seq_items, torch.int32), int(seq_items.numel()), _idx_ptr("seg_begin", seg_begin, torch.int64, n),
        _idx_ptr("seg_len", seg_len, torch.int32), n, int(max_len), int(flags.numel()), _flags("flags", flags), _stream()))


def rows_compact(flags: torch.Tensor, cap: int, rows: torch.Tensor | None = None, count: torch.Tensor | None = None):
    n, dev = int(flags.numel()), flags.device
    if rows is None:
        rows = _out(cap, torch.int32, dev)
    if count is None:
        count = torch.empty(1, dtype=torch.int32, device=dev)
    lib = _lib.load()
    need = int(lib.sagnn_rows_compact_workspace_bytes(n))
    ws = torch.empty(max(need // 4, 1), dtype=torch.int32, device=dev)
    check(lib.sagnn_rows_compact_i32(_flags("flags", flags), n, _idx_ptr("rows", rows, torch.int32, int(cap)), int(cap),
                                     _idx_ptr("count", count, torch.int32, 1), ws.data_ptr(), ws.numel() * 4, _stream()))
    return rows, count


def rows_gather(x: torch.Tensor, rows: torch.Tensor, count: torch.Tensor | None = None, out: torch.Tensor | None = None):
    flat = x.dim() == 2
    xv = x.unsqueeze(1) if flat else x
    N, t, d, ld_n, ld_t = _ntd("x", xv)
    cap = int(rows.numel())
    if out is None:
        out = torch.empty((cap, d) if flat else (cap, t, d), dtype=torch.float32, device=x.device)
    if not out.is_contiguous() or out.numel() != cap * t * d:
        raise ValueError("out: expected a contiguous tensor of cap * t * d elements")
    if cap == 0:
        return out
    check(_lib.load().sagnn_rows_gather_f32(
        x.data_ptr(), ld_n, ld_t, N, t, d, _idx_ptr("rows", rows, torch.int32), cap,
        None if count is None else _idx_ptr("count", count, torch.int32, 1), out.data_ptr(), _stream()))
    return out


def rows_scatter(src: torch.Tensor, rows: torch.Tensor, count: torch.Tensor, out: torch.Tensor):
    flat = out.dim() == 2
    ov = out.unsqueeze(1) if flat else out
    N, t, d, ld_n, ld_t = _ntd("out", ov)
    cap = int(rows.numel())
    if not src.is_contiguous() or src.dtype != torch.float32 or src.numel() != cap * t * d:
        raise ValueError("src: expected a contiguous float32 tensor of cap * t * d elements")
    if cap == 0:
        return out
    check(_lib.load().sagnn_rows_scatter_f32(
        src.data_ptr(), _idx_ptr("rows", rows, torch.int32), cap, _idx_ptr("count", count, torch.int32, 1), t, d,
        out.data_ptr(), ld_n, ld_t, N, _stream()))
    return out
```

Baseline: 18.02 billion.

## Pass LSTM hidden state to split attention as packed f16 hi/lo pairs

Adds a packed path for d = 64 under the f16x2 engine: the LSTM writes h directly as f16 hi plus scaled lo halves, and the split attention kernel consumes them without re-converting. LayerNorm is folded into the QKV weights (gamma into W, beta into the bias) and applied as a per-row scale and shift after the MFMA, so the separate normalise-and-pack pass over the tile goes away. The cost is an extra precomputation pass over the weights and a range guard on mean times rstd. The new entry points are only reached through new API functions, so the SpMM metric is probably unaffected.

```diff
diff --git a/include/sagnn.h b/include/sagnn.h
--- a/include/sagnn.h
+++ b/include/sagnn.h
@@ -135,6 +135,14 @@
 int sagnn_layernorm_td_f32(const float* x, int64_t ld_n, int64_t ld_t, int64_t n, int t, int d,
                            const float* gamma, const float* beta, float eps, float* y,
                            int64_t ld_y, void* stream);
+int sagnn_fusion_packed_supported(int d, int t, int heads);
+int sagnn_lstm_fwd_packed_f32(const float* x, int64_t ld_n, int64_t ld_t, int64_t n, int t, int d, const float* W,
+                              const float* b, float forget_bias, const void* h_init_packed, int64_t ld_hi,
+                              const float* c_init, void* h_packed, int64_t ld_h, float* c_final, void* stream);
+int sagnn_ln_mhsa_mean_packed_f32(const void* h_packed, int64_t ld_n, int64_t ld_t, int64_t n, int t, int d, int heads,
+                                  const float* ln_gamma, const float* ln_beta, float ln_eps, const float* Wq,
+                                  const float* bq, const float* Wk, const float* bk, const float* Wv, const float* bv,
+                                  float* out, int64_t ld_out, void* stream);
 int sagnn_mhsa_mean_f32(const float* x, int64_t ld_n, int64_t ld_t, int64_t n, int t, int d, int heads,
                         const float* Wq, const float* bq, const float* Wk, const float* bk,
                         const float* Wv, const float* bv, float* out, int64_t ld_out,
diff --git a/sa-gnn_amd/_lib.py b/sa-gnn_amd/_lib.py
--- a/sa-gnn_amd/_lib.py
+++ b/sa-gnn_amd/_lib.py
@@ -135,6 +135,12 @@
                                    c_float, c_void_p, c_void_p, c_int64, c_void_p]),
     "sagnn_lstm_fwd_state_f32": (c_int, [c_void_p, c_int64, c_int64, c_int64, c_int, c_int, c_void_p, c_void_p, c_float,
                                          c_void_p, c_void_p, c_int64, c_void_p, c_void_p, c_int64, c_void_p, c_void_p]),
+    "sagnn_fusion_packed_supported": (c_int, [c_int, c_int, c_int]),
+    "sagnn_lstm_fwd_packed_f32": (c_int, [c_void_p, c_int64, c_int64, c_int64, c_int, c_int, c_void_p, c_void_p, c_float,
+                                          c_void_p, c_int64, c_void_p, c_void_p, c_int64, c_void_p, c_void_p]),
+    "sagnn_ln_mhsa_mean_packed_f32": (c_int, [c_void_p, c_int64, c_int64, c_int64, c_int, c_int, c_int, c_void_p, c_void_p,
+                                              c_float, c_void_p, c_void_p, c_void_p, c_void_p, c_void_p, c_void_p, c_void_p,
+                                              c_int64, c_void_p]),
     "sagnn_layernorm_td_f32": (c_int, [c_void_p, c_int64, c_int64, c_int64, c_int, c_int, c_void_p, c_void_p,
                                        c_float, c_void_p, c_int64, c_void_p]),
     "sagnn_mhsa_mean_f32": (c_int, [c_void_p, c_int64, c_int64, c_int64, c_int, c_int, c_int, c_void_p,
diff --git a/sa-gnn_amd/csrc/attn_split.hip b/sa-gnn_amd/csrc/attn_split.hip
--- a/sa-gnn_amd/csrc/attn_split.hip
+++ b/sa-gnn_amd/csrc/attn_split.hip
@@ -61,7 +61,21 @@
   return v;
 }
 
-template <int D, int T, int LP, bool BWD>
+constexpr float kMuRLim = 1.f;
+
+template <int E>
+__device__ __forceinline__ float unpack_h(i32x4 pk, float kinv) {
+  float r;
+  if constexpr (E & 1) asm("v_fma_mix_f32 %0, %1, %2, %3 op_sel:[1,0,1] op_sel_hi:[1,0,1]" : "=v"(r) : "v"(pk[2 + (E >> 1)]), "v"(kinv), "v"(pk[E >> 1]));
+  else asm("v_fma_mix_f32 %0, %1, %2, %3 op_sel_hi:[1,0,1]" : "=v"(r) : "v"(pk[2 + (E >> 1)]), "v"(kinv), "v"(pk[E >> 1]));
+  return r;
+}
+__device__ __forceinline__ float unpack_h_at(const float* row, int k) {
+  const _Float16* const p = reinterpret_cast<const _Float16*>(row) + 8 * (k >> 2) + (k & 3);
+  return fmaf((float)p[4], kLoInv, (float)p[0]);
+}
+
+template <int D, int T, int LP, bool BWD, bool PK>
 __global__ __launch_bounds__(64 * (D >= 64 ? 4 : D / 16), (D == 128 || (BWD && T >= 8)) ? 1 : 2) void ln_mhsa_split_kernel(
     const float* __restrict__ x, int64_t ld_n, int64_t ld_t, int64_t n, const float* __restrict__ gamma,
     const float* __restrict__ beta, float eps, int apply_ln, const float* __restrict__ Wq,
@@ -69,6 +83,7 @@
     const float* __restrict__ Wv, const float* __restrict__ bv, float* out, int64_t ld_out,
     int64_t n_tiles, float* __restrict__ dqkv_out, float* __restrict__ y_out, unsigned int* __restrict__ redo_ctr) {
   static_assert(!BWD || D <= 64 || LP == 1, "d = 128: the backward front keeps a pair in one lane");
+  static_assert(!PK || (D == 64 && !BWD), "packed h: the d = 64 forward");
   constexpr int NW = D >= 64 ? 4 : D / 16, NT = 64 * NW, KS = D / 32;
   constexpr int DK = D / 16;
   constexpr int HPW = 16 / DK;
@@ -115,7 +130,12 @@
       for (int ks = 0; ks < KS; ++ks) {
         float wv[8];
 #pragma unroll
-        for (int j = 0; j < 8; ++j) wv[j] = Ws[mat][(size_t)(32 * ks + 8 * q + j) * D + cbase + m] * (mat == 0 ? qscale : 1.f);
+        for (int j = 0; j < 8; ++j) {
+          const int k = 32 * ks + 8 * q + j;
+          wv[j] = Ws[mat][(size_t)k * D + cbase + m];
+          if constexpr (PK) wv[j] *= gamma[k];
+          wv[j] *= (mat == 0 ? qscale : 1.f);
+        }
         range_seg4(wr, wv[0], wv[1], wv[2], wv[3]);
         range_seg4(wr, wv[4], wv[5], wv[6], wv[7]);
 #pragma unroll
@@ -128,11 +148,31 @@
     if (range_bad(wr)) flags[2] = 1;
   }
   f32x4 bias3[3];
+  f32x4 g3[3];
 #pragma unroll
   for (int r = 0; r < 4; ++r) {
     bias3[0][r] = bq[col0 + r] * qscale;
     bias3[1][r] = bk[col0 + r];
     bias3[2][r] = bv[col0 + r];
+  }
+  if constexpr (PK) {
+    const float* const Ws[3] = {Wq, Wk, Wv};
+#pragma unroll
+    for (int mat = 0; mat < 3; ++mat) {
+      const float sc = mat == 0 ? qscale : 1.f;
+      f32x4 cs = {0.f, 0.f, 0.f, 0.f}, gs = {0.f, 0.f, 0.f, 0.f};
+      for (int k = 0; k < D; ++k) {
+        const f32x4 w = *reinterpret_cast<const f32x4*>(Ws[mat] + (size_t)k * D + col0);
+        const float gk = gamma[k], bk_ = beta[k];
+#pragma unroll
+        for (int r = 0; r < 4; ++r) {
+          gs[r] += (w[r] * gk) * sc;
+          cs[r] = fmaf(bk_, w[r] * sc, cs[r]);
+        }
+      }
+      bias3[mat] += cs;
+      g3[mat] = gs;
+    }
   }
   float4 g4 = make_float4(1.f, 1.f, 1.f, 1.f), b4 = make_float4(0.f, 0.f, 0.f, 0.f);
   if (apply_ln) {
@@ -161,6 +201,20 @@
     if (tid == 0) flags[par] = 0;
     int fr_ = fr, fc4_ = fc4, m_ = m, q_ = q;
     asm volatile("" : "+v"(fr_), "+v"(fc4_), "+v"(m_), "+v"(q_));
+    bool mu_bad = false;
+    if constexpr (PK) {
+#pragma unroll
+      for (int p = 0; p < NFILL; ++p) {
+        const int r = fill_row(p, fr_);
+        const i32x4 pk = __builtin_bit_cast(i32x4, xr[p]);
+        const int off = r * (D * 2) + (((fc4_ >> 3) ^ swz<D>(r)) << 4) + ((fc4_ >> 2) & 1) * 8;
+        *reinterpret_cast<i32x2*>(Yp + off) = i32x2{pk[0], pk[1]};
+        *reinterpret_cast<i32x2*>(Yp + PLANE + off) = i32x2{pk[2], pk[3]};
+        float kinv = kLoInv;
+        asm volatile("" : "+v"(kinv));
+        xr[p] = make_float4(unpack_h<0>(pk, kinv), unpack_h<1>(pk, kinv), unpack_h<2>(pk, kinv), unpack_h<3>(pk, kinv));
+      }
+    }
 
     float2 wst[NFILL];
     if constexpr (WL) {
@@ -189,6 +243,7 @@
           if constexpr (GP >= 2) q2 += __shfl_xor(q2, 16);
           if constexpr (GP == 4) q2 += __shfl_xor(q2, 32);
           const float2 st = make_float2(mean, rsqrtf(q2 * (1.f / (float)(T * D)) + eps));
+          if constexpr (PK) mu_bad |= !(fabsf(st.x) * st.y <= kMuRLim);
 #pragma unroll
           for (int i = 0; i < PP; ++i) wst[j * PP + i] = st;
           const int r0 = fill_row(j * PP, fr_);
@@ -216,13 +271,15 @@
           const float dm = st.x - mean;
           m2 += st.y + (float)D * dm * dm;
         }
-        nstat[tid] = make_float2(mean, rsqrtf(m2 * (1.f / (float)(T * D)) + eps));
-      }
-      lds_barrier();
+        const float2 st = make_float2(mean, rsqrtf(m2 * (1.f / (float)(T * D)) + eps));
+        if constexpr (PK) mu_bad |= !(fabsf(st.x) * st.y <= kMuRLim);
+        nstat[tid] = st;
+      }
+      if constexpr (!PK) lds_barrier();
     }
     RangeTrack yr = range_init();
 #pragma unroll
-    for (int p = 0; p < NFILL; ++p) {
+    for (int p = 0; p < (PK ? 0 : NFILL); ++p) {
       const int r = fill_row(p, fr_);
       float4 y = xr[p];
       if (apply_ln) {
@@ -245,13 +302,14 @@
     }
     fetch_tile(tile + gridDim.x);
     lds_barrier();
-    if (range_bad(yr)) flags[par] = 1;
+    if (PK ? mu_bad : range_bad(yr)) flags[par] = 1;
 
 #pragma unroll
     for (int bt = 0; bt < kBT; ++bt) {
       const int row = bt * 16 + m_;
       const int sw = swz<D>(row);
       f32x4 hi[3] = {bias3[0], bias3[1], bias3[2]};
+      if constexpr (PK) hi[0] = hi[1] = hi[2] = f32x4{0.f, 0.f, 0.f, 0.f};
       f32x4 lo[3];
 #pragma unroll
       for (int ks = 0; ks < KS; ++ks) {
@@ -268,10 +326,20 @@
         }
       }
       f32x4 acc[3];
+      float rs = 1.f, nmur = 0.f;
+      if constexpr (PK) {
+        const int nb = row / T;
+        const float2 st = nstat[nb < NB ? nb : NB - 1];
+        rs = st.y;
+        nmur = -st.x * st.y;
+      }
 #pragma unroll
       for (int mat = 0; mat < 3; ++mat)
 #pragma unroll
-        for (int r = 0; r < 4; ++r) acc[mat][r] = fmaf(lo[mat][r], kLoInv, hi[mat][r]);
+        for (int r = 0; r < 4; ++r) {
+          acc[mat][r] = fmaf(lo[mat][r], kLoInv, hi[mat][r]);
+          if constexpr (PK) acc[mat][r] = fmaf(rs, acc[mat][r], fmaf(nmur, g3[mat][r], bias3[mat][r]));
+        }
       char* rec = tab + q_ * GS + row * kRec + (row / T) * PN;
       *reinterpret_cast<f32x4*>(rec) = acc[0];
       *reinterpret_cast<f32x4*>(rec + 16) = acc[1];
@@ -293,7 +361,7 @@
         const float* const xrow = x + (node0 + nb) * ld_n + (int64_t)ts * ld_t;
         float acc = bs[mat][col] * sc;
         for (int k = 0; k < D; ++k) {
-          float yv = xrow[k];
+          float yv = PK ? unpack_h_at(xrow, k) : xrow[k];
           if (apply_ln) {
             const float ik = st.y * gamma[k];
             yv = yv * ik + (beta[k] - st.x * ik);
@@ -463,7 +531,7 @@
 
 namespace sagnn {
 
-template <int D, int T, bool BWD = false>
+template <int D, int T, bool BWD = false, bool PK = false>
 static int launch_split(const float* x, int64_t ld_n, int64_t ld_t, int64_t n, const float* gamma, const float* beta,
                         float eps, int apply_ln, const float* Wq, const float* bq, const float* Wk, const float* bk,
                         const float* Wv, const float* bv, float* out, int64_t ld_out, hipStream_t s,
@@ -472,14 +540,14 @@
   constexpr int LP = (BWD && D == 128) ? 1 : lanes_per_pair(T, D);
   constexpr int GS = kRows * kRec + NB * pad_node(T) + pad_group(T);
   const size_t lds = (size_t)2 * kRows * D * 2 + (size_t)NW * 4 * GS + (size_t)(kRows + NB) * sizeof(float2) + 16;
-  if (int rc = ensure_dynamic_lds(reinterpret_cast<const void*>(&ln_mhsa_split_kernel<D, T, LP, BWD>), lds)) return rc;
+  if (int rc = ensure_dynamic_lds(reinterpret_cast<const void*>(&ln_mhsa_split_kernel<D, T, LP, BWD, PK>), lds)) return rc;
   const int per_cu = (D == 128 || (BWD && T >= 8)) ? 1 : D == 64 ? 2 : 4;
   constexpr int CB = D == 128 ? 2 : 1;
   const int64_t n_tiles = (n + NB - 1) / NB;
   const int64_t want = (int64_t)cu_count_current() * per_cu / CB;
   const int64_t blocks = n_tiles < want ? n_tiles : (want > 0 ? want : 1);
   ProfileScope prof(kProfMhsa, s, n, T);
-  hipLaunchKernelGGL((ln_mhsa_split_kernel<D, T, LP, BWD>), dim3((unsigned)blocks, CB), dim3(64 * NW), lds, s, x, ld_n, ld_t, n,
+  hipLaunchKernelGGL((ln_mhsa_split_kernel<D, T, LP, BWD, PK>), dim3((unsigned)blocks, CB), dim3(64 * NW), lds, s, x, ld_n, ld_t, n,
                      gamma, beta, eps, apply_ln, Wq, bq, Wk, bk, Wv, bv, out, ld_out, n_tiles, dqkv, y, redo_counter());
   SAGNN_HIP_TRY(hipGetLastError());
   return SAGNN_OK;
@@ -507,6 +575,21 @@
   if (d == 128) return dispatch_t<128>(x, ld_n, ld_t, n, t, gamma, beta, eps, apply_ln, Wq, bq, Wk, bk, Wv, bv, out, ld_out, s);
   if (d == 64) return dispatch_t<64>(x, ld_n, ld_t, n, t, gamma, beta, eps, apply_ln, Wq, bq, Wk, bk, Wv, bv, out, ld_out, s);
   return dispatch_t<32>(x, ld_n, ld_t, n, t, gamma, beta, eps, apply_ln, Wq, bq, Wk, bk, Wv, bv, out, ld_out, s);
+}
+
+int ln_mhsa_mean_split_packed(const float* hp, int64_t ld_n, int64_t ld_t, int64_t n, int t, int d, int heads,
+                              const float* gamma, const float* beta, float eps, const float* Wq, const float* bq,
+                              const float* Wk, const float* bk, const float* Wv, const float* bv, float* out, int64_t ld_out,
+                              hipStream_t s) {
+  if (d != 64 || !mhsa_split_supported(d, t, heads)) return fail(SAGNN_ERR_DIM, "split attention, packed h: unsupported d/t/heads");
+#define SAGNN_T_CASE(TT) \
+  case TT: return launch_split<64, TT, false, true>(hp, ld_n, ld_t, n, gamma, beta, eps, 1, Wq, bq, Wk, bk, Wv, bv, out, ld_out, s);
+  switch (t) {
+    SAGNN_T_CASE(1) SAGNN_T_CASE(2) SAGNN_T_CASE(3) SAGNN_T_CASE(4) SAGNN_T_CASE(5) SAGNN_T_CASE(6)
+    SAGNN_T_CASE(8) SAGNN_T_CASE(12) SAGNN_T_CASE(16)
+    default: return fail(SAGNN_ERR_DIM, "split attention: t = %d has no specialised kernel", t);
+  }
+#undef SAGNN_T_CASE
 }
 
 template <int D>
diff --git a/sa-gnn_amd/csrc/common.h b/sa-gnn_amd/csrc/common.h
--- a/sa-gnn_amd/csrc/common.h
+++ b/sa-gnn_amd/csrc/common.h
@@ -47,6 +47,13 @@
 int lstm_fwd_f16(const float* x, int64_t ld_n, int64_t ld_t, int64_t n, int t, int d, const float* W, const float* b,
                  float forget_bias, const float* drop, float* h, int64_t ld_h, float* gates_out, float* c_out,
                  const float* h_init, int64_t ld_hi, const float* c_init, float* c_final, hipStream_t s);
+int lstm_fwd_f16_packed(const float* x, int64_t ld_n, int64_t ld_t, int64_t n, int t, int d, const float* W, const float* b,
+                        float forget_bias, float* h, int64_t ld_h, const float* h_init, int64_t ld_hi, const float* c_init,
+                        float* c_final, hipStream_t s);
+int ln_mhsa_mean_split_packed(const float* hp, int64_t ld_n, int64_t ld_t, int64_t n, int t, int d, int heads,
+                              const float* gamma, const float* beta, float eps, const float* Wq, const float* bq,
+                              const float* Wk, const float* bk, const float* Wv, const float* bv, float* out, int64_t ld_out,
+                              hipStream_t s);
 int ln_mhsa_mean_split(const float* x, int64_t ld_n, int64_t ld_t, int64_t n, int t, int d, int heads,
                        const float* gamma, const float* beta, float eps, int apply_ln, const float* Wq,
                        const float* bq, const float* Wk, const float* bk, const float* Wv, const float* bv,
diff --git a/sa-gnn_amd/csrc/engine.cpp b/sa-gnn_amd/csrc/engine.cpp
--- a/sa-gnn_amd/csrc/engine.cpp
+++ b/sa-gnn_amd/csrc/engine.cpp
@@ -25,6 +25,10 @@
   if (vec && mhsa_mfma_supported(d, t, heads)) return AttnFwd::F32Mfma;
   if (!d32_or_64(d) && wide_supported(d)) return AttnFwd::Wide;
   return AttnFwd::Valu;
+}
+
+bool select_fusion_packed(Engine e, int d, int t, int heads) {
+  return e == Engine::F16x2 && d == 64 && mhsa_split_supported(d, t, heads);
 }
 
 AttnBwdFront select_attn_bwd_front(Engine e, int d, int t, int heads) {
diff --git a/sa-gnn_amd/csrc/engine.h b/sa-gnn_amd/csrc/engine.h
--- a/sa-gnn_amd/csrc/engine.h
+++ b/sa-gnn_amd/csrc/engine.h
@@ -16,6 +16,7 @@
 
 LstmFwd select_lstm_fwd(Engine e, int d, int t, bool vec, int64_t ld_h, bool h_vec, bool train, bool drop, bool drop_vec);
 AttnFwd select_attn_fwd(Engine e, int d, int t, int heads, bool vec);
+bool select_fusion_packed(Engine e, int d, int t, int heads);
 AttnBwdFront select_attn_bwd_front(Engine e, int d, int t, int heads);
 AttnBwdTail select_attn_bwd_tail(Engine e, int d);
 LstmBwd select_lstm_bwd(Engine e, int d, bool workspace);
diff --git a/sa-gnn_amd/csrc/fusion.hip b/sa-gnn_amd/csrc/fusion.hip
--- a/sa-gnn_amd/csrc/fusion.hip
+++ b/sa-gnn_amd/csrc/fusion.hip
@@ -401,6 +401,50 @@
   return SAGNN_OK;
 }
 
+extern "C" int sagnn_fusion_packed_supported(int d, int t, int heads) {
+  return sagnn::select_fusion_packed(sagnn::calling_engine(), d, t, heads) ? 1 : 0;
+}
+
+extern "C" int sagnn_lstm_fwd_packed_f32(const float* x, int64_t ld_n, int64_t ld_t, int64_t n, int t, int d, const float* W,
+                                         const float* b, float forget_bias, const void* h_init_packed, int64_t ld_hi,
+                                         const float* c_init, void* h_packed, int64_t ld_h, float* c_final, void* stream) {
+  if (int rc = check_dims(n, t, d)) return rc;
+  if (!sagnn::select_fusion_packed(sagnn::calling_engine(), d, 1, 16))
+    return sagnn::fail(SAGNN_ERR_DIM, "packed LSTM: d = %d is not run as the packed pair under this engine", d);
+  if (!x || !W || !b || !h_packed) return sagnn::fail(SAGNN_ERR_NULL, "null tensor pointer");
+  if ((h_init_packed == nullptr) != (c_init == nullptr)) return sagnn::fail(SAGNN_ERR_NULL, "give both h_init and c_init or neither");
+  if (int rc = check_strides(ld_n, ld_t, n, t, d)) return rc;
+  if (ld_h < (int64_t)t * d) return sagnn::fail(SAGNN_ERR_ARG, "ld_h smaller than t*d");
+  if (h_init_packed && ld_hi < d) return sagnn::fail(SAGNN_ERR_ARG, "ld_hi smaller than d");
+  if (!sagnn::aligned16(x) || (ld_n & 3) || (ld_t & 3) || !sagnn::aligned16(h_packed) || (ld_h & 3) ||
+      (h_init_packed && (!sagnn::aligned16(h_init_packed) || (ld_hi & 3))))
+    return sagnn::fail(SAGNN_ERR_ALIGN, "packed LSTM: x, h and h_init rows must be 16-byte aligned");
+  if (n == 0) return SAGNN_OK;
+  return sagnn::lstm_fwd_f16_packed(x, ld_n, ld_t, n, t, d, W, b, forget_bias, static_cast<float*>(h_packed), ld_h,
+                                    static_cast<const float*>(h_init_packed), ld_hi, c_init, c_final,
+                                    static_cast<hipStream_t>(stream));
+}
+
+extern "C" int sagnn_ln_mhsa_mean_packed_f32(const void* h_packed, int64_t ld_n, int64_t ld_t, int64_t n, int t, int d, int heads,
+                                             const float* ln_gamma, const float* ln_beta, float ln_eps, const float* Wq,
+                                             const float* bq, const float* Wk, const float* bk, const float* Wv,
+                                             const float* bv, float* out, int64_t ld_out, void* stream) {
+  if (int rc = check_dims(n, t, d)) return rc;
+  if (heads < 1 || d % heads) return sagnn::fail(SAGNN_ERR_DIM, "heads = %d does not divide d = %d", heads, d);
+  if (!sagnn::select_fusion_packed(sagnn::calling_engine(), d, t, heads))
+    return sagnn::fail(SAGNN_ERR_DIM, "packed attention: d = %d, t = %d, heads = %d is not run as the packed pair under this engine",
+                       d, t, heads);
+  if (!h_packed || !ln_gamma || !ln_beta || !Wq || !bq || !Wk || !bk || !Wv || !bv || !out)
+    return sagnn::fail(SAGNN_ERR_NULL, "null tensor pointer");
+  if (int rc = check_strides(ld_n, ld_t, n, t, d)) return rc;
+  if (ld_out < d) return sagnn::fail(SAGNN_ERR_ARG, "ld_out smaller than d");
+  if (!sagnn::aligned16(h_packed) || (ld_n & 3) || (ld_t & 3))
+    return sagnn::fail(SAGNN_ERR_ALIGN, "packed attention: h rows must be 16-byte aligned");
+  if (n == 0) return SAGNN_OK;
+  return sagnn::ln_mhsa_mean_split_packed(static_cast<const float*>(h_packed), ld_n, ld_t, n, t, d, heads, ln_gamma, ln_beta,
+                                          ln_eps, Wq, bq, Wk, bk, Wv, bv, out, ld_out, static_cast<hipStream_t>(stream));
+}
+
 static bool fused(sagnn::AttnFwd k) { return k == sagnn::AttnFwd::Split || k == sagnn::AttnFwd::F32Mfma; }
 
 static int fused_attention(sagnn::AttnFwd k, const float* x, int64_t ld_n, int64_t ld_t, int64_t n, int t, int d, int heads,
diff --git a/sa-gnn_amd/csrc/lstm_f16.hip b/sa-gnn_amd/csrc/lstm_f16.hip
--- a/sa-gnn_amd/csrc/lstm_f16.hip
+++ b/sa-gnn_amd/csrc/lstm_f16.hip
@@ -15,4 +15,16 @@
   return fail(SAGNN_ERR_DIM, "f16 LSTM supports d = 32 or 64, got %d", d);
 }
 
+int lstm_fwd_f16_packed(const float* x, int64_t ld_n, int64_t ld_t, int64_t n, int t, int d, const float* W, const float* b,
+                        float forget_bias, float* h, int64_t ld_h, const float* h_init, int64_t ld_hi, const float* c_init,
+                        float* c_final, hipStream_t s) {
+  if (d != 64) return fail(SAGNN_ERR_DIM, "f16 LSTM, packed h: d = 64 only, got %d", d);
+  if (ld_h >= (1 << 22) || (int64_t)t * d >= (1 << 18))
+    return fail(SAGNN_ERR_ARG, "f16 LSTM: output row stride must stay below 2^22 floats and t*d below 2^18");
+  if (ld_h < (int64_t)t * d) return fail(SAGNN_ERR_ARG, "f16 LSTM: ld_h = %lld < t*d", (long long)ld_h);
+  const float* drop = nullptr;
+  float *gates_out = nullptr, *c_out = nullptr;
+  return lstm_f16_d64_pack(SAGNN_LSTM_F16_PASS);
 }
+
+}
diff --git a/sa-gnn_amd/csrc/lstm_f16_d64_pack.hip b/sa-gnn_amd/csrc/lstm_f16_d64_pack.hip
--- /dev/null
+++ b/sa-gnn_amd/csrc/lstm_f16_d64_pack.hip
@@ -0,0 +1,8 @@
+#include "lstm_f16_kernel.h"
+
+namespace sagnn {
+int lstm_f16_d64_pack(SAGNN_LSTM_F16_ARGS) {
+  if (drop) return fail(SAGNN_ERR_ARG, "f16 LSTM: the packed form takes no dropout mask");
+  return launch_lstm_f16<64, false, false, true>(SAGNN_LSTM_F16_PASS);
+}
+}
diff --git a/sa-gnn_amd/csrc/lstm_f16_kernel.h b/sa-gnn_amd/csrc/lstm_f16_kernel.h
--- a/sa-gnn_amd/csrc/lstm_f16_kernel.h
+++ b/sa-gnn_amd/csrc/lstm_f16_kernel.h
@@ -57,13 +57,14 @@
   return __builtin_amdgcn_rcpf(1.f + __builtin_amdgcn_exp2f(-1.44269504088896340736f * z));
 }
 
-template <int D, bool SAVE, bool DROP>
+template <int D, bool SAVE, bool DROP, bool PACK>
 __global__ __launch_bounds__(64 * (D / 16), 1) void lstm_fwd_f16_kernel(
     const float* __restrict__ x, int64_t ld_n, int64_t ld_t, int64_t n, int t, const float* __restrict__ W,
     const float* __restrict__ bias, float forget_bias, const float* __restrict__ drop, float* __restrict__ h_out,
     int64_t ld_h, float* __restrict__ gates_out, float* __restrict__ c_out, int64_t n_tiles,
     const float* __restrict__ h_init, int64_t ld_hi, const float* __restrict__ c_init, float* __restrict__ c_final,
     unsigned int* __restrict__ redo_ctr) {
+  static_assert(!PACK || (!SAVE && !DROP), "packed h: inference without a mask");
   constexpr int NW = D / 16;
   constexpr int NT = 64 * NW;
   constexpr int KSH = D / 32;
@@ -170,6 +171,14 @@
 #pragma unroll
       for (int p = 0; p < NFILL; ++p) {
         const int r = p * RPP + fr;
+        if constexpr (PACK) {
+          i32x4 pk = {0, 0, 0, 0};
+          if (r < rows_valid) pk = *reinterpret_cast<const i32x4*>(h_init + (row0 + r) * ld_hi + fc4);
+          const int off = r * (D * 2) + (((fc4 >> 3) ^ swz<D>(r)) << 4) + ((fc4 >> 2) & 1) * 8;
+          *reinterpret_cast<i32x2*>(Hp + off) = i32x2{pk[0], pk[1]};
+          *reinterpret_cast<i32x2*>(Hp + PLANE + off) = i32x2{pk[2], pk[3]};
+          continue;
+        }
         float4 v = make_float4(0.f, 0.f, 0.f, 0.f);
         if (r < rows_valid) v = *reinterpret_cast<const float4*>(h_init + (row0 + r) * ld_hi + fc4);
         range_seg4_hi(xrng, v.x, v.y, v.z, v.w);
@@ -270,10 +279,14 @@
         } else if constexpr (K == 115) {
           *reinterpret_cast<i32x2*>(Hnxt + hoff) = i32x2{w0[0], w0[1]};
           *reinterpret_cast<i32x2*>(Hnxt + PLANE + hoff) = i32x2{w1[0], w1[1]};
+          if constexpr (PACK)
+            __builtin_amdgcn_raw_buffer_store_b128(i32x4{w0[0], w0[1], w1[0], w1[1]}, rs_h, (row * (int)ld_h + ts * D + hid) * 4, 0, 0);
         } else if constexpr (K == 116) {
-          const i32x4 hvv = {__builtin_bit_cast(int, hv[0]), __builtin_bit_cast(int, hv[1]), __builtin_bit_cast(int, hv[2]),
-                             __builtin_bit_cast(int, hv[3])};
-          __builtin_amdgcn_raw_buffer_store_b128(hvv, rs_h, (row * (int)ld_h + ts * D + hid) * 4, 0, 0);
+          if constexpr (!PACK) {
+            const i32x4 hvv = {__builtin_bit_cast(int, hv[0]), __builtin_bit_cast(int, hv[1]), __builtin_bit_cast(int, hv[2]),
+                               __builtin_bit_cast(int, hv[3])};
+            __builtin_amdgcn_raw_buffer_store_b128(hvv, rs_h, (row * (int)ld_h + ts * D + hid) * 4, 0, 0);
+          }
           c[PB] = f32x4{cn[0], cn[1], cn[2], cn[3]};
         } else if constexpr (K == 117) {
           if constexpr (SAVE) {
@@ -391,7 +404,12 @@
       for (int idx = tid; idx < kRows * D; idx += NT) {
         const int r = idx / D, uu = idx - r * D;
         const bool live = r < rows_valid;
-        hs[idx] = (h_init && live) ? h_init[(row0 + r) * ld_hi + uu] : 0.f;
+        if constexpr (PACK) {
+          const _Float16* const hp = reinterpret_cast<const _Float16*>(h_init + (row0 + r) * ld_hi) + 8 * (uu >> 2) + (uu & 3);
+          hs[idx] = (h_init && live) ? fmaf((float)hp[4], kLoInv, (float)hp[0]) : 0.f;
+        } else {
+          hs[idx] = (h_init && live) ? h_init[(row0 + r) * ld_hi + uu] : 0.f;
+        }
         cs[idx] = (c_init && live) ? c_init[(row0 + r) * D + uu] : 0.f;
       }
       constexpr int RSTEP = NT / D, RPT = kRows / RSTEP;
@@ -440,7 +458,14 @@
           hnx[idx] = hnew;
           if (r < rows_valid) {
             const int64_t e_td = ((row0 + r) * t + ts) * D + uu;
-            h_out[(row0 + r) * ld_h + (int64_t)ts * D + uu] = DROP ? hnew * drop[e_td] : hnew;
+            if constexpr (PACK) {
+              _Float16* const hp = reinterpret_cast<_Float16*>(h_out + (row0 + r) * ld_h + (int64_t)ts * D) + 8 * (uu >> 2) + (uu & 3);
+              const _Float16 hd = (_Float16)hnew;
+              hp[0] = hd;
+              hp[4] = (_Float16)((hnew - (float)hd) * 4096.f);
+            } else {
+              h_out[(row0 + r) * ld_h + (int64_t)ts * D + uu] = DROP ? hnew * drop[e_td] : hnew;
+            }
             if constexpr (SAVE) {
               float* const gp = gates_out + ((row0 + r) * t + ts) * NC + uu;
               gp[0] = gi, gp[D] = gj, gp[2 * D] = gf, gp[3 * D] = go;
@@ -461,18 +486,18 @@
 
 namespace sagnn {
 
-template <int D, bool SAVE, bool DROP>
+template <int D, bool SAVE, bool DROP, bool PACK = false>
 int launch_lstm_f16(const float* x, int64_t ld_n, int64_t ld_t, int64_t n, int t, const float* W, const float* b,
                     float forget_bias, const float* drop, float* h, int64_t ld_h, float* gates_out, float* c_out,
                     const float* h_init, int64_t ld_hi, const float* c_init, float* c_final, hipStream_t s) {
   const size_t lds = (size_t)8 * kRows * D * 2 + 16;
-  if (int rc = ensure_dynamic_lds(reinterpret_cast<const void*>(&lstm_fwd_f16_kernel<D, SAVE, DROP>), lds)) return rc;
+  if (int rc = ensure_dynamic_lds(reinterpret_cast<const void*>(&lstm_fwd_f16_kernel<D, SAVE, DROP, PACK>), lds)) return rc;
   const int per_cu = D == 64 ? 1 : 2;
   const int64_t n_tiles = (n + kRows - 1) / kRows;
   const int64_t want = (int64_t)cu_count_current() * per_cu;
   const int64_t blocks = n_tiles < want ? n_tiles : want;
   ProfileScope prof(kProfLstm, s, n, t);
-  hipLaunchKernelGGL((lstm_fwd_f16_kernel<D, SAVE, DROP>), dim3((unsigned)blocks), dim3(64 * (D / 16)), lds, s, x, ld_n, ld_t,
+  hipLaunchKernelGGL((lstm_fwd_f16_kernel<D, SAVE, DROP, PACK>), dim3((unsigned)blocks), dim3(64 * (D / 16)), lds, s, x, ld_n, ld_t,
                      n, t, W, b, forget_bias, drop, h, ld_h, gates_out, c_out, n_tiles, h_init, ld_hi, c_init, c_final, redo_counter());
   SAGNN_HIP_TRY(hipGetLastError());
   return SAGNN_OK;
@@ -487,5 +512,6 @@
 int lstm_f16_d64_save(SAGNN_LSTM_F16_ARGS);
 int lstm_f16_d32(SAGNN_LSTM_F16_ARGS);
 int lstm_f16_d32_save(SAGNN_LSTM_F16_ARGS);
-
-}
+int lstm_f16_d64_pack(SAGNN_LSTM_F16_ARGS);
+
+}
diff --git a/sa-gnn_amd/ops.py b/sa-gnn_amd/ops.py
--- a/sa-gnn_amd/ops.py
+++ b/sa-gnn_amd/ops.py
@@ -426,6 +426,39 @@
     return out
 
 
+def fusion_packed(d: int, t: int, heads: int) -> bool:
+    return bool(_lib.load().sagnn_fusion_packed_supported(int(d), int(t), int(heads)))
+
+
+def lstm_fwd_packed(x: torch.Tensor, W: torch.Tensor, b: torch.Tensor, out: torch.Tensor, forget_bias: float = 1.0,
+                    h0: torch.Tensor | None = None, c0: torch.Tensor | None = None, c_out: torch.Tensor | None = None):
+    n, t, d, ld, ldt = _ntd("x", x)
+    _, _, _, ldh, _ = _ntd("out", out, dense_td=True)
+    if (h0 is None) != (c0 is None):
+        raise ValueError("give both h0 and c0 or neither")
+    ld_hi = 0
+    if h0 is not None:
+        ld_hi = _f32_rows("h0", h0, d, n)
+        if _f32_rows("c0", c0, d, n) != d:
+            raise ValueError("c0 must be contiguous [n, d]")
+    if c_out is not None and _f32_rows("c_out", c_out, d, n) != d:
+        raise ValueError("c_out must be contiguous [n, d]")
+    check(_lib.load().sagnn_lstm_fwd_packed_f32(x.data_ptr(), ld, ldt, n, t, d, _vec("W", W, 8 * d * d), _vec("b", b, 4 * d),
+                                                float(forget_bias), _ptr(h0), ld_hi, _ptr(c0), out.data_ptr(), ldh,
+                                                _ptr(c_out), _stream()))
+    return out
+
+
+def ln_mhsa_mean_packed(hp: torch.Tensor, gamma, beta, Wq, bq, Wk, bk, Wv, bv, heads: int, eps: float = 1e-12):
+    n, t, d, ld, ldt = _ntd("hp", hp)
+    out = torch.empty((n, d), dtype=torch.float32, device=hp.device)
+    check(_lib.load().sagnn_ln_mhsa_mean_packed_f32(
+        hp.data_ptr(), ld, ldt, n, t, d, int(heads), _vec("gamma", gamma, d), _vec("beta", beta, d), float(eps),
+        _vec("Wq", Wq, d * d), _vec("bq", bq, d), _vec("Wk", Wk, d * d), _vec("bk", bk, d), _vec("Wv", Wv, d * d),
+        _vec("bv", bv, d), out.data_ptr(), d, _stream()))
+    return out
+
+
 def layernorm_td(x: torch.Tensor, gamma: torch.Tensor, beta: torch.Tensor, eps: float = 1e-12,
                  out: torch.Tensor | None = None):
     n, t, d, ld, ldt = _ntd("x", x)
```

Result: slower. 17.83 billion (-1.0%).
